# efmanu/SubspaceInference.jl

Measured on AMD Instinct MI355X. Metric: posterior samples/sec (whole node) + subspace-construct wall-clock, 1M-param MLP M=20, higher is better.
Workload: dtype f64

## Files before the change

include/subspace_hip.h:

```cpp
#ifndef SUBSPACE_HIP_H
#define SUBSPACE_HIP_H

#include <stdint.h>

#ifdef __cplusplus
extern "C" {
#endif

typedef struct si_ctx si_ctx;

enum {
  SI_OK = 0,
  SI_ERR_INVALID = -1,
  SI_ERR_STATE = -2,
  SI_ERR_HIP = -3,
  SI_ERR_NOMEM = -4,
  SI_ERR_BOUNDS = -5,
  SI_ERR_NODEVICE = -6,
  SI_ERR_COMM = -7
};

enum { SI_F32 = 0, SI_F64 = 1 };
enum { SI_ACT_IDENTITY = 0, SI_ACT_RELU = 1, SI_ACT_TANH = 2, SI_ACT_SIGMOID = 3, SI_ACT_LEAKYRELU = 4, SI_ACT_ELU = 5,
       SI_ACT_SOFTPLUS = 6, SI_ACT_SELU = 7, SI_ACT_COUNT = 8 };
enum { SI_LAYER_DENSE = 0, SI_LAYER_CONV = 1, SI_LAYER_MAXPOOL = 2, SI_LAYER_FLATTEN = 3 };

typedef struct {
  int32_t kind;
  int32_t in;
  int32_t out;
  int32_t act;
  int64_t w_off;
  int64_t b_off;
  int32_t kw, kh;
  int32_t cin, cout;
  int32_t wi, hi;
  int32_t sw, sh;
  int32_t pw, ph;
  int32_t dw, dh;
} si_layer;

enum {
  SI_K_PUSH = 0,
  SI_K_GRAM = 1,
  SI_K_GRAM_RED = 2,
  SI_K_PROJECT = 3,
  SI_K_RECON = 4,
  SI_K_DENSE = 5,
  SI_K_SSE = 6,
  SI_K_RWMH = 7,
  SI_K_DENSE_MAIN = 8,
  SI_K_EIG_HOST = 9,
  SI_K_BACKWARD = 10,
  SI_K_CONV = 11,
  SI_K_CONV_AUX = 12,
  SI_K_COUNT = 13
};

typedef struct {
  double ms[SI_K_COUNT];
  int64_t launches[SI_K_COUNT];
  double flops[SI_K_COUNT];
  double bytes[SI_K_COUNT];
} si_stats;

int32_t si_version(void);

int32_t si_create(si_ctx** out, int32_t device_id);
int32_t si_destroy(si_ctx* ctx);
const char* si_last_error(si_ctx* ctx);
int32_t si_set_stream(si_ctx* ctx, void* hip_stream);
int32_t si_synchronize(si_ctx* ctx);
int32_t si_set_profiling(si_ctx* ctx, int32_t on);
int32_t si_set_profiling_classes(si_ctx* ctx, uint32_t class_mask);
int32_t si_get_stats(si_ctx* ctx, si_stats* out);
int32_t si_reset_stats(si_ctx* ctx);
int32_t si_device_name(si_ctx* ctx, char* buf, int32_t buflen);

int32_t si_construct_begin(si_ctx* ctx, int64_t N, int64_t K_capacity, int32_t max_cols);
int32_t si_construct_set_mean(si_ctx* ctx, const void* w_host, int32_t w_dtype);
int32_t si_construct_set_storage(si_ctx* ctx, int32_t a_dtype);
int32_t si_construct_push(si_ctx* ctx, const void* w_host, int32_t w_dtype, double n);
int32_t si_construct_push_dev(si_ctx* ctx, const void* w_dev, int32_t w_dtype, double n);
int32_t si_construct_push_batch_dev(si_ctx* ctx, const void* w_dev, int32_t w_dtype, int64_t ld, int32_t count,
                                    const double* n_host);
int32_t si_construct_gram(si_ctx* ctx);
int32_t si_construct_gram_get(si_ctx* ctx, double* G_host , int64_t* K_out);
int32_t si_construct_gram_set(si_ctx* ctx, const double* G_host );
int32_t si_construct_gram_ptr(si_ctx* ctx, double** G_dev_out, int64_t* K_out);
int32_t si_construct_needs_refine(si_ctx* ctx, int32_t M, int32_t* flag_out);
int32_t si_construct_refine(si_ctx* ctx);
int32_t si_construct_finish(si_ctx* ctx, int32_t M, double* W_swa_out ,
                            double* P_out , double* s_out ,
                            int64_t* K_out);
int32_t si_construct_result_ptr(si_ctx* ctx, double** W_swa_dev_out, double** P_dev_out, int64_t* ld_out, int32_t* M_out);
int32_t si_construct_get_result(si_ctx* ctx, double* W_swa_out , double* P_out , double* s_out ,
                                int64_t* N_out, int32_t* M_out);
int32_t si_construct_get_A(si_ctx* ctx, int64_t k0, int64_t nk, double* A_out);

int32_t si_infer_setup(si_ctx* ctx, const si_layer* layers, int32_t L, int64_t N, int32_t M,
                       const double* W_swa, const double* P, const double* X, const double* Y,
                       int32_t in_dim, int32_t out_dim, int64_t B, double sigma_m,
                       int32_t compute_dtype);
int32_t si_infer_setup_dev(si_ctx* ctx, const si_layer* layers, int32_t L, int64_t N, int32_t M,
                           const double* W_swa_dev, const double* P_dev, int64_t ldP, int32_t borrow,
                           const double* X_dev, const double* Y_dev, int32_t in_dim, int32_t out_dim, int64_t B,
                           double sigma_m, int32_t compute_dtype);
int32_t si_infer_set_prior(si_ctx* ctx, double sigma_p);
int32_t si_logdensity(si_ctx* ctx, const double* Z, int32_t C, double* lp_out );
int32_t si_logdensity_grad(si_ctx* ctx, const double* z , double* lp_out, double* grad_out );
int32_t si_logdensity_grad_batch(si_ctx* ctx, const double* Z , int32_t C, double* lp_out ,
                                 double* grad_out );
int32_t si_grad_kernel_info(si_ctx* ctx, int32_t* fused_out);
int32_t si_sample_mala(si_ctx* ctx, int64_t itr, double sigma_z, uint64_t seed, int32_t chain_id0, int32_t nchains,
                       double* Z_out , double* lp_out , double* accept_rate_out ,
                       double* G_out );
int32_t si_mala_kernel_info(si_ctx* ctx, int32_t* fused_out, int32_t* passes_out);
int32_t si_sample_hmc(si_ctx* ctx, int64_t itr, int64_t n_adapts, double sigma_z, double delta, uint64_t seed, int32_t chain_id0,
                      int32_t nchains, double* Z_out , double* lp_out ,
                      double* alpha_out , double* eps_out ,
                      double* G_out , double* Minv_out );
int32_t si_hmc_kernel_info(si_ctx* ctx, int32_t* fused_out, int32_t* passes_out, int32_t* search_rounds_out);
int32_t si_sample_nuts(si_ctx* ctx, int64_t itr, int64_t n_adapts, double sigma_z, double delta, int32_t max_depth, double max_dh,
                       uint64_t seed, int32_t chain_id0, int32_t nchains, double* Z_out ,
                       double* lp_out , double* alpha_out , double* eps_out ,
                       int32_t* depth_out , int32_t* nleaf_out , int32_t* sel_out ,
                       double* G_out , double* Minv_out ,
                       double* leaf_out , int64_t leaf_cap);
int32_t si_nuts_kernel_info(si_ctx* ctx, int32_t* fused_out, int32_t* passes_out, int32_t* search_rounds_out, int64_t* rounds_out,
                            int64_t* leaves_out);
int32_t si_fit_advi(si_ctx* ctx, int64_t max_iters , int32_t samples_per_step , double sigma_z, double eta, double tau,
                    int32_t window , uint64_t seed, int32_t chain_id0, int32_t nruns , int64_t ndraws ,
                    double* theta_out , double* Z_out ,
                    double* elbo_out , double* theta_trace_out ,
                    double* points_out );
int32_t si_advi_kernel_info(si_ctx* ctx, int32_t* fused_out, int32_t* passes_out);
int32_t si_forward(si_ctx* ctx, const double* z , double* Yhat_out );
int32_t si_predict(si_ctx* ctx, const double* Z , int32_t C, const double* Xnew ,
                   int64_t Bn, double* Yhat_out);
int32_t si_sample_rwmh(si_ctx* ctx, int64_t itr, double sigma_z, uint64_t seed, int32_t chain_id0,
                       int32_t nchains, double* Z_out, double* lp_out, double* accept_rate_out);
int32_t si_sample_rwmh_weights(si_ctx* ctx, int64_t itr, double sigma_z, uint64_t seed, int32_t chain_id0,
                               int32_t nchains, double* Z_out, double* lp_out, double* accept_rate_out, double* W_out);
int32_t si_rwmh_begin(si_ctx* ctx, int64_t itr, double sigma_z, uint64_t seed, int32_t chain_id0, int32_t nchains,
                      int64_t d_total);
int32_t si_rwmh_step_eval(si_ctx* ctx, double* sse_local_out );
int32_t si_rwmh_step_accept(si_ctx* ctx, const double* sse_total );
int32_t si_rwmh_sse_ptr(si_ctx* ctx, double** sse_dev_out, int32_t* nchains_out);
int32_t si_rwmh_end(si_ctx* ctx, double* Z_out, double* lp_out, double* accept_rate_out);
int32_t si_rwmh_abort(si_ctx* ctx);
int32_t si_set_chain_loop(si_ctx* ctx, int32_t on);
int32_t si_chain_kernel_info(si_ctx* ctx, int32_t* density_specialised, int32_t* loop_specialised);
const char* si_chain_spec_message(si_ctx* ctx);
int32_t si_reconstruct(si_ctx* ctx, const double* Z , int64_t C, double* W_out);

int32_t si_train_setup(si_ctx* ctx, const si_layer* layers, int32_t L, int64_t N, const float* w0 ,
                       const double* X, const double* Y, int32_t in_dim, int32_t out_dim, int64_t B_total,
                       int64_t batch_max, int32_t opt_kind, double eta, double p1, double p2);
enum { SI_DTYPE_OF_DATA = -1 };
int32_t si_train_setup_ex(si_ctx* ctx, const si_layer* layers, int32_t L, int64_t N, const float* w0 , const void* X,
                          const void* Y, int32_t data_dtype, int32_t in_dim, int32_t out_dim, int64_t B_total, int64_t batch_max,
                          int32_t opt_kind, double eta, double p1, double p2, int32_t compute_dtype);
int32_t si_train_compute_dtype(si_ctx* ctx, int32_t* out );
int32_t si_train_step(si_ctx* ctx, const int64_t* idx , int64_t nb,
                      double* loss_out );
int32_t si_train_push(si_ctx* ctx, double n);
int32_t si_train_get_weights(si_ctx* ctx, float* w_out );
int32_t si_train_get_opt_state(si_ctx* ctx, float* m_out , float* v_out , double* beta_pows_out );
int32_t si_train_grad(si_ctx* ctx, const int64_t* idx, int64_t nb, int64_t nb_total, double* sse_local_out );
int32_t si_train_grad_ptr(si_ctx* ctx, double** grad_dev_out, int64_t* n_out);
int32_t si_train_grad_get(si_ctx* ctx, double* g_out );
int32_t si_train_grad_set(si_ctx* ctx, const double* g_in );
int32_t si_train_apply(si_ctx* ctx);

#define SI_COMM_ID_BYTES 128
enum { SI_COMM_SUM = 0, SI_COMM_MAX = 1 };
int32_t si_comm_unique_id(uint8_t* id_out );
int32_t si_comm_init_rank(si_ctx* ctx, int32_t world, int32_t rank, const uint8_t* id );
int32_t si_comm_destroy(si_ctx* ctx);
int32_t si_comm_info(si_ctx* ctx, int32_t* world_out, int32_t* rank_out, int32_t* rccl_version_out);
int32_t si_comm_allreduce_host(si_ctx* ctx, double* inout, int64_t n, int32_t op);
int32_t si_comm_allgather_host(si_ctx* ctx, const double* send , int64_t n, double* recv );
int32_t si_comm_barrier(si_ctx* ctx);
int32_t si_row_shard(int64_t n_total, int32_t rank, int32_t world, int64_t* r0_out, int64_t* r1_out);
int32_t si_construct_allreduce_gram(si_ctx* ctx);
int32_t si_construct_allgather(si_ctx* ctx, int64_t n_total);
int32_t si_bcast_subspace(si_ctx* ctx, int32_t root, int64_t N, int32_t M);
int32_t si_rwmh_allreduce_sse(si_ctx* ctx);
int32_t si_sample_rwmh_sharded(si_ctx* ctx, int64_t itr, double sigma_z, uint64_t seed, int32_t chain_id0, int32_t nchains,
                               int64_t d_total, double* Z_out, double* lp_out, double* accept_rate_out);
int32_t si_train_allreduce_grad(si_ctx* ctx, double* sse_total_out);
int32_t si_train_step_dp(si_ctx* ctx, const int64_t* idx, int64_t nb, int64_t nb_total, double* loss_out);

int si_host_sym_eig(int n, double* a, double* w);
int si_host_sym_eig_top(int n, const double* g, int m, double* w_top, double* V);
int si_host_jacobi_eig_psd(int n, double* a, double* w, double* v);
int32_t si_host_hmc_windows(int64_t n_adapts, int64_t* window_start, int64_t* window_end, int64_t* splits, int32_t cap);
int si_host_cpu_budget(void);
double si_host_parse_cpu_max(const char* text);
int si_host_copy_plan(int budget, int nproc, const char* env );

#ifdef __cplusplus
}
#endif
#endif
```

subspaceinference.jl_amd/_capi.py:

```python
import ctypes
import os
from ctypes import (POINTER, Structure, byref, c_char_p, c_double, c_int, c_int32, c_int64, c_uint64,
                    c_void_p)

import numpy as np

HERE = os.path.dirname(os.path.abspath(__file__))
LIB_PATH = os.path.join(HERE, "libsubspace_hip.so")

SI_OK, SI_ERR_INVALID, SI_ERR_STATE, SI_ERR_HIP, SI_ERR_NOMEM, SI_ERR_BOUNDS, SI_ERR_NODEVICE = 0, -1, -2, -3, -4, -5, -6
SI_ERR_COMM = -7
SI_COMM_ID_BYTES, SI_COMM_SUM, SI_COMM_MAX = 128, 0, 1
SI_F32, SI_F64 = 0, 1
SI_DTYPE_OF_DATA = -1
ACT_IDENTITY, ACT_RELU, ACT_TANH, ACT_SIGMOID = 0, 1, 2, 3
ACT_LEAKYRELU, ACT_ELU, ACT_SOFTPLUS, ACT_SELU = 4, 5, 6, 7
K_NAMES = ["push", "gram", "gram_reduce", "project", "reconstruct", "dense", "sse", "rwmh", "dense_main", "eig_host", "backward",
           "conv", "conv_aux"]
LAYER_DENSE, LAYER_CONV, LAYER_MAXPOOL, LAYER_FLATTEN = 0, 1, 2, 3
K_COUNT = len(K_NAMES)


class SubspaceError(RuntimeError):

    def __init__(self, msg, code=SI_ERR_INVALID):
        super().__init__(msg)
        self.code = code


class BoundsError(SubspaceError, IndexError):
    """Julia's BoundsError at `U[:,1:M]` (src/subspace_construction.jl:65) when rank(A) < M."""


class SiLayer(Structure):
    _fields_ = [("kind", c_int32), ("in_", c_int32), ("out", c_int32), ("act", c_int32),
                ("w_off", c_int64), ("b_off", c_int64),
                ("kw", c_int32), ("kh", c_int32), ("cin", c_int32), ("cout", c_int32), ("wi", c_int32), ("hi", c_int32),
                ("sw", c_int32), ("sh", c_int32), ("pw", c_int32), ("ph", c_int32), ("dw", c_int32), ("dh", c_int32)]


class SiStats(Structure):
    _fields_ = [("ms", c_double * K_COUNT), ("launches", c_int64 * K_COUNT),
                ("flops", c_double * K_COUNT), ("bytes", c_double * K_COUNT)]


SIGNATURES = {
    "si_version": (c_int32, []),
    "si_create": (c_int32, [POINTER(c_void_p), c_int32]),
    "si_destroy": (c_int32, [c_void_p]),
    "si_last_error": (c_char_p, [c_void_p]),
    "si_set_stream": (c_int32, [c_void_p, c_void_p]),
    "si_synchronize": (c_int32, [c_void_p]),
    "si_set_profiling": (c_int32, [c_void_p, c_int32]),
    "si_set_profiling_classes": (c_int32, [c_void_p, ctypes.c_uint32]),
    "si_get_stats": (c_int32, [c_void_p, POINTER(SiStats)]),
    "si_reset_stats": (c_int32, [c_void_p]),
    "si_device_name": (c_int32, [c_void_p, c_char_p, c_int32]),
    "si_construct_begin": (c_int32, [c_void_p, c_int64, c_int64, c_int32]),
    "si_construct_set_mean": (c_int32, [c_void_p, c_void_p, c_int32]),
    "si_construct_push": (c_int32, [c_void_p, c_void_p, c_int32, c_double]),
    "si_construct_push_dev": (c_int32, [c_void_p, c_void_p, c_int32, c_double]),
    "si_construct_push_batch_dev": (c_int32, [c_void_p, c_void_p, c_int32, c_int64, c_int32, c_void_p]),
    "si_construct_gram": (c_int32, [c_void_p]),
    "si_construct_gram_get": (c_int32, [c_void_p, c_void_p, POINTER(c_int64)]),
    "si_construct_gram_set": (c_int32, [c_void_p, c_void_p]),
    "si_construct_gram_ptr": (c_int32, [c_void_p, POINTER(c_void_p), POINTER(c_int64)]),
    "si_construct_result_ptr": (c_int32, [c_void_p, POINTER(c_void_p), POINTER(c_void_p), POINTER(c_int64),
                                          POINTER(c_int32)]),
    "si_construct_needs_refine": (c_int32, [c_void_p, c_int32, POINTER(c_int32)]),
    "si_construct_refine": (c_int32, [c_void_p]),
    "si_construct_finish": (c_int32, [c_void_p, c_int32, c_void_p, c_void_p, c_void_p, POINTER(c_int64)]),
    "si_construct_get_A": (c_int32, [c_void_p, c_int64, c_int64, c_void_p]),
    "si_construct_get_result": (c_int32, [c_void_p, c_void_p, c_void_p, c_void_p, POINTER(c_int64), POINTER(c_int32)]),
    "si_infer_setup": (c_int32, [c_void_p, POINTER(SiLayer), c_int32, c_int64, c_int32, c_void_p, c_void_p,
                                 c_void_p, c_void_p, c_int32, c_int32, c_int64, c_double, c_int32]),
    "si_infer_setup_dev": (c_int32, [c_void_p, POINTER(SiLayer), c_int32, c_int64, c_int32, c_void_p, c_void_p, c_int64,
                                     c_int32, c_void_p, c_void_p, c_int32, c_int32, c_int64, c_double, c_int32]),
    "si_infer_set_prior": (c_int32, [c_void_p, c_double]),
    "si_logdensity": (c_int32, [c_void_p, c_void_p, c_int32, c_void_p]),
    "si_logdensity_grad": (c_int32, [c_void_p, c_void_p, c_void_p, c_void_p]),
    "si_logdensity_grad_batch": (c_int32, [c_void_p, c_void_p, c_int32, c_void_p, c_void_p]),
    "si_grad_kernel_info": (c_int32, [c_void_p, POINTER(c_int32)]),
    "si_forward": (c_int32, [c_void_p, c_void_p, c_void_p]),
    "si_predict": (c_int32, [c_void_p, c_void_p, c_int32, c_void_p, c_int64, c_void_p]),
    "si_sample_rwmh": (c_int32, [c_void_p, c_int64, c_double, c_uint64, c_int32, c_int32, c_void_p, c_void_p,
                                 c_void_p]),
    "si_sample_rwmh_weights": (c_int32, [c_void_p, c_int64, c_double, c_uint64, c_int32, c_int32, c_void_p, c_void_p,
                                         c_void_p, c_void_p]),
    "si_sample_mala": (c_int32, [c_void_p, c_int64, c_double, c_uint64, c_int32, c_int32, c_void_p, c_void_p, c_void_p,
                                 c_void_p]),
    "si_mala_kernel_info": (c_int32, [c_void_p, POINTER(c_int32), POINTER(c_int32)]),
    "si_sample_hmc": (c_int32, [c_void_p, c_int64, c_int64, c_double, c_double, c_uint64, c_int32, c_int32, c_void_p, c_void_p,
                                c_void_p, c_void_p, c_void_p, c_void_p]),
    "si_hmc_kernel_info": (c_int32, [c_void_p, POINTER(c_int32), POINTER(c_int32), POINTER(c_int32)]),
    "si_sample_nuts": (c_int32, [c_void_p, c_int64, c_int64, c_double, c_double, c_int32, c_double, c_uint64, c_int32, c_int32,
                                 c_void_p, c_void_p, c_void_p, c_void_p, c_void_p, c_void_p, c_void_p, c_void_p, c_void_p, c_void_p,
                                 c_int64]),
    "si_nuts_kernel_info": (c_int32, [c_void_p, POINTER(c_int32), POINTER(c_int32), POINTER(c_int32), POINTER(c_int64),
                                      POINTER(c_int64)]),
    "si_fit_advi": (c_int32, [c_void_p, c_int64, c_int32, c_double, c_double, c_double, c_int32, c_uint64, c_int32, c_int32, c_int64,
                              c_void_p, c_void_p, c_void_p, c_void_p, c_void_p]),
    "si_advi_kernel_info": (c_int32, [c_void_p, POINTER(c_int32), POINTER(c_int32)]),
    "si_rwmh_begin": (c_int32, [c_void_p, c_int64, c_double, c_uint64, c_int32, c_int32, c_int64]),
    "si_rwmh_step_eval": (c_int32, [c_void_p, c_void_p]),
    "si_rwmh_step_accept": (c_int32, [c_void_p, c_void_p]),
    "si_rwmh_sse_ptr": (c_int32, [c_void_p, POINTER(c_void_p), POINTER(c_int32)]),
    "si_rwmh_end": (c_int32, [c_void_p, c_void_p, c_void_p, c_void_p]),
    "si_rwmh_abort": (c_int32, [c_void_p]),
    "si_reconstruct": (c_int32, [c_void_p, c_void_p, c_int64, c_void_p]),
    "si_train_setup": (c_int32, [c_void_p, POINTER(SiLayer), c_int32, c_int64, c_void_p, c_void_p, c_void_p, c_int32,
                                 c_int32, c_int64, c_int64, c_int32, c_double, c_double, c_double]),
    "si_train_setup_ex": (c_int32, [c_void_p, POINTER(SiLayer), c_int32, c_int64, c_void_p, c_void_p, c_void_p, c_int32, c_int32,
                                    c_int32, c_int64, c_int64, c_int32, c_double, c_double, c_double, c_int32]),
    "si_train_compute_dtype": (c_int32, [c_void_p, c_void_p]),
    "si_train_step": (c_int32, [c_void_p, c_void_p, c_int64, c_void_p]),
    "si_train_push": (c_int32, [c_void_p, c_double]),
    "si_train_get_weights": (c_int32, [c_void_p, c_void_p]),
    "si_train_get_opt_state": (c_int32, [c_void_p, c_void_p, c_void_p, c_void_p]),
    "si_train_grad": (c_int32, [c_void_p, c_void_p, c_int64, c_int64, c_void_p]),
    "si_train_grad_ptr": (c_int32, [c_void_p, c_void_p, c_void_p]),
    "si_train_grad_get": (c_int32, [c_void_p, c_void_p]),
    "si_train_grad_set": (c_int32, [c_void_p, c_void_p]),
    "si_train_apply": (c_int32, [c_void_p]),
    "si_comm_unique_id": (c_int32, [c_void_p]),
    "si_comm_init_rank": (c_int32, [c_void_p, c_int32, c_int32, c_void_p]),
    "si_comm_destroy": (c_int32, [c_void_p]),
    "si_comm_info": (c_int32, [c_void_p, POINTER(c_int32), POINTER(c_int32), POINTER(c_int32)]),
    "si_comm_allreduce_host": (c_int32, [c_void_p, c_void_p, c_int64, c_int32]),
    "si_comm_allgather_host": (c_int32, [c_void_p, c_void_p, c_int64, c_void_p]),
    "si_comm_barrier": (c_int32, [c_void_p]),
    "si_row_shard": (c_int32, [c_int64, c_int32, c_int32, POINTER(c_int64), POINTER(c_int64)]),
    "si_construct_allreduce_gram": (c_int32, [c_void_p]),
    "si_construct_allgather": (c_int32, [c_void_p, c_int64]),
    "si_bcast_subspace": (c_int32, [c_void_p, c_int32, c_int64, c_int32]),
    "si_rwmh_allreduce_sse": (c_int32, [c_void_p]),
    "si_sample_rwmh_sharded": (c_int32, [c_void_p, c_int64, c_double, c_uint64, c_int32, c_int32, c_int64, c_void_p, c_void_p,
                                         c_void_p]),
    "si_train_allreduce_grad": (c_int32, [c_void_p, c_void_p]),
    "si_train_step_dp": (c_int32, [c_void_p, c_void_p, c_int64, c_int64, c_void_p]),
    "si_host_sym_eig": (c_int, [c_int, c_void_p, c_void_p]),
    "si_host_sym_eig_top": (c_int, [c_int, c_void_p, c_int, c_void_p, c_void_p]),
    "si_host_jacobi_eig_psd": (c_int, [c_int, c_void_p, c_void_p, c_void_p]),
    "si_set_chain_loop": (c_int32, [c_void_p, c_int32]),
    "si_chain_kernel_info": (c_int32, [c_void_p, POINTER(c_int32), POINTER(c_int32)]),
    "si_chain_spec_message": (c_char_p, [c_void_p]),
    "si_construct_set_storage": (c_int32, [c_void_p, c_int32]),
    "si_host_hmc_windows": (c_int32, [c_int64, POINTER(c_int64), POINTER(c_int64), c_void_p, c_int32]),
    "si_host_cpu_budget": (c_int, []),
    "si_host_parse_cpu_max": (c_double, [c_char_p]),
    "si_host_copy_plan": (c_int, [c_int, c_int, c_char_p]),
}

_lib = None

ADVI_REFUSALS = (
    ("max_iters < 1", lambda a: not a["T"] >= 1),
    ("samples_per_step < 1", lambda a: not a["S"] >= 1),
    ("samples_per_step * ceil(M / 2) >= 2^24", lambda a: a["S"] * ((a["M"] + 1) // 2) >= 2 ** 24),
    ("window outside 1 .. 1024", lambda a: not 1 <= a["W"] <= 1024),
    ("nruns < 1", lambda a: not a["R"] >= 1),
    ("chain_id0 < 0", lambda a: not a["chain_id0"] >= 0),
    ("sigma_z <= 0", lambda a: not a["sigma_z"] > 0.0),
    ("tau <= 0", lambda a: not a["tau"] > 0.0),
    ("eta <= 0", lambda a: not a["eta"] > 0.0),
    ("ndraws < 0", lambda a: not a["D"] >= 0),
)


def advi_refusal(m, max_iters, samples_per_step, sigma_z, eta, tau, window, chain_id0, nruns, ndraws):
    a = dict(M=m, T=max_iters, S=samples_per_step, sigma_z=sigma_z, eta=eta, tau=tau, W=window, chain_id0=chain_id0, R=nruns, D=ndraws)
    return next((what for what, bad in ADVI_REFUSALS if bad(a)), None)


def load():
    global _lib
    if _lib is not None:
        return _lib
    if not os.path.exists(LIB_PATH):
        raise SubspaceError(
            "libsubspace_hip.so is missing (%s): build it with `python __graft_entry__.py` -- "
            "this package has no CPU or PyTorch fallback" % LIB_PATH, SI_ERR_NODEVICE)
    if os.environ.get("SI_PRELOAD_TORCH", "1") != "0":
        try:
            import torch
        except Exception:
            pass
    lib = ctypes.CDLL(LIB_PATH, mode=ctypes.RTLD_GLOBAL)
    for name, (res, args) in SIGNATURES.items():
        fn = getattr(lib, name)
        fn.restype = res
        fn.argtypes = args
    _lib = lib
    return lib


def _ptr(a):
    return None if a is None else c_void_p(a.__array_interface__["data"][0])


def conv_out_size(wi, k, s, p, d):
    return (wi + 2 * p - d * (k - 1) - 1) // s + 1


def _layer_array(table):
    arr = (SiLayer * len(table))()
    for i, row in enumerate(table):
        if row[0] == "conv":
            _, (kw, kh, cin, cout), (wi, hi), (sw, sh), (pw, ph), (dw, dh), act, w_off, b_off = row
            wo, ho = conv_out_size(wi, kw, sw, pw, dw), conv_out_size(hi, kh, sh, ph, dh)
            arr[i] = SiLayer(LAYER_CONV, wi * hi * cin, wo * ho * cout, int(act), int(w_off), int(b_off), kw, kh, cin, cout,
                             wi, hi, sw, sh, pw, ph, dw, dh)
        elif row[0] == "maxpool":
            _, (kw, kh), c, (wi, hi), (sw, sh) = row
            wo, ho = (wi - kw) // sw + 1, (hi - kh) // sh + 1
            arr[i] = SiLayer(LAYER_MAXPOOL, wi * hi * c, wo * ho * c, 0, 0, 0, kw, kh, c, c, wi, hi, sw, sh, 0, 0, 1, 1)
        elif row[0] == "flatten":
            _, c, (wi, hi) = row
            arr[i] = SiLayer(LAYER_FLATTEN, wi * hi * c, wi * hi * c, 0, 0, 0, 0, 0, c, c, wi, hi, 1, 1, 0, 0, 1, 1)
        else:
            fin, fout, act, w_off, b_off = row[:5]
            arr[i] = SiLayer(LAYER_DENSE, int(fin), int(fout), int(act), int(w_off), int(b_off))
    return arr


def _f64(a, order="F"):
    return np.require(a, dtype=np.float64, requirements=[order, "A"])


class Context:

    def __init__(self, device=0):
        self.lib = load()
        h = c_void_p()
        rc = self.lib.si_create(byref(h), int(device))
        if rc != SI_OK:
            msg = self.lib.si_last_error(None).decode()
            raise SubspaceError(msg, rc)
        self.h = h
        self.device = int(device)

    def _check(self, rc):
        if rc == SI_OK:
            return
        msg = self.lib.si_last_error(self.h).decode()
        if rc == SI_ERR_BOUNDS:
            raise BoundsError(msg, rc)
        raise SubspaceError(msg, rc)

    def close(self):
        if getattr(self, "h", None) is not None and self.h:
            self.lib.si_destroy(self.h)
            self.h = None

    def __del__(self):
        try:
            self.close()
        except Exception:
            pass

    def __enter__(self):
        return self

    def __exit__(self, *exc):
        self.close()

    def device_name(self):
        buf = ctypes.create_string_buffer(256)
        self._check(self.lib.si_device_name(self.h, buf, 256))
        return buf.value.decode()

    def set_stream(self, stream_handle):
        self._check(self.lib.si_set_stream(self.h, c_void_p(stream_handle) if stream_handle else None))

    def synchronize(self):
        self._check(self.lib.si_synchronize(self.h))

    def set_profiling(self, on, classes=None):
        self._check(self.lib.si_set_profiling(self.h, 1 if on else 0))
        mask = 0xFFFFFFFF if classes is None else sum(1 << K_NAMES.index(k) for k in classes)
        self._check(self.lib.si_set_profiling_classes(self.h, mask))

    def reset_stats(self):
        self._check(self.lib.si_reset_stats(self.h))

    def stats(self):
        st = SiStats()
        self._check(self.lib.si_get_stats(self.h, byref(st)))
        return {K_NAMES[i]: {"ms": st.ms[i], "launches": st.launches[i], "flops": st.flops[i], "bytes": st.bytes[i]}
                for i in range(K_COUNT)}

    def comm_init_rank(self, world, rank, uid):
        if len(uid) != SI_COMM_ID_BYTES:
            raise SubspaceError("comm_init_rank: the id must be %d bytes" % SI_COMM_ID_BYTES)
        buf = ctypes.create_string_buffer(bytes(uid), SI_COMM_ID_BYTES)
        self._check(self.lib.si_comm_init_rank(self.h, int(world), int(rank), buf))

    def comm_destroy(self):
        self._check(self.lib.si_comm_destroy(self.h))
# ... 246 lines not shown
            raise SubspaceError("DimensionMismatch: z has %d rows, M = %d" % (z.shape[0], self._m))
        lp = np.empty(z.shape[1], dtype=np.float64)
        self._check(self.lib.si_logdensity(self.h, _ptr(z), z.shape[1], _ptr(lp)))
        return lp

    def logdensity_grad(self, z):
        z = _f64(z).reshape(-1)
        if z.size != self._m:
            raise SubspaceError("DimensionMismatch: z has %d elements, M = %d" % (z.size, self._m))
        lp = np.empty(1, dtype=np.float64)
        g = np.empty(self._m, dtype=np.float64)
        self._check(self.lib.si_logdensity_grad(self.h, _ptr(z), _ptr(lp), _ptr(g)))
        return float(lp[0]), g

    def logdensity_grad_batch(self, z):
        z = _f64(z)
        if z.ndim == 1:
            z = z.reshape(-1, 1, order="F")
        if z.ndim != 2 or z.shape[0] != self._m:
            raise SubspaceError("DimensionMismatch: z has %d rows, M = %d" % (z.shape[0], self._m))
        lp = np.empty(z.shape[1], dtype=np.float64)
        g = np.empty((self._m, z.shape[1]), dtype=np.float64, order="F")
        self._check(self.lib.si_logdensity_grad_batch(self.h, _ptr(z), z.shape[1], _ptr(lp), _ptr(g)))
        return lp, g

    def grad_kernel_info(self):
        f = c_int32(0)
        self._check(self.lib.si_grad_kernel_info(self.h, byref(f)))
        return int(f.value)

    def forward(self, z):
        z = _f64(z).reshape(-1)
        yhat = np.empty((self._out, self._b), dtype=np.float64, order="F")
        self._check(self.lib.si_forward(self.h, _ptr(z), _ptr(yhat)))
        return yhat

    def predict(self, z, xnew):
        z = _f64(z)
        if z.ndim == 1:
            z = z.reshape(-1, 1, order="F")
        xnew = _f64(xnew)
        if z.shape[0] != self._m or xnew.ndim != 2 or xnew.shape[0] != self._in:
            raise SubspaceError("DimensionMismatch: Z %s, Xnew %s" % (z.shape, xnew.shape))
        out = np.empty((self._out, xnew.shape[1], z.shape[1]), dtype=np.float64, order="F")
        self._check(self.lib.si_predict(self.h, _ptr(z), z.shape[1], _ptr(xnew), xnew.shape[1], _ptr(out)))
        return out

    def sample_rwmh(self, itr, sigma_z, seed, chain_id0=0, nchains=1, want_z=True):
        z = np.empty((self._m, int(itr), int(nchains)), dtype=np.float64, order="F") if want_z else None
        lp = np.empty((int(itr), int(nchains)), dtype=np.float64, order="F")
        acc = np.empty(int(nchains), dtype=np.float64)
        self._check(self.lib.si_sample_rwmh(self.h, int(itr), float(sigma_z), int(seed), int(chain_id0), int(nchains),
                                            _ptr(z), _ptr(lp), _ptr(acc)))
        return z, lp, acc

    def sample_rwmh_weights(self, itr, sigma_z, seed, chain_id0=0, nchains=1, out=None):
        z = np.empty((self._m, int(itr), int(nchains)), dtype=np.float64, order="F")
        lp = np.empty((int(itr), int(nchains)), dtype=np.float64, order="F")
        acc = np.empty(int(nchains), dtype=np.float64)
        if out is None:
            w = np.empty((self._ni, int(itr), int(nchains)), dtype=np.float64, order="F")
        else:
            w = out
            if w.dtype != np.float64 or w.shape != (self._ni, int(itr), int(nchains)) or not w.flags.f_contiguous:
                raise ValueError("sample_rwmh_weights: `out` must be a Fortran-ordered float64 array of shape (N, itr, nchains)")
        self._check(self.lib.si_sample_rwmh_weights(self.h, int(itr), float(sigma_z), int(seed), int(chain_id0), int(nchains),
                                                    _ptr(z), _ptr(lp), _ptr(acc), _ptr(w)))
        return z, lp, acc, w

    def sample_mala(self, itr, sigma_z, seed, chain_id0=0, nchains=1, grad=False):
        z = np.empty((self._m, int(itr), int(nchains)), dtype=np.float64, order="F")
        lp = np.empty((int(itr), int(nchains)), dtype=np.float64, order="F")
        acc = np.empty(int(nchains), dtype=np.float64)
        g = np.empty((self._m, int(itr), int(nchains)), dtype=np.float64, order="F") if grad else None
        self._check(self.lib.si_sample_mala(self.h, int(itr), float(sigma_z), int(seed), int(chain_id0), int(nchains),
                                            _ptr(z), _ptr(lp), _ptr(acc), _ptr(g)))
        return (z, lp, acc, g) if grad else (z, lp, acc)

    def mala_kernel_info(self):
        f, p = c_int32(0), c_int32(0)
        self._check(self.lib.si_mala_kernel_info(self.h, byref(f), byref(p)))
        return int(f.value), int(p.value)

    def sample_hmc(self, itr, sigma_z, seed, chain_id0=0, nchains=1, n_adapts=None, delta=0.8, grad=False, metric=False):
        itr, c = int(itr), int(nchains)
        na = int(round(itr / 2)) if n_adapts is None else int(n_adapts)
        cols = max(itr, 0) + 1
        z = np.empty((self._m, cols, max(c, 0)), dtype=np.float64, order="F")
        lp, alpha, eps = (np.empty((cols, max(c, 0)), dtype=np.float64, order="F") for _ in range(3))
        g = np.empty_like(z, order="F") if grad else None
        mi = np.empty_like(z, order="F") if metric else None
        self._check(self.lib.si_sample_hmc(self.h, itr, na, float(sigma_z), float(delta), int(seed), int(chain_id0), c, _ptr(z),
                                           _ptr(lp), _ptr(alpha), _ptr(eps), _ptr(g), _ptr(mi)))
        return (z, lp, alpha, eps) + ((g,) if grad else ()) + ((mi,) if metric else ())

    def hmc_kernel_info(self):
        f, p, r = c_int32(0), c_int32(0), c_int32(0)
        self._check(self.lib.si_hmc_kernel_info(self.h, byref(f), byref(p), byref(r)))
        return int(f.value), int(p.value), int(r.value)

    def sample_nuts(self, itr, sigma_z, seed, chain_id0=0, nchains=1, n_adapts=None, delta=0.8, max_depth=10, max_dh=1000.0,
                    tree=True, grad=False, metric=False, leaf_cap=0):
        itr, c = int(itr), int(nchains)
        na = int(round(itr / 2)) if n_adapts is None else int(n_adapts)
        cols = max(itr, 0) + 1
        z = np.empty((self._m, cols, max(c, 0)), dtype=np.float64, order="F")
        lp, alpha, eps = (np.empty((cols, max(c, 0)), dtype=np.float64, order="F") for _ in range(3))
        depth, nleaf, sel = (np.zeros((cols, max(c, 0)), dtype=np.int32, order="F") if tree else None for _ in range(3))
        g = np.empty_like(z, order="F") if grad else None
        mi = np.empty_like(z, order="F") if metric else None
        leaf = np.full((3 * self._m + 1, int(leaf_cap), max(c, 0)), np.nan, dtype=np.float64, order="F") if leaf_cap else None
        self._check(self.lib.si_sample_nuts(self.h, itr, na, float(sigma_z), float(delta), int(max_depth), float(max_dh), int(seed),
                                            int(chain_id0), c, _ptr(z), _ptr(lp), _ptr(alpha), _ptr(eps), _ptr(depth), _ptr(nleaf),
                                            _ptr(sel), _ptr(g), _ptr(mi), _ptr(leaf), int(leaf_cap)))
        return ((z, lp, alpha, eps) + ((depth, nleaf, sel) if tree else ()) + ((g,) if grad else ()) + ((mi,) if metric else ())
                + ((leaf,) if leaf_cap else ()))

    def nuts_kernel_info(self):
        f, p, r = c_int32(0), c_int32(0), c_int32(0)
        n, lv = c_int64(0), c_int64(0)
        self._check(self.lib.si_nuts_kernel_info(self.h, byref(f), byref(p), byref(r), byref(n), byref(lv)))
        return int(f.value), int(p.value), int(r.value), int(n.value), int(lv.value)

    def fit_advi(self, max_iters, sigma_z, seed, samples_per_step=10, eta=0.1, tau=1.0, window=100, chain_id0=0, nruns=1,
                 ndraws=None, trace=False):
        t, s, w, r = int(max_iters), int(samples_per_step), int(window), int(nruns)
        d = t if ndraws is None else int(ndraws)
        why = advi_refusal(self._m, t, s, float(sigma_z), float(eta), float(tau), w, int(chain_id0), r, d)
        if why is not None:
            raise SubspaceError("si_fit_advi: bad argument (%s)" % why, SI_ERR_INVALID)
        m = self._m
        theta = np.empty((2 * m, r), dtype=np.float64, order="F")
        z = np.empty((m, d, r), dtype=np.float64, order="F")
        elbo = np.empty((t, r), dtype=np.float64, order="F")
        tr = np.empty((2 * m, t + 1, r), dtype=np.float64, order="F") if trace else None
        pts = np.empty((m, s, t, r), dtype=np.float64, order="F") if trace else None
        self._check(self.lib.si_fit_advi(self.h, t, s, float(sigma_z), float(eta), float(tau), w, int(seed), int(chain_id0), r, d,
                                         _ptr(theta), _ptr(z) if d > 0 else None, _ptr(elbo), _ptr(tr), _ptr(pts)))
        return (theta, z, elbo, tr, pts) if trace else (theta, z, elbo)

    def advi_kernel_info(self):
        f, p = c_int32(0), c_int32(0)
        self._check(self.lib.si_advi_kernel_info(self.h, byref(f), byref(p)))
        return int(f.value), int(p.value)

    def set_chain_loop(self, on):
        self._check(self.lib.si_set_chain_loop(self.h, int(on)))

    def chain_kernel_info(self):
        d, l = c_int32(0), c_int32(0)
        self._check(self.lib.si_chain_kernel_info(self.h, byref(d), byref(l)))
        return bool(d.value), bool(l.value), (self.lib.si_chain_spec_message(self.h) or b"").decode()

    def rwmh_begin(self, itr, sigma_z, seed, chain_id0=0, nchains=1, d_total=0):
        self._check(self.lib.si_rwmh_begin(self.h, int(itr), float(sigma_z), int(seed), int(chain_id0), int(nchains),
                                           int(d_total)))
        self._sw = (int(itr), int(nchains))

    def rwmh_step_eval(self, on_device=False):
        if on_device:
            self._check(self.lib.si_rwmh_step_eval(self.h, None))
            return None
        sse = np.empty(self._sw[1], dtype=np.float64)
        self._check(self.lib.si_rwmh_step_eval(self.h, _ptr(sse)))
        return sse

    def rwmh_step_accept(self, sse_total=None):
        if sse_total is None:
            self._check(self.lib.si_rwmh_step_accept(self.h, None))
            return
        sse_total = np.ascontiguousarray(sse_total, dtype=np.float64)
        self._check(self.lib.si_rwmh_step_accept(self.h, _ptr(sse_total)))

    def rwmh_sse_ptr(self):
        ptr, c = c_void_p(), c_int32()
        self._check(self.lib.si_rwmh_sse_ptr(self.h, byref(ptr), byref(c)))
        return int(ptr.value), int(c.value)

    def rwmh_abort(self):
        self._check(self.lib.si_rwmh_abort(self.h))

    def rwmh_end(self):
        itr, c = self._sw
        z = np.empty((self._m, itr, c), dtype=np.float64, order="F")
        lp = np.empty((itr, c), dtype=np.float64, order="F")
        acc = np.empty(c, dtype=np.float64)
        self._check(self.lib.si_rwmh_end(self.h, _ptr(z), _ptr(lp), _ptr(acc)))
        return z, lp, acc

    def reconstruct(self, z, out=None):
        z = _f64(z)
        if z.ndim == 1:
            z = z.reshape(-1, 1, order="F")
        if out is None:
            w = np.empty((self._ni, z.shape[1]), dtype=np.float64, order="F")
        else:
            w = out
            if w.dtype != np.float64 or w.shape != (self._ni, z.shape[1]) or not w.flags.f_contiguous:
                raise ValueError("reconstruct: `out` must be a Fortran-ordered float64 array of shape (N, C)")
        self._check(self.lib.si_reconstruct(self.h, _ptr(z), z.shape[1], _ptr(w)))
        return w


def comm_unique_id():
    lib = load()
    buf = ctypes.create_string_buffer(SI_COMM_ID_BYTES)
    rc = lib.si_comm_unique_id(buf)
    if rc != SI_OK:
        raise SubspaceError(lib.si_last_error(None).decode(), rc)
    return buf.raw


def row_shard(n_total, rank, world):
    r0, r1 = c_int64(), c_int64()
    if load().si_row_shard(int(n_total), int(rank), int(world), byref(r0), byref(r1)) != SI_OK:
        raise SubspaceError("si_row_shard: bad argument")
    return int(r0.value), int(r1.value)


def host_hmc_windows(n_adapts):
    lib = load()
    ws, we = c_int64(), c_int64()
    n = lib.si_host_hmc_windows(int(n_adapts), byref(ws), byref(we), None, 0)
    splits = np.zeros(max(1, n), dtype=np.int64)
    lib.si_host_hmc_windows(int(n_adapts), byref(ws), byref(we), _ptr(splits), n)
    return int(ws.value), int(we.value), [int(v) for v in splits[:n]]


def host_sym_eig(g):
    lib = load()
    a = np.array(g, dtype=np.float64, order="F")
    n = a.shape[0]
    w = np.empty(n, dtype=np.float64)
    rc = lib.si_host_sym_eig(n, _ptr(a), _ptr(w))
    if rc != 0:
        raise SubspaceError("eigensolver did not converge")
    return w, a


def host_sym_eig_top(g, m):
    lib = load()
    a = np.array(g, dtype=np.float64, order="F")
    n = a.shape[0]
    w = np.empty(int(m), dtype=np.float64)
    v = np.empty((n, int(m)), dtype=np.float64, order="F")
    rc = lib.si_host_sym_eig_top(n, _ptr(a), int(m), _ptr(w), _ptr(v))
    return (w, v) if rc == 0 else None


def host_jacobi_eig_psd(g):
    lib = load()
    a = np.array(g, dtype=np.float64, order="F")
    n = a.shape[0]
    w = np.empty(n, dtype=np.float64)
    v = np.empty((n, n), dtype=np.float64, order="F")
    lib.si_host_jacobi_eig_psd(n, _ptr(a), _ptr(w), _ptr(v))
    return w, v
```

subspaceinference.jl_amd/build.py:

```python
import os
import shutil
import subprocess

HERE = os.path.dirname(os.path.abspath(__file__))
CSRC = os.path.join(HERE, "csrc")
LIB = os.path.join(HERE, "libsubspace_hip.so")
ARCH = "gfx950"

SOURCES = [
    ("capi.hip", []),
    ("capi_infer.hip", []),
    ("capi_sample.hip", []),
    ("capi_mala.hip", []),
    ("capi_advi.hip", []),
    ("capi_hmc.hip", []),
    ("capi_nuts.hip", []),
    ("capi_train.hip", []),
    ("comm.hip", []),
    ("host_copy.cpp", []),
    ("kernels_stream.hip", ["-ffp-contract=off"]),
    ("kernels_chain.hip", ["-ffp-contract=off"]),
    ("kernels_mala.hip", ["-ffp-contract=off"]),
    ("kernels_hmc.hip", ["-ffp-contract=off"]),
    ("kernels_nuts.hip", ["-ffp-contract=off"]),
    ("kernels_advi.hip", ["-ffp-contract=off"]),
    ("kernels_chain_grid.hip", ["-ffp-contract=off", "-mllvm", "-amdgpu-mfma-vgpr-form=1"]),
    ("kernels_chain_grad.hip", ["-ffp-contract=off", "-mllvm", "-amdgpu-mfma-vgpr-form=1"]),
    ("kernels_gemm.hip", []),
    ("kernels_gemm_small.hip", []),
    ("kernels_gemm_panel.hip", []),
    ("kernels_gemm_f32.hip", []),
    ("kernels_gram.hip", []),
    ("kernels_gram_wave.hip", ["-DSI_GW_PART=0"], "kernels_gram_wave0"),
    ("kernels_gram_wave.hip", ["-DSI_GW_PART=1"], "kernels_gram_wave1"),
    ("kernels_gram_wave.hip", ["-DSI_GW_PART=2"], "kernels_gram_wave2"),
    ("kernels_project.hip", []),
    ("kernels_bwd.hip", []),
    ("kernels_bwd_f32.hip", []),
    ("kernels_conv.hip", []),
    ("kernels_conv.hip", ["-DSI_CONV_F32"], "kernels_conv_f32"),
    ("capi_net.hip", []),
    ("eig.cpp", ["-DSI_EIG_NS=base"]),
    ("eig.cpp", ["-DSI_EIG_NS=avx2", "-mavx2", "-mfma"], "eig_avx2"),
    ("eig.cpp", ["-DSI_EIG_NS=avx512", "-mavx512f", "-mavx512vl", "-mavx512dq", "-mfma"], "eig_avx512"),
    ("eig_dispatch.cpp", []),
    ("chain_spec_rtc.cpp", []),
]
HEADERS = ["si_internal.h", "dev_buf.h", "philox.h", "kernels_gemm.h", "gemm_pipeline.h", "chain_common.h", "hmc_device.h", "capi_common.h", "chain_spec.inc", "chain_spec_args.h",
           "chain_spec_rtc.h", os.path.join("..", "..", "include", "subspace_hip.h")]
SPEC_SOURCES = [("SI_SPEC_SRC_COMMON", "chain_common.h"), ("SI_SPEC_SRC_PHILOX", "philox.h"), ("SI_SPEC_SRC_ARGS", "chain_spec_args.h"),
                ("SI_SPEC_SRC_KERNELS", "chain_spec.inc")]


def _embed_spec_source(objdir):
    out = os.path.join(objdir, "chain_spec_src.h")
    parts = ["// generated by build.py from " + ", ".join(f for _, f in SPEC_SOURCES) + " -- do not edit\n"]
    for name, f in SPEC_SOURCES:
        text = open(os.path.join(CSRC, f)).read().replace("#pragma once", "")
        assert ')SISPEC"' not in text
        chunks, cur = [], ""
        for line in text.splitlines(keepends=True):
            if len(cur) + len(line) > 12000:
                chunks.append(cur)
                cur = ""
            cur += line
        chunks.append(cur)
        parts.append("static const char %s[] =\n%s;\n" % (name, "\n".join('R"SISPEC(' + c + ')SISPEC"' for c in chunks)))
    new = "".join(parts)
    if not os.path.exists(out) or open(out).read() != new:
        with open(out, "w") as fh:
            fh.write(new)
    return out


def _hipcc():
    exe = shutil.which("hipcc") or "/opt/rocm/bin/hipcc"
    if not os.path.exists(exe):
        raise RuntimeError("hipcc not found: cannot build libsubspace_hip.so")
    return exe


def _stale(target, deps):
    if not os.path.exists(target):
        return True
    t = os.path.getmtime(target)
    return any(os.path.getmtime(d) > t for d in deps)


DEV_LIB = os.path.join(os.path.dirname(HERE), "tools", "bin", "libsubspace_hip_dev.so")


def build(force=False, verbose=False, dev=False):
    hipcc = _hipcc()
    objdir = os.path.join(CSRC, "build_dev" if dev else "build")
    os.makedirs(objdir, exist_ok=True)
    lib = DEV_LIB if dev else LIB
    os.makedirs(os.path.dirname(lib), exist_ok=True)
    hdrs = [os.path.join(CSRC, h) for h in HEADERS] + [os.path.abspath(__file__)]
    _embed_spec_source(objdir)
    objs, jobs = [], []
    for entry in SOURCES + ([("guard_alloc.hip", [])] if dev else []):
        src, extra = entry[0], entry[1]
        s = os.path.join(CSRC, src)
        o = os.path.join(objdir, (entry[2] if len(entry) > 2 else os.path.splitext(src)[0]) + ".o")
        objs.append(o)
        if force or _stale(o, [s] + hdrs):
            jobs.append([hipcc, "--offload-arch=" + ARCH, "-O3", "-std=c++17", "-fPIC", "-Wall", "-Wno-unused-function",
                         "-I", objdir, "-c", s, "-o", o] + extra + (["-DSI_DEV_KNOBS"] if dev else []))

    def run(cmd):
        if verbose:
            print(" ".join(cmd))
        subprocess.run(cmd, check=True)
    if jobs:
        from concurrent.futures import ThreadPoolExecutor
        with ThreadPoolExecutor(max_workers=min(len(jobs), max(1, (os.cpu_count() or 2) - 1), 8)) as ex:
            list(ex.map(run, jobs))
    if force or _stale(lib, objs):
        cmd = [hipcc, "--offload-arch=" + ARCH, "-shared", "-fPIC", "-o", lib] + objs + ["-lhiprtc"]
        if verbose:
            print(" ".join(cmd))
        subprocess.run(cmd, check=True)
    return lib


if __name__ == "__main__":
    import sys
    print(build(verbose=True, dev="--dev" in sys.argv))
```

subspaceinference.jl_amd/csrc/capi.hip:

```cpp
#include <algorithm>
#include <cmath>
#include <chrono>
#include <cstdlib>
#include <cstring>
#include <new>
#include <type_traits>
#include <vector>

#include "capi_common.h"



namespace si {

#ifdef SI_DEV_KNOBS
hipError_t guard_malloc(void** out, size_t bytes);
hipError_t guard_free(void* p);
hipError_t raw_dev_malloc(void** out, size_t bytes) { return guard_malloc(out, bytes); }
hipError_t raw_dev_free(void* p) { return guard_free(p); }
#else
hipError_t raw_dev_malloc(void** out, size_t bytes) { return hipMalloc(out, bytes); }
hipError_t raw_dev_free(void* p) { return hipFree(p); }
#endif

static thread_local std::string g_create_err;

int32_t fail(Ctx* c, int32_t code, const std::string& msg) {
  if (c)
    c->err = msg;
  else
    g_create_err = msg;
  return code;
}

static hipEvent_t get_event(Ctx* c) {
  if (!c->event_pool.empty()) {
    hipEvent_t e = c->event_pool.back();
    c->event_pool.pop_back();
    return e;
  }
  hipEvent_t e = nullptr;
  if (hipEventCreate(&e) != hipSuccess) return nullptr;
  return e;
}

ProfScope::ProfScope(Ctx* c_, int cls_, double flops, double bytes) : c(c_), cls(cls_) {
  if (!c) return;
  c->stats.launches[cls] += 1;
  c->stats.flops[cls] += flops;
  c->stats.bytes[cls] += bytes;
  if (!c->profiling || !((c->prof_mask >> cls) & 1u) || c->pending.size() >= (1u << 20)) return;
  a = get_event(c);
  b = get_event(c);
  if (a && b) (void)hipEventRecord(a, c->stream);
}
ProfScope::~ProfScope() {
  if (!c || !a || !b) return;
  (void)hipEventRecord(b, c->stream);
  c->pending.push_back({a, b, cls});
}

static void resolve_events(Ctx* c) {
  for (auto& p : c->pending) {
    float ms = 0.f;
    if (hipEventElapsedTime(&ms, p.a, p.b) == hipSuccess) c->stats.ms[p.cls] += (double)ms;
    c->event_pool.push_back(p.a);
    c->event_pool.push_back(p.b);
  }
  c->pending.clear();
}


static void free_construct(Ctx* c) {
  if (c->i_ready && c->i_swa == c->d_swa && c->d_swa != nullptr) free_infer(c);
  static_cast<ConstructState&>(*c) = ConstructState();
}

void free_infer(Ctx* c) { static_cast<InferState&>(*c) = InferState(); }

int32_t construct_adopt(Ctx* c, int64_t N, int32_t M) {
  const int64_t ld = pad_ld(N);
  DevBuf<double> w, p;
  if (!w.alloc((size_t)ld) || !p.alloc((size_t)ld * (size_t)M))
    return fail(c, SI_ERR_NOMEM, "allocation of W_swa / P for a received subspace failed");
  SI_HIP(c, hipMemsetAsync(w, 0, (size_t)ld * sizeof(double), c->stream));
  SI_HIP(c, hipMemsetAsync(p, 0, (size_t)ld * (size_t)M * sizeof(double), c->stream));
  construct_install(c, N, M, w.release(), p.release());
  return SI_OK;
}

void construct_install(Ctx* c, int64_t N, int32_t M, double* w_swa, double* P) {
  (void)hipStreamSynchronize(c->stream);
  free_construct(c);
  c->N = N;
  c->ldA = pad_ld(N);
  c->d_swa.adopt(w_swa, (size_t)c->ldA);
  c->d_P.adopt(P, (size_t)c->ldA * (size_t)M);
  c->M_built = M;
  c->svals.assign((size_t)M, 0.0);
  c->c_active = false;
  c->c_finished = true;
}

struct DenseCost {
  double flops, bytes;
};
template <typename T>
static DenseCost dense_cost(const si_layer& ly, const si_layer* head, int slots, bool kept, int64_t B, int n) {
  const double es = (double)sizeof(T), w = (double)ly.in * ly.out, dB = (double)B, dn = (double)n;
  if (!head) return {2.0 * w * dB * dn, (w + ly.out + (double)(ly.in + ly.out) * dB) * es * dn};
  const double wh = (double)head->in * head->out;
  return {2.0 * (w + wh) * dB * dn, kept ? (w + ly.out + (double)(ly.in + ly.out) * dB) * es * dn
                                         : ((w + ly.out + (double)ly.in * dB + wh) * es + (double)slots * head->out * dB * 8.0) * dn};
}

template <typename T>
const T* dense_forward(Ctx* ctx, hipStream_t st, const DenseForward<T>& a) {
  constexpr bool f64 = std::is_same<T, double>::value;
  const size_t nl = a.nl, nplain = a.fuse_tail ? nl - 2 : nl;
  const int64_t B = a.B;
  ChainBatch cb = a.cb;
  cb.hin = 0;
  const T* h = a.X;
  for (size_t l = 0; l < nplain; ++l) {
    const si_layer& ly = a.layers[l];
    T* o = a.kept ? a.kept[l].get() : a.pingpong[l & 1];
    const DenseCost c = dense_cost<T>(ly, nullptr, 0, false, B, cb.n);
    {
      ProfScope ps(ctx, SI_K_DENSE, c.flops, a.traffic ? c.bytes : 0.0);
      ProfScope pm((int)l == a.main_layer ? ctx : nullptr, SI_K_DENSE_MAIN, c.flops, c.bytes);
      if constexpr (f64)
        launch_dense_f64(st, a.w + ly.w_off, a.w + ly.b_off, h, o, ly.out, ly.in, B, ly.act, cb);
      else
        launch_dense_f32(st, a.w + ly.w_off, a.w + ly.b_off, h, o, ly.out, ly.in, B, ly.act, cb);
    }
    h = o;
    cb.hin = cb.hout;
  }
  const si_layer& ll = a.layers[nl - 1];
  const int64_t di = (int64_t)ll.out * B;
  const double d = (double)di, dn = (double)cb.n;
  Ctx* sse_prof = a.traffic ? ctx : nullptr;
  if (a.fuse_tail) {
    const si_layer& ly = a.layers[nl - 2];
    const DenseCost c = dense_cost<T>(ly, &ll, a.slots, a.kept != nullptr, B, cb.n);
    {
      ProfScope ps(ctx, SI_K_DENSE, c.flops, a.traffic ? c.bytes : 0.0);
      ProfScope pm(((int)nl - 2 == a.main_layer || (int)nl - 1 == a.main_layer) ? ctx : nullptr, SI_K_DENSE_MAIN, c.flops, c.bytes);
      T* keep = a.kept ? a.kept[nl - 2].get() : nullptr;
      if constexpr (f64)
        launch_dense_f64_fused(st, a.w + ly.w_off, a.w + ly.b_off, h, ly.out, ly.in, B, ly.act, a.w + ll.w_off, ll.out, a.part, cb, keep);
      else
        launch_dense_f32_fused(st, a.w + ly.w_off, a.w + ly.b_off, h, ly.out, ly.in, B, ly.act, a.w + ll.w_off, ll.out, a.part, cb, keep);
    }
    ProfScope ps(sse_prof, SI_K_SSE, (3.0 + a.slots) * d * dn, (16.0 + 8.0 * a.slots) * d * dn);
    launch_tail_sse(st, a.part, a.slots, ll.out, B, a.w64 + ll.b_off, ll.act, a.Y, a.yhat, a.ssepart, a.sse_blocks, cb);
    if (!a.defer_sse_final) launch_sse_final(st, a.ssepart, a.sse_blocks, a.sse, cb.n);
  } else {
    ProfScope ps(sse_prof, SI_K_SSE, 3.0 * d * dn, (8.0 + (double)sizeof(T)) * d * dn);
    if constexpr (f64)
      launch_sse(st, h, a.Y, di, a.ssepart, a.sse_blocks, a.sse, cb.n, cb.hout, !a.defer_sse_final);
    else
      launch_sse_f32(st, h, a.Y, di, a.ssepart, a.sse_blocks, a.sse, cb.n, cb.hout, a.yhat, a.yhat ? di : 0, !a.defer_sse_final);
  }
  return h;
}
template const double* dense_forward<double>(Ctx*, hipStream_t, const DenseForward<double>&);
template const float* dense_forward<float>(Ctx*, hipStream_t, const DenseForward<float>&);

int32_t dense_reverse_sweep(Ctx* ctx, hipStream_t st, const DenseSweep& s) {
  int cur = 0;
  size_t top = s.nl;
  bool have_db = false;
  if (s.fuse_tail) {
    const si_layer& ll = s.layers[s.nl - 1];
    const si_layer& lp = s.layers[s.nl - 2];
    launch_rowsum(st, s.delta[cur], ll.out, s.B, s.rspart, s.gw + ll.b_off);
    launch_tail_bwd(st, s.w + ll.w_off, s.delta[cur], s.hs[s.nl - 2], ll.out, ll.in, s.B, lp.act, s.delta[cur ^ 1], s.bwpart,
                    s.gw + ll.w_off, s.gw + lp.b_off);
    cur ^= 1;
    top = s.nl - 1;
    have_db = true;
  }
  for (size_t li = top; li-- > 0;) {
    const si_layer& ly = s.layers[li];
    const double* hprev = li > 0 ? s.hs[li - 1] : s.X;
    launch_backward_weight(st, s.delta[cur], hprev, s.bwpart, ly.out, ly.in, s.B, ctx->num_cu, s.gw + ly.w_off,
                           (have_db && li + 1 == top) ? nullptr : s.gw + ly.b_off);
    if (li > 0) {
      launch_backward_data(st, s.w + ly.w_off, s.delta[cur], hprev, s.delta[cur ^ 1], ly.out, ly.in, s.B, s.layers[li - 1].act);
      cur ^= 1;
    }
  }
  return SI_OK;
}

int32_t dense_value_and_grad_f64(Ctx* ctx, hipStream_t st, const DenseValueGrad& s) {
  const DenseSweep& sw = s.sw;
  const size_t nl = sw.nl;
  const DenseForward<double> fw{sw.layers, nl, sw.fuse_tail, sw.w, sw.w, sw.X, s.Y, sw.B, sw.hs, {nullptr, nullptr}, ChainBatch(), s.slots,
                                s.part, sw.hs[nl - 1], s.ssepart, s.sse_blocks, s.sse, false, -1, s.traffic};
  dense_forward(ctx, st, fw);
  double bflops = 0.0;
  for (size_t l = 0; l < nl; ++l) bflops += 4.0 * (double)sw.layers[l].in * sw.layers[l].out * (double)sw.B;
  ProfScope ps(ctx, SI_K_BACKWARD, bflops, 0.0);
  SI_HIP(ctx, hipMemsetAsync(sw.gw, 0, (size_t)pad_ld(s.N) * sizeof(double), st));
  launch_delta_out(st, s.Y, sw.hs[nl - 1], (int64_t)sw.layers[nl - 1].out * sw.B, s.scale, sw.layers[nl - 1].act, sw.delta[0]);
  return dense_reverse_sweep(ctx, st, sw);
}

}

using namespace si;


extern "C" {

int32_t si_version(void) { return 500; }

const char* si_last_error(si_ctx* ctx) { return ctx ? ctx->err.c_str() : g_create_err.c_str(); }

int32_t si_create(si_ctx** out, int32_t device_id) {
  if (!out) return fail(nullptr, SI_ERR_INVALID, "si_create: out is NULL");
  *out = nullptr;
  int ndev = 0;
  hipError_t e = hipGetDeviceCount(&ndev);
  if (e != hipSuccess || ndev <= 0)
    return fail(nullptr, SI_ERR_NODEVICE,
                std::string("si_create: no HIP device available (") +
                    (e != hipSuccess ? hipGetErrorString(e) : "device count 0") +
                    "); this library has no CPU backend");
  if (device_id < 0 || device_id >= ndev)
    return fail(nullptr, SI_ERR_INVALID, "si_create: device_id out of range");
  si_ctx* c = new (std::nothrow) si_ctx();
  if (!c) return fail(nullptr, SI_ERR_NOMEM, "si_create: host allocation failed");
  c->device = device_id;
  hipDeviceProp_t prop;
  if ((e = hipSetDevice(device_id)) != hipSuccess || (e = hipGetDeviceProperties(&prop, device_id)) != hipSuccess ||
      (e = hipStreamCreateWithFlags(&c->own_stream, hipStreamNonBlocking)) != hipSuccess) {
    std::string m = std::string("si_create: ") + hipGetErrorString(e);
    delete c;
    return fail(nullptr, SI_ERR_HIP, m);
  }
  c->stream = c->own_stream;
  c->num_cu = prop.multiProcessorCount > 0 ? prop.multiProcessorCount : 256;
  snprintf(c->devname, sizeof(c->devname), "%s (%s)", prop.name, prop.gcnArchName);
  if (std::strncmp(prop.gcnArchName, "gfx950", 6) != 0) {
    std::string m = std::string("si_create: device is ") + prop.gcnArchName +
                    ", but libsubspace_hip.so carries gfx950 code objects only";
    (void)hipStreamDestroy(c->own_stream);
    delete c;
    return fail(nullptr, SI_ERR_NODEVICE, m);
  }
  *out = c;
  return SI_OK;
}

int32_t si_destroy(si_ctx* ctx) {
  CHECK_CTX(ctx);
  (void)hipSetDevice(ctx->device);
  (void)hipStreamSynchronize(ctx->stream);
  resolve_events(ctx);
  for (auto e : ctx->event_pool) (void)hipEventDestroy(e);
  comm_release(ctx);
  if (ctx->stream2) (void)hipStreamSynchronize(ctx->stream2);
  const hipStream_t stream2 = ctx->stream2, own_stream = ctx->own_stream;
  delete ctx;
  if (stream2) (void)hipStreamDestroy(stream2);
  if (own_stream) (void)hipStreamDestroy(own_stream);
  return SI_OK;
}

int32_t si_set_stream(si_ctx* ctx, void* hip_stream) {
  CHECK_CTX(ctx);
  BIND(ctx);
  SI_HIP(ctx, hipStreamSynchronize(ctx->stream));
  ctx->stream = hip_stream ? static_cast<hipStream_t>(hip_stream) : ctx->own_stream;
  return SI_OK;
}

int32_t si_synchronize(si_ctx* ctx) {
  CHECK_CTX(ctx);
  BIND(ctx);
  SI_HIP(ctx, hipStreamSynchronize(ctx->stream));
  return SI_OK;
}

int32_t si_set_profiling_classes(si_ctx* ctx, uint32_t class_mask) {
  CHECK_CTX(ctx);
  ctx->prof_mask = class_mask;
  return SI_OK;
}

int32_t si_set_profiling(si_ctx* ctx, int32_t on) {
  CHECK_CTX(ctx);
  ctx->profiling = on != 0;
  return SI_OK;
}

int32_t si_get_stats(si_ctx* ctx, si_stats* out) {
  CHECK_CTX(ctx);
  if (!out) return fail(ctx, SI_ERR_INVALID, "si_get_stats: out is NULL");
  BIND(ctx);
  SI_HIP(ctx, hipStreamSynchronize(ctx->stream));
  resolve_events(ctx);
  *out = ctx->stats;
  return SI_OK;
}

int32_t si_reset_stats(si_ctx* ctx) {
  CHECK_CTX(ctx);
  BIND(ctx);
  SI_HIP(ctx, hipStreamSynchronize(ctx->stream));
  resolve_events(ctx);
  std::memset(&ctx->stats, 0, sizeof(ctx->stats));
  return SI_OK;
}

int32_t si_device_name(si_ctx* ctx, char* buf, int32_t buflen) {
  CHECK_CTX(ctx);
  if (!buf || buflen <= 0) return fail(ctx, SI_ERR_INVALID, "si_device_name: bad buffer");
  std::strncpy(buf, ctx->devname, (size_t)buflen - 1);
  buf[buflen - 1] = 0;
  return SI_OK;
}

static int32_t ensure_A(si_ctx* ctx) {
  ctx->a_pending = false;
  const size_t esz = ctx->a_dtype == SI_F32 ? 4 : 8;
  const size_t need = (size_t)ctx->ldA * (size_t)ctx->Kcap * esz;
  if (ctx->d_A.size() < need) {
    SI_HIP(ctx, hipStreamSynchronize(ctx->stream));
    if (!ctx->d_A.alloc(need))
      return fail(ctx, SI_ERR_NOMEM, "si_construct_begin: device allocation of the deviation matrix failed");
    ctx->a_zero_dtype = -1;
    ctx->a_zero_cols = 0;
  }
  if (ctx->a_zero_dtype != ctx->a_dtype || ctx->a_zero_cols < ctx->Kcap) {
    if (ctx->ldA > ctx->N)
      SI_HIP(ctx, hipMemset2DAsync(ctx->d_A + (size_t)ctx->N * esz, (size_t)ctx->ldA * esz, 0,
                                   (size_t)(ctx->ldA - ctx->N) * esz, (size_t)ctx->Kcap, ctx->stream));
    ctx->a_zero_dtype = ctx->a_dtype;
    ctx->a_zero_cols = ctx->Kcap;
  }
  return SI_OK;
}

int32_t si_construct_begin(si_ctx* ctx, int64_t N, int64_t K_capacity, int32_t max_cols) {
  CHECK_CTX(ctx);
  if (N <= 0 || K_capacity <= 0 || max_cols < 0)
    return fail(ctx, SI_ERR_INVALID, "si_construct_begin: N and K_capacity must be positive, max_cols >= 0");
  BIND(ctx);
  SI_HIP(ctx, hipStreamSynchronize(ctx->stream));
  const int64_t kcap = max_cols > 0 ? std::min<int64_t>(max_cols, K_capacity) : K_capacity;
// ... 554 lines not shown
```

subspaceinference.jl_amd/csrc/capi_infer.hip:

```cpp
#include "capi_common.h"
#include "chain_spec_rtc.h"

using namespace si;

extern "C" {

static constexpr int SI_FUSED_MAX_WIDTH = 256;
static bool fused_chain_class(const si_ctx* ctx) {
  if (ctx->f32 || ctx->plan.has_conv) return false;
  const int L = (int)ctx->layers.size();
  if (L < 1 || L > SI_CHAIN_MAX_LAYERS) return false;
  for (int l = 0; l + 1 < L; ++l)
    if (ctx->layers[(size_t)l].out > SI_FUSED_MAX_WIDTH) return false;
  if (!ctx->fuse_tail && ctx->layers[(size_t)L - 1].out > SI_FUSED_MAX_WIDTH) return false;
  if ((int64_t)ctx->out_dim * ctx->B > (int64_t)256 * ctx->sse_blocks) return false;
  ChainFusedPlan fp;
  return chain_fused_plan(fp, ctx->layers.data(), L, ctx->B, 1, ctx->fuse_tail,
                          ctx->fuse_tail ? dense_fused_slot_feats(ctx->layers[(size_t)L - 2].out) : 0, ctx->fuse_slots) != 0;
}
void fused_fill_program(const si_ctx* ctx, ChainFusedPlan& fp) {
  fp.prog = ctx->d_cgprog;
  for (int i = 0; i < 5; ++i) {
    fp.prog_start[i] = ctx->cg_start[i];
    fp.prog_count[i] = ctx->cg_count[i];
    fp.prog_chunks[i] = ctx->cg_chunks[i];
  }
}
static size_t fused_plan_for(const si_ctx* ctx, int nchains, ChainFusedPlan& fp, int* nb_out, bool* wave_tiles) {
  fused_fill_program(ctx, fp);
  const int L = (int)ctx->layers.size();
  const int sf = ctx->fuse_tail ? dense_fused_slot_feats(ctx->layers[(size_t)L - 2].out) : 0;
  *wave_tiles = false;
  for (int nb : {2, 1}) {
    const size_t lds = chain_fused_plan(fp, ctx->layers.data(), L, ctx->B, nb, ctx->fuse_tail, sf, ctx->fuse_slots);
    const int64_t wgs = (ctx->B + 16 * nb - 1) / (16 * nb) * nchains;
    if (lds != 0 && (nb == 1 || (lds <= (size_t)80 * 1024 && wgs >= (int64_t)2 * ctx->num_cu))) {
      *nb_out = nb;
      return lds;
    }
  }
  return 0;
}

static bool alloc_forward(si_ctx* ctx, int slots) {
  for (DevBuf<double>* b : {&ctx->d_w, &ctx->d_act[0], &ctx->d_act[1], &ctx->d_ssepart, &ctx->d_part, &ctx->d_yhat}) b->reset();
  for (DevBuf<float>* b : {&ctx->d_w32, &ctx->d_act32[0], &ctx->d_act32[1]}) b->reset();
  ctx->fw_slots = 0;
  const size_t S = (size_t)slots, dB = (size_t)ctx->out_dim * (size_t)ctx->B;
  const size_t pslots = (size_t)std::max(ctx->fuse_slots, ctx->fuse_slots32);
  if (!ctx->d_w.alloc(S * (size_t)pad_ld(ctx->iN)) ||
      (!ctx->f32 && (!ctx->d_act[0].alloc(S * (size_t)ctx->act_elems) || !ctx->d_act[1].alloc(S * (size_t)ctx->act_elems))) ||
      (ctx->f32 && (!ctx->d_w32.alloc(S * (size_t)pad_ld(ctx->iN)) || !ctx->d_act32[0].alloc(S * (size_t)ctx->act_elems) ||
                    !ctx->d_act32[1].alloc(S * (size_t)ctx->act_elems))) ||
      !ctx->d_ssepart.alloc(S * (size_t)ctx->sse_blocks) ||
      (ctx->fuse_tail && !ctx->d_part.alloc(S * pslots * dB)) ||
      ((ctx->fuse_tail || ctx->f32 || ctx->fused_ok) && !ctx->d_yhat.alloc(S * dB)))
    return false;
  ctx->wsq_blocks = sse_num_blocks(ctx->iN, ctx->num_cu);
  if (!ctx->d_wsqpart.alloc(S * (size_t)ctx->wsq_blocks)) return false;
  ctx->fw_slots = slots;
  return true;
}

enum SetupSrc { SRC_HOST = 0, SRC_DEV_COPY = 1, SRC_DEV_BORROW = 2 };

static int32_t infer_setup_common(si_ctx* ctx, const si_layer* layers, int32_t L, int64_t N, int32_t M, const double* W_swa,
                                  const double* P, int64_t ldP_in, const double* X, const double* Y, int32_t in_dim,
                                  int32_t out_dim, int64_t B, double sigma_m, int32_t compute_dtype, SetupSrc src) {
  CHECK_CTX(ctx);
  if (!layers || L <= 0 || N <= 0 || M <= 0 || !X || !Y || in_dim <= 0 || out_dim <= 0 || B <= 0)
    return fail(ctx, SI_ERR_INVALID, "si_infer_setup: bad argument");
  if (!(sigma_m > 0.0)) return fail(ctx, SI_ERR_INVALID, "si_infer_setup: sigma_m must be positive");
  if (compute_dtype != SI_F64 && compute_dtype != SI_F32)
    return fail(ctx, SI_ERR_INVALID, "si_infer_setup: compute_dtype must be SI_F64 (the reference's arithmetic) or SI_F32");
  if ((W_swa == nullptr) != (P == nullptr))
    return fail(ctx, SI_ERR_INVALID, "si_infer_setup: W_swa and P must both be given or both be NULL");
  NetPlan plan;
  {
    const int32_t prc = net_plan(ctx, "si_infer_setup", layers, L, N, in_dim, out_dim, plan);
    if (prc != SI_OK) return prc;
  }
  int main_layer = 0;
  double main_flops = -1.0;
  for (int l = 0; l < L; ++l) {
    const LayerPlan& q = plan.L[(size_t)l];
    const double fl = q.kind == SI_LAYER_DENSE ? 2.0 * q.in_feat * (double)q.out_feat
                      : q.kind == SI_LAYER_CONV ? 2.0 * q.KW * q.KH * q.C * (double)q.Co * q.Wo * q.Ho : 0.0;
    if (fl > main_flops) {
      main_flops = fl;
      main_layer = l;
    }
  }
  BIND(ctx);
  SI_HIP(ctx, hipStreamSynchronize(ctx->stream));
  free_infer(ctx);
  if (!W_swa) {
    if (!ctx->c_finished) return fail(ctx, SI_ERR_STATE, "si_infer_setup: no finished construction to take W_swa / P from");
    if (ctx->N != N || ctx->M_built != M)
      return fail(ctx, SI_ERR_INVALID, "si_infer_setup: N / M differ from the finished construction");
    ctx->i_swa = ctx->d_swa;
    ctx->i_P = ctx->d_P;
    ctx->ldP = ctx->ldA;
  } else {
    if (src == SRC_DEV_BORROW) {
      ctx->ldP = ldP_in;
      ctx->i_swa = W_swa;
      ctx->i_P = P;
    } else {
      const hipMemcpyKind kind = src == SRC_HOST ? hipMemcpyHostToDevice : hipMemcpyDeviceToDevice;
      ctx->ldP = pad_ld(N);
      if (!ctx->d_iswa.alloc((size_t)ctx->ldP) || !ctx->d_iP.alloc((size_t)ctx->ldP * M)) {
        free_infer(ctx);
        return fail(ctx, SI_ERR_NOMEM, "si_infer_setup: allocation of W_swa / P failed");
      }
      SI_HIP(ctx, hipMemsetAsync(ctx->d_iswa, 0, (size_t)ctx->ldP * sizeof(double), ctx->stream));
      SI_HIP(ctx, hipMemsetAsync(ctx->d_iP, 0, (size_t)ctx->ldP * M * sizeof(double), ctx->stream));
      SI_HIP(ctx, hipMemcpyAsync(ctx->d_iswa, W_swa, (size_t)N * sizeof(double), kind, ctx->stream));
      SI_HIP(ctx, hipMemcpy2DAsync(ctx->d_iP, (size_t)ctx->ldP * sizeof(double), P, (size_t)ldP_in * sizeof(double),
                                   (size_t)N * sizeof(double), (size_t)M, kind, ctx->stream));
      ctx->i_swa = ctx->d_iswa;
      ctx->i_P = ctx->d_iP;
    }
  }
  ctx->layers.assign(layers, layers + L);
  ctx->iN = N;
  ctx->iM = M;
  ctx->in_dim = in_dim;
  ctx->out_dim = out_dim;
  ctx->B = B;
  ctx->sigma_m = sigma_m;
  ctx->main_layer = main_layer;
  ctx->plan = plan;
  ctx->fuse_tail = !plan.has_conv && (L >= 2) && layers[L - 1].out <= SI_FUSE_MAX_OUT &&
                   layers[L - 1].act < SI_ACT_LEAKYRELU && layers[L - 2].act < SI_ACT_LEAKYRELU;
  ctx->fuse_slots = ctx->fuse_tail ? dense_fused_slots(layers[L - 2].out) : 0;
  ctx->f32 = compute_dtype == SI_F32;
  ctx->fuse_slots32 = (ctx->f32 && ctx->fuse_tail) ? dense_f32_fused_slots(layers[L - 2].out, layers[L - 2].in, layers[L - 2].w_off % 4 == 0) : 0;
  int64_t maxstored = 1;
  for (int l = 0; l < (ctx->fuse_tail ? L - 2 : L); ++l) maxstored = std::max<int64_t>(maxstored, plan.L[(size_t)l].out_elems);
  ctx->max_stored = maxstored;
  ctx->act_elems = pad_ld(maxstored * B);
  ctx->sse_blocks = sse_num_blocks((int64_t)out_dim * B, ctx->num_cu);
  ctx->fused_ok = fused_chain_class(ctx);
  if (ctx->fused_ok) {
    std::vector<CgTileD> prog;
    chain_fused_program(ctx->layers.data(), L, ctx->fuse_tail, prog, ctx->cg_start, ctx->cg_count, ctx->cg_chunks);
    if (!ctx->d_cgprog.alloc(prog.size())) {
      free_infer(ctx);
      return fail(ctx, SI_ERR_NOMEM, "si_infer_setup: device allocation failed");
    }
    SI_HIP(ctx, hipMemcpy(ctx->d_cgprog, prog.data(), prog.size() * sizeof(CgTileD), hipMemcpyHostToDevice));
  }
  if (!ctx->d_X.alloc((size_t)in_dim * B) || !ctx->d_Y.alloc((size_t)out_dim * B) ||
      (ctx->f32 && !ctx->d_X32.alloc((size_t)pad_ld(std::max<int64_t>((int64_t)in_dim * B, plan.input_spatial ? plan.in_elems * B : 0)))) ||
      (ctx->f32 && plan.has_conv && !ctx->d_wpack32.alloc(plan.wpack_elems)) ||
      !alloc_forward(ctx, 1) ||
      (plan.has_conv && !ctx->d_wpack.alloc(plan.wpack_elems)) ||
      (plan.input_spatial && !ctx->d_Xc.alloc((size_t)plan.in_elems * B))) {
    free_infer(ctx);
    return fail(ctx, SI_ERR_NOMEM, "si_infer_setup: device allocation failed");
  }
  {
    const hipMemcpyKind kind = src == SRC_HOST ? hipMemcpyHostToDevice : hipMemcpyDeviceToDevice;
    SI_HIP(ctx, hipMemcpyAsync(ctx->d_X, X, (size_t)in_dim * B * sizeof(double), kind, ctx->stream));
    SI_HIP(ctx, hipMemcpyAsync(ctx->d_Y, Y, (size_t)out_dim * B * sizeof(double), kind, ctx->stream));
  }
  if (plan.input_spatial) net_input(ctx, plan, ctx->d_X, ctx->d_Xc, B);
  if (ctx->f32 && plan.input_spatial)
    launch_narrow_f32(ctx->stream, ctx->d_Xc, ctx->d_X32, plan.in_elems * B);
  else if (ctx->f32)
    launch_narrow_f32(ctx->stream, ctx->d_X, ctx->d_X32, (int64_t)in_dim * B);
  SI_HIP(ctx, hipGetLastError());
  SI_HIP(ctx, hipStreamSynchronize(ctx->stream));
  ctx->i_ready = true;
  return SI_OK;
}

int32_t si_infer_setup(si_ctx* ctx, const si_layer* layers, int32_t L, int64_t N, int32_t M, const double* W_swa,
                       const double* P, const double* X, const double* Y, int32_t in_dim, int32_t out_dim,
                       int64_t B, double sigma_m, int32_t compute_dtype) {
  return infer_setup_common(ctx, layers, L, N, M, W_swa, P, N, X, Y, in_dim, out_dim, B, sigma_m, compute_dtype, SRC_HOST);
}

int32_t si_infer_setup_dev(si_ctx* ctx, const si_layer* layers, int32_t L, int64_t N, int32_t M, const double* W_swa_dev,
                           const double* P_dev, int64_t ldP, int32_t borrow, const double* X_dev, const double* Y_dev,
                           int32_t in_dim, int32_t out_dim, int64_t B, double sigma_m, int32_t compute_dtype) {
  CHECK_CTX(ctx);
  if (W_swa_dev && P_dev) {
    if (ldP < N) return fail(ctx, SI_ERR_INVALID, "si_infer_setup_dev: ldP < N");
    if (borrow) {
      if ((ldP & 1) || ldP < N + (N & 1) || (reinterpret_cast<uintptr_t>(P_dev) & 15u) ||
          (reinterpret_cast<uintptr_t>(W_swa_dev) & 15u))
        return fail(ctx, SI_ERR_INVALID,
                    "si_infer_setup_dev: borrowed W_swa / P need 16-byte aligned bases, an even ldP >= N + (N mod 2) and "
                    "N + (N mod 2) readable elements of W_swa");
    }
  }
  return infer_setup_common(ctx, layers, L, N, M, W_swa_dev, P_dev, ldP, X_dev, Y_dev, in_dim, out_dim, B, sigma_m,
                            compute_dtype, borrow ? SRC_DEV_BORROW : SRC_DEV_COPY);
}

int32_t si_construct_result_ptr(si_ctx* ctx, double** W_swa_dev_out, double** P_dev_out, int64_t* ld_out, int32_t* M_out) {
  CHECK_CTX(ctx);
  if (!ctx->c_finished) return fail(ctx, SI_ERR_STATE, "si_construct_result_ptr: no finished construction");
  if (W_swa_dev_out) *W_swa_dev_out = ctx->d_swa;
  if (P_dev_out) *P_dev_out = ctx->d_P;
  if (ld_out) *ld_out = ctx->ldA;
  if (M_out) *M_out = ctx->M_built;
  return SI_OK;
}

static constexpr double SI_BATCH_BYTES = 2.0 * 1024.0 * 1024.0 * 1024.0;
static int batch_width(const si_ctx* ctx, int C) {
  if (ctx->plan.has_conv) return 1;
  const double pslots = (double)std::max(ctx->fuse_slots, ctx->fuse_slots32);
  const double per = (ctx->f32 ? 4.0 : 8.0) * 2.0 * (double)ctx->act_elems +
                     8.0 * ((pslots + 1.0) * (double)ctx->out_dim * (double)ctx->B + (ctx->f32 ? 1.5 : 1.0) * (double)pad_ld(ctx->iN) +
                            (double)ctx->sse_blocks);
  const double fit = std::floor(SI_BATCH_BYTES / per);
  return (int)std::max(1.0, std::min({(double)C, fit, 1024.0}));
}

int32_t ensure_chains(si_ctx* ctx, int32_t C) {
  const int want = batch_width(ctx, C);
  if (ctx->fw_slots < want) {
    SI_HIP(ctx, hipStreamSynchronize(ctx->stream));
    if (!alloc_forward(ctx, want)) {
      if (!alloc_forward(ctx, 1)) {
        ctx->i_ready = false;
        return fail(ctx, SI_ERR_NOMEM, "forward workspace allocation failed");
      }
    }
  }
  if (ctx->chains_cap >= C) return SI_OK;
  SI_HIP(ctx, hipStreamSynchronize(ctx->stream));
  for (DevBuf<double>* b : {&ctx->d_zcur, &ctx->d_zprop, &ctx->d_lpcur, &ctx->d_sse, &ctx->d_wsq}) b->reset();
  ctx->d_nacc.reset();
  ctx->d_steps.reset();
  ctx->chains_cap = 0;
  if (!ctx->d_wsq.alloc((size_t)C) || !ctx->d_zcur.alloc((size_t)ctx->iM * C) || !ctx->d_zprop.alloc((size_t)ctx->iM * C) ||
      !ctx->d_lpcur.alloc((size_t)C) || !ctx->d_sse.alloc((size_t)C) || !ctx->d_nacc.alloc((size_t)C) || !ctx->d_steps.alloc((size_t)C))
    return fail(ctx, SI_ERR_NOMEM, "sampler state allocation failed");
  ctx->chains_cap = C;
  return SI_OK;
}

int32_t eval_density(si_ctx* ctx, int c0, int nc, const double** yhat_out) {
  ctx->last_density_spec = 0;
  const int64_t N = ctx->iN, B = ctx->B, ldw = pad_ld(N);
  const int32_t M = ctx->iM;
  const double dn = (double)nc;
  {
    ProfScope ps(ctx, SI_K_RECON, 2.0 * (double)N * M * dn, (double)N * (M + 1 + dn) * 8.0);
    launch_reconstruct(ctx->stream, ctx->i_swa, ctx->i_P, ctx->ldP, N, M, ctx->d_zprop + (size_t)c0 * M, nc, ctx->d_w, ldw,
                       ctx->num_cu, ctx->f32 ? ctx->d_w32 : nullptr, ldw);
  }
  if (ctx->sigma_p > 0.0)
    launch_sse(ctx->stream, ctx->d_w, nullptr, N, ctx->d_wsqpart, ctx->wsq_blocks, ctx->d_wsq + c0, nc, ldw);
  if (ctx->plan.has_conv && ctx->f32) {
    float* last32 = nullptr;
    const int32_t rc = net_forward<float>(ctx, ctx->plan, ctx->d_w32, ctx->d_X32, B, ctx->d_act32, ctx->d_wpack32, true, &last32);
    if (rc != SI_OK) return rc;
    const int64_t d = (int64_t)ctx->out_dim * B;
    {
      ProfScope ps(ctx, SI_K_SSE, 3.0 * (double)d, 12.0 * (double)d);
      launch_sse_f32(ctx->stream, last32, ctx->d_Y, d, ctx->d_ssepart, ctx->sse_blocks, ctx->d_sse + c0, 1, ctx->act_elems,
                     yhat_out ? ctx->d_yhat : nullptr, d, !ctx->defer_sse_final);
    }
    SI_HIP(ctx, hipGetLastError());
    if (yhat_out) *yhat_out = ctx->d_yhat;
    return SI_OK;
  }
  if (ctx->plan.has_conv) {
    double* last = nullptr;
    const int32_t rc = net_forward<double>(ctx, ctx->plan, ctx->d_w, ctx->plan.input_spatial ? ctx->d_Xc : ctx->d_X, B, ctx->d_act,
                                           ctx->d_wpack, true, &last);
    if (rc != SI_OK) return rc;
    const int64_t d = (int64_t)ctx->out_dim * B;
    {
      ProfScope ps(ctx, SI_K_SSE, 3.0 * (double)d, 16.0 * (double)d);
      launch_sse(ctx->stream, last, ctx->d_Y, d, ctx->d_ssepart, ctx->sse_blocks, ctx->d_sse + c0, 1, ctx->act_elems, !ctx->defer_sse_final);
    }
    SI_HIP(ctx, hipGetLastError());
    if (yhat_out) *yhat_out = last;
    return SI_OK;
  }
  if (ctx->fused_ok && ctx->chain_mode != 0 && !yhat_out) {
    ChainFusedPlan fp;
    int nb = 1;
    bool wave_tiles = false;
    const size_t lds = fused_plan_for(ctx, nc, fp, &nb, &wave_tiles);
    if (lds != 0) {
      const int64_t d = (int64_t)ctx->out_dim * B;
      {
        const double fl = 2.0 * (double)N * (double)B * dn;
        const double by = ((double)N * dn + (double)ctx->in_dim * (double)B + (double)d * dn) * 8.0;
        ProfScope ps(ctx, SI_K_DENSE, fl, by);
        ProfScope pm(ctx, SI_K_DENSE_MAIN, fl, by);
        const SpecKernels* sk = nullptr;
        if (ctx->chain_spec && ctx->fuse_tail)
          sk = spec_kernels(ctx->layers.data(), (int)ctx->layers.size(), nb, dense_fused_slot_feats(ctx->layers[ctx->layers.size() - 2].out), 0, false,
                            &ctx->spec_message);
        ctx->last_density_spec = sk != nullptr;
        if (sk) {
          const double* wp = ctx->d_w;
          const double* xp = ctx->d_X;
          double* yp = ctx->d_yhat;
          long long ws = ldw, ys = d;
          int Bi = (int)B;
          void* args[] = {&wp, &ws, &xp, &yp, &ys, &Bi};
          if (sk->stack && nc >= 16) {
            const int splits = nc >= ctx->num_cu ? 1 : std::min(8, (ctx->num_cu + nc - 1) / nc);
            SI_HIP(ctx, hipModuleLaunchKernel(sk->stack, (unsigned)splits, (unsigned)nc, 1, 512, 1, 1,
                                              (unsigned)((size_t)sk->wvec_doubles * sizeof(double)), ctx->stream, args, nullptr));
          } else {
            SI_HIP(ctx, hipModuleLaunchKernel(sk->fused, (unsigned)((B + 16 * nb - 1) / (16 * nb)), (unsigned)nc, 1, 256, 1, 1,
                                              (unsigned)((size_t)sk->lds_doubles * sizeof(double)), ctx->stream, args, nullptr));
          }
        } else {
          launch_chain_fused(ctx->stream, fp, nb, wave_tiles, lds, ctx->d_w, ldw, ctx->d_X, ctx->d_yhat, d, nc);
        }
      }
      {
        ProfScope ps(ctx, SI_K_SSE, 3.0 * (double)d * dn, 16.0 * (double)d * dn);
        launch_sse(ctx->stream, ctx->d_yhat, ctx->d_Y, d, ctx->d_ssepart, ctx->sse_blocks, ctx->d_sse + c0, nc, d, !ctx->defer_sse_final);
      }
      SI_HIP(ctx, hipGetLastError());
      return SI_OK;
    }
  }
  const int slots = ctx->f32 ? ctx->fuse_slots32 : ctx->fuse_slots;
  ChainBatch cb;
  cb.n = nc;
  cb.w = ldw;
  cb.hout = ctx->act_elems;
  cb.part = (int64_t)slots * ctx->out_dim * B;
  const double* yh = ctx->d_yhat;
  double* yhat = yhat_out ? ctx->d_yhat.get() : nullptr;
  if (ctx->f32) {
    const DenseForward<float> fw{ctx->layers.data(), ctx->layers.size(), ctx->fuse_tail, ctx->d_w32, ctx->d_w, ctx->d_X32, ctx->d_Y, B, nullptr,
                                 {ctx->d_act32[0], ctx->d_act32[1]}, cb, slots, ctx->d_part, yhat, ctx->d_ssepart, ctx->sse_blocks,
                                 ctx->d_sse + c0, ctx->defer_sse_final, ctx->main_layer, true};
    dense_forward(ctx, ctx->stream, fw);
  } else {
    const DenseForward<double> fw{ctx->layers.data(), ctx->layers.size(), ctx->fuse_tail, ctx->d_w, ctx->d_w, ctx->d_X, ctx->d_Y, B, nullptr,
                                  {ctx->d_act[0], ctx->d_act[1]}, cb, slots, ctx->d_part, yhat, ctx->d_ssepart, ctx->sse_blocks,
                                  ctx->d_sse + c0, ctx->defer_sse_final, ctx->main_layer, true};
    const double* h = dense_forward(ctx, ctx->stream, fw);
    if (!ctx->fuse_tail) yh = h;
  }
  SI_HIP(ctx, hipGetLastError());
  if (yhat_out) *yhat_out = yh;
  return SI_OK;
}

int32_t eval_density_all(si_ctx* ctx, int C) {
  const int w = std::max(1, ctx->fw_slots);
  for (int c0 = 0; c0 < C; c0 += w) {
    const int32_t rc = eval_density(ctx, c0, std::min(w, C - c0), nullptr);
    if (rc != SI_OK) return rc;
  }
  return SI_OK;
}

double mvnormal_c0(double d, double sigma) {
  return -(d * std::log(2.0 * 3.14159265358979323846) + d * std::log(sigma * sigma)) / 2.0;
}

double prior_c0(const si_ctx* ctx) { return ctx->sigma_p > 0.0 ? mvnormal_c0((double)ctx->iN, ctx->sigma_p) : 0.0; }

int32_t si_infer_set_prior(si_ctx* ctx, double sigma_p) {
  CHECK_CTX(ctx);
  if (!ctx->i_ready) return fail(ctx, SI_ERR_STATE, "si_infer_set_prior: call si_infer_setup first");
  if (ctx->sw_Z) return fail(ctx, SI_ERR_STATE, "si_infer_set_prior: a step-wise RWMH session is open");
  if (!(sigma_p >= 0.0)) return fail(ctx, SI_ERR_INVALID, "si_infer_set_prior: sigma_p must be >= 0 (0 = off, the reference's behaviour)");
  ctx->sigma_p = sigma_p;
  return SI_OK;
}

int32_t si_logdensity(si_ctx* ctx, const double* Z, int32_t C, double* lp_out) {
  CHECK_CTX(ctx);
  if (!ctx->i_ready) return fail(ctx, SI_ERR_STATE, "si_logdensity: call si_infer_setup first");
  if (!Z || C <= 0 || !lp_out) return fail(ctx, SI_ERR_INVALID, "si_logdensity: bad argument");
  if (ctx->sw_Z) return fail(ctx, SI_ERR_STATE, "si_logdensity: a step-wise RWMH session is open; its proposal / SSE buffers are shared (si_rwmh_end or si_rwmh_abort first)");
  BIND(ctx);
  int32_t rc = ensure_chains(ctx, C);
  if (rc != SI_OK) return rc;
  SI_HIP(ctx, hipMemcpyAsync(ctx->d_zprop, Z, (size_t)ctx->iM * C * sizeof(double), hipMemcpyHostToDevice, ctx->stream));
  if ((rc = eval_density_all(ctx, C)) != SI_OK) return rc;
  std::vector<double> sse((size_t)C), wsq((size_t)C, 0.0);
  SI_HIP(ctx, hipMemcpyAsync(sse.data(), ctx->d_sse, (size_t)C * sizeof(double), hipMemcpyDeviceToHost, ctx->stream));
  if (ctx->sigma_p > 0.0)
    SI_HIP(ctx, hipMemcpyAsync(wsq.data(), ctx->d_wsq, (size_t)C * sizeof(double), hipMemcpyDeviceToHost, ctx->stream));
  SI_HIP(ctx, hipStreamSynchronize(ctx->stream));
  const double d = (double)ctx->out_dim * (double)ctx->B;
  const double c0 = mvnormal_c0(d, ctx->sigma_m), s2 = ctx->sigma_m * ctx->sigma_m;
  for (int c = 0; c < C; ++c) {
    lp_out[c] = c0 - (sse[(size_t)c] / s2) / 2.0;
    if (ctx->sigma_p > 0.0) lp_out[c] += prior_c0(ctx) - (wsq[(size_t)c] / (ctx->sigma_p * ctx->sigma_p)) / 2.0;
  }
  return SI_OK;
}

static int32_t drop_grad(si_ctx* ctx) {
  ctx->d_hs.clear();
  ctx->d_pidx.clear();
  ctx->g_scratch = NetScratch();
  ctx->g_ws32 = SweepF32Ws();
  for (DevBuf<double>* b : {&ctx->d_delta[0], &ctx->d_delta[1], &ctx->d_gw, &ctx->d_bwpart, &ctx->d_rspart, &ctx->d_ptgpart, &ctx->d_gz}) b->reset();
  return fail(ctx, SI_ERR_NOMEM, "si_logdensity_grad: workspace allocation failed");
}

static int32_t ensure_grad(si_ctx* ctx) {
  if (ctx->g_ready) return SI_OK;
  const int64_t B = ctx->B;
  if (ctx->plan.has_conv && ctx->f32)
    return fail(ctx, SI_ERR_INVALID, "si_logdensity_grad: compute_dtype = SI_F32 has a reverse sweep for Dense chains only; set a Conv chain up with SI_F64 for gradients");
  if (ctx->plan.has_conv) {
    const NetPlan& p = ctx->plan;
    size_t nb, nr, nw, nd;
    net_scratch_sizes(p, B, ctx->num_cu, &nb, &nr, &nw, &nd);
    ctx->d_hs = std::vector<DevBuf<double>>(p.L.size());
    ctx->d_pidx = std::vector<DevBuf<uint8_t>>(p.L.size());
    bool ok = true;
    for (size_t l = 0; l < p.L.size() && ok; ++l) {
      if (net_grad_fused(p, l))
        ok = ctx->d_pidx[l].alloc(net_pidx_bytes(p, l, B));
      else
        ok = ctx->d_hs[l].alloc((size_t)p.L[l].out_elems * B);
    }
    ctx->g_scratch.pidx = ctx->d_pidx.data();
    ok = ok && ctx->d_delta[0].alloc((size_t)p.max_elems * B) && ctx->d_delta[1].alloc((size_t)p.max_elems * B) &&
         ctx->d_gw.alloc((size_t)pad_ld(ctx->iN)) && ctx->g_scratch.bwpart.alloc(nb) && ctx->g_scratch.rspart.alloc(nr) &&
         ctx->g_scratch.wt.alloc(nw) && ctx->g_scratch.dbtmp.alloc(nd) && ctx->d_ptgpart.alloc((size_t)ptg_blocks() * ctx->iM) &&
         ctx->d_gz.alloc((size_t)ctx->iM);
    if (!ok) return drop_grad(ctx);
    ctx->g_ready = true;
    return SI_OK;
  }
  if (ctx->f32) {
    const bool ok32 = sweep_f32_alloc(ctx, ctx->g_ws32, ctx->layers.data(), (int)ctx->layers.size(), ctx->fuse_tail, ctx->iN, ctx->in_dim,
                                      ctx->out_dim, B) &&
                      ctx->d_gw.alloc((size_t)pad_ld(ctx->iN)) && ctx->d_ptgpart.alloc((size_t)ptg_blocks() * ctx->iM) &&
                      ctx->d_gz.alloc((size_t)ctx->iM);
    if (!ok32) return drop_grad(ctx);
    ctx->g_ready = true;
    return SI_OK;
  }
  int64_t maxw = 1;
  size_t maxpart = 1;
  ctx->d_hs = std::vector<DevBuf<double>>(ctx->layers.size());
  bool ok = true;
  for (size_t l = 0; l < ctx->layers.size() && ok; ++l) {
    const si_layer& ly = ctx->layers[l];
    maxw = std::max<int64_t>(maxw, ly.out);
    maxpart = std::max(maxpart, backward_weight_part_elems(ly.out, ly.in, B, ctx->num_cu));
    ok = ctx->d_hs[l].alloc((size_t)ly.out * B);
  }
  if (ctx->fuse_tail) maxpart = std::max(maxpart, tail_bwd_part_elems(ctx->layers.back().out, ctx->layers.back().in));
  ok = ok && ctx->d_delta[0].alloc((size_t)maxw * B) && ctx->d_delta[1].alloc((size_t)maxw * B) &&
       ctx->d_gw.alloc((size_t)pad_ld(ctx->iN)) && ctx->d_bwpart.alloc(maxpart) && ctx->d_rspart.alloc((size_t)rowsum_chunks() * maxw) &&
       ctx->d_ptgpart.alloc((size_t)ptg_blocks() * ctx->iM) && ctx->d_gz.alloc((size_t)ctx->iM);
  if (!ok) return drop_grad(ctx);
  ctx->g_ready = true;
  return SI_OK;
}

static int32_t logdensity_grad_point(si_ctx* ctx, const double* z, double* lp_out, double* grad_out) {
  int32_t rc = ensure_chains(ctx, 1);
  if (rc != SI_OK) return rc;
  if ((rc = ensure_grad(ctx)) != SI_OK) return rc;
  const int64_t N = ctx->iN, B = ctx->B;
  const int32_t M = ctx->iM;
  const size_t nl = ctx->layers.size();
  const double s2 = ctx->sigma_m * ctx->sigma_m;
  SI_HIP(ctx, hipMemcpyAsync(ctx->d_zprop, z, (size_t)M * sizeof(double), hipMemcpyHostToDevice, ctx->stream));
  {
    ProfScope ps(ctx, SI_K_RECON, 2.0 * (double)N * M, (double)N * (M + 2) * 8.0);
    launch_reconstruct(ctx->stream, ctx->i_swa, ctx->i_P, ctx->ldP, N, M, ctx->d_zprop, 1, ctx->d_w, pad_ld(N), ctx->num_cu,
                       ctx->f32 ? ctx->d_w32 : nullptr, pad_ld(N));
  }
  const bool prior = ctx->sigma_p > 0.0;
  if (prior) launch_sse(ctx->stream, ctx->d_w, nullptr, N, ctx->d_wsqpart, ctx->wsq_blocks, ctx->d_wsq, 1, pad_ld(N));
  if (ctx->f32) {
    DenseSweepF32 sw{ctx->layers.data(), nl, ctx->fuse_tail, ctx->d_w32, ctx->d_w, ctx->d_X32, ctx->d_Y, &ctx->g_ws32, ctx->d_part,
                     ctx->d_ssepart, ctx->d_sse, ctx->sse_blocks, B, N, 1.0 / s2};
    if ((rc = dense_value_and_grad_f32(ctx, ctx->stream, sw)) != SI_OK) return rc;
    launch_widen_f32_to_f64(ctx->stream, ctx->g_ws32.gw32, N, ctx->d_gw, ctx->num_cu);
  } else if (ctx->plan.has_conv) {
    const NetPlan& p = ctx->plan;
    double bflops = 0.0;
    for (const auto& q : p.L)
      bflops += q.kind == SI_LAYER_DENSE ? 4.0 * (double)q.in_feat * q.out_feat * (double)B
                : q.kind == SI_LAYER_CONV ? 4.0 * (double)q.KW * q.KH * q.C * q.Co * (double)q.Wo * q.Ho * (double)B : 0.0;
    const NetValueGrad vg{&p, ctx->d_w, p.input_spatial ? ctx->d_Xc : ctx->d_X, ctx->d_Y, B, ctx->d_hs.data(), ctx->d_wpack, ctx->d_ssepart,
                          ctx->sse_blocks, ctx->d_sse, {ctx->d_delta[0], ctx->d_delta[1]}, ctx->d_gw, &ctx->g_scratch, N, 1.0 / s2, bflops};
    if ((rc = net_value_and_grad(ctx, vg)) != SI_OK) return rc;
  } else {
    const DenseValueGrad vg{{ctx->layers.data(), nl, ctx->fuse_tail, ctx->d_w, ctx->d_X, ctx->d_hs.data(), {ctx->d_delta[0], ctx->d_delta[1]},
                             ctx->d_gw, ctx->d_rspart, ctx->d_bwpart, B},
                            ctx->d_Y, ctx->fuse_slots, ctx->d_part, ctx->d_ssepart, ctx->d_sse, ctx->sse_blocks, N, 1.0 / s2, true};
    if ((rc = dense_value_and_grad_f64(ctx, ctx->stream, vg)) != SI_OK) return rc;
  }
  if (prior) launch_prior_grad(ctx->stream, ctx->d_gw, ctx->d_w, N, 1.0 / (ctx->sigma_p * ctx->sigma_p), ctx->num_cu);
  launch_ptg(ctx->stream, ctx->i_P, ctx->ldP, N, M, ctx->d_gw, ctx->d_ptgpart, ctx->d_gz);
  SI_HIP(ctx, hipGetLastError());
  double sse = 0.0, wsq = 0.0;
  SI_HIP(ctx, hipMemcpyAsync(&sse, ctx->d_sse, sizeof(double), hipMemcpyDeviceToHost, ctx->stream));
  SI_HIP(ctx, hipMemcpyAsync(grad_out, ctx->d_gz, (size_t)M * sizeof(double), hipMemcpyDeviceToHost, ctx->stream));
  if (prior) SI_HIP(ctx, hipMemcpyAsync(&wsq, ctx->d_wsq, sizeof(double), hipMemcpyDeviceToHost, ctx->stream));
  SI_HIP(ctx, hipStreamSynchronize(ctx->stream));
  const int64_t d = (int64_t)ctx->out_dim * B;
  *lp_out = mvnormal_c0((double)d, ctx->sigma_m) - (sse / s2) / 2.0;
  if (prior) *lp_out += prior_c0(ctx) - (wsq / (ctx->sigma_p * ctx->sigma_p)) / 2.0;
  return SI_OK;
}

int32_t grad_entry_check(si_ctx* ctx, const char* who, bool args_ok) {
  if (!ctx->i_ready) return fail(ctx, SI_ERR_STATE, std::string(who) + ": call si_infer_setup first");
  if (!args_ok) return fail(ctx, SI_ERR_INVALID, std::string(who) + ": bad argument");
  if (ctx->sw_Z) return fail(ctx, SI_ERR_STATE, std::string(who) + ": a step-wise RWMH session is open; its proposal / SSE buffers are shared (si_rwmh_end or si_rwmh_abort first)");
  return SI_OK;
}

int32_t si_logdensity_grad(si_ctx* ctx, const double* z, double* lp_out, double* grad_out) {
  CHECK_CTX(ctx);
  const int32_t rc = grad_entry_check(ctx, "si_logdensity_grad", z && lp_out && grad_out);
  if (rc != SI_OK) return rc;
  BIND(ctx);
  return logdensity_grad_point(ctx, z, lp_out, grad_out);
}

static int vgrad_class(si_ctx* ctx) {
  if (ctx->vg_class >= 0) return ctx->vg_class;
  ctx->vg_class = 0;
  if (ctx->f32 || ctx->plan.has_conv) return 0;
  const int L = (int)ctx->layers.size();
  ChainVgradPlan vp;
  if (chain_vgrad_plan(vp, ctx->layers.data(), L, ctx->B, 1) == 0) return 0;
  if (ctx->layers[0].in != ctx->in_dim || ctx->layers[(size_t)L - 1].out != ctx->out_dim) return 0;
  std::vector<char> seen((size_t)ctx->iN, 0);
  auto mark = [&](int64_t off, int64_t n) {
    if (off < 0 || off + n > ctx->iN) return false;
    for (int64_t i = off; i < off + n; ++i) {
      if (seen[(size_t)i]) return false;
      seen[(size_t)i] = 1;
    }
    return true;
  };
  int64_t total = 0;
  for (const si_layer& ly : ctx->layers) {
    if (!mark(ly.w_off, (int64_t)ly.in * ly.out) || !mark(ly.b_off, ly.out)) return 0;
    total += (int64_t)ly.in * ly.out + ly.out;
  }
  if (total != ctx->iN) return 0;
  const size_t lds2 = chain_vgrad_plan(vp, ctx->layers.data(), L, ctx->B, 2);
  ctx->vg_class = (lds2 != 0 && lds2 <= (size_t)64 * 1024) ? 2 : 1;
  return ctx->vg_class;
}

static int vgrad_route(si_ctx* ctx, int64_t* G_out, int64_t* fit_out) {
  const int64_t B = ctx->B, ldw = pad_ld(ctx->iN);
  const int nb = vgrad_class(ctx);
  const int64_t G = nb > 0 ? (B + 16 * nb - 1) / (16 * nb) : 0;
  const double per = 8.0 * ((double)ldw * ((double)G + 2.0) + (double)G + 2.0 * ctx->iM + 1.0);
  *G_out = G;
  *fit_out = nb > 0 ? (int64_t)std::min(65535.0, std::floor(SI_BATCH_BYTES / per)) : 0;
  return nb;
}

static int32_t vgrad_ensure(si_ctx* ctx, const char* who, int cap, int64_t G) {
  if (ctx->vg_cap >= cap) return SI_OK;
  const int64_t ldw = pad_ld(ctx->iN);
  const int32_t M = ctx->iM;
  SI_HIP(ctx, hipStreamSynchronize(ctx->stream));
  const size_t S = (size_t)cap;
  ctx->vg_cap = 0;
  if (!ctx->d_vg_z.alloc(S * M) || !ctx->d_vg_w.alloc(S * (size_t)ldw) || !ctx->d_vg_part.alloc(S * (size_t)G * (size_t)ldw) ||
      !ctx->d_vg_ssepart.alloc(S * (size_t)G) || !ctx->d_vg_gw.alloc(S * (size_t)ldw) || !ctx->d_vg_lp.alloc(S) ||
      !ctx->d_vg_gz.alloc(S * M)) {
    for (DevBuf<double>* b : {&ctx->d_vg_z, &ctx->d_vg_w, &ctx->d_vg_part, &ctx->d_vg_ssepart, &ctx->d_vg_gw, &ctx->d_vg_lp, &ctx->d_vg_gz})
      b->reset();
    return fail(ctx, SI_ERR_NOMEM, std::string(who) + ": workspace allocation failed");
  }
  ctx->vg_cap = cap;
  return SI_OK;
}

static void vgrad_pass(si_ctx* ctx, int nb, int64_t G, const double* z_dev, int n, double* lp_dev, double* gz_dev) {
  const int64_t N = ctx->iN, B = ctx->B, ldw = pad_ld(N);
  const int32_t M = ctx->iM;
  ChainVgradPlan vp;
  const size_t lds = chain_vgrad_plan(vp, ctx->layers.data(), (int)ctx->layers.size(), B, nb);
  const double s2 = ctx->sigma_m * ctx->sigma_m;
  const double c0 = mvnormal_c0((double)ctx->out_dim * (double)B, ctx->sigma_m);
  {
    ProfScope ps(ctx, SI_K_RECON, 2.0 * (double)N * M * n, (double)N * (M + 1 + n) * 8.0);
    launch_reconstruct(ctx->stream, ctx->i_swa, ctx->i_P, ctx->ldP, N, M, z_dev, n, ctx->d_vg_w, ldw, ctx->num_cu);
  }
  {
    ProfScope ps(ctx, SI_K_BACKWARD, 6.0 * (double)N * (double)B * n, 0.0);
    launch_chain_vgrad(ctx->stream, vp, nb, lds, ctx->d_vg_w, ldw, ctx->d_X, ctx->d_Y, 1.0 / s2, ctx->d_vg_part, ldw, ctx->d_vg_ssepart, n);
    launch_chain_vgrad_reduce(ctx->stream, ctx->d_vg_part, (int)G, N, ldw, ctx->d_vg_ssepart, ctx->d_vg_w, ldw, ctx->i_P, ctx->ldP, M,
                              ctx->sigma_p, prior_c0(ctx), c0, s2, ctx->d_vg_gw, lp_dev, gz_dev, n);
  }
}

}

namespace si {

int32_t StackedVgrad::open(si_ctx* c, const char* who, int32_t npoints) {
  ctx = c, C = npoints;
  int64_t fit = 0;
  nb = vgrad_route(ctx, &G, &fit);
  fused = fit >= 1;
  if (fused) {
    const int32_t rc = vgrad_ensure(ctx, who, (int)std::min<int64_t>(fit, C), G);
    if (rc != SI_OK) return rc;
  } else {
    hz.resize((size_t)ctx->iM * C);
    hlp.resize((size_t)C);
    hg.resize((size_t)ctx->iM * C);
  }
  passes = fused ? (C + ctx->vg_cap - 1) / ctx->vg_cap : C;
  return SI_OK;
}

void StackedVgrad::eval(const double* z_dev, double* lp_dev, double* g_dev, hipError_t& e, int32_t& rc) {
  const size_t M = (size_t)ctx->iM;
  if (fused) {
    for (int32_t p0 = 0; p0 < C; p0 += ctx->vg_cap)
      vgrad_pass(ctx, nb, G, z_dev + M * p0, std::min<int32_t>(ctx->vg_cap, C - p0), lp_dev + p0, g_dev + M * p0);
    e = hipGetLastError();
    return;
  }
  e = hipMemcpyAsync(hz.data(), z_dev, hz.size() * sizeof(double), hipMemcpyDeviceToHost, ctx->stream);
  if (e == hipSuccess) e = hipStreamSynchronize(ctx->stream);
  for (int32_t c = 0; c < C && e == hipSuccess && rc == SI_OK; ++c)
    rc = logdensity_grad_point(ctx, hz.data() + M * c, hlp.data() + c, hg.data() + M * c);
  if (rc != SI_OK) return;
  if (e == hipSuccess) e = hipMemcpyAsync(lp_dev, hlp.data(), hlp.size() * sizeof(double), hipMemcpyHostToDevice, ctx->stream);
  if (e == hipSuccess) e = hipMemcpyAsync(g_dev, hg.data(), hg.size() * sizeof(double), hipMemcpyHostToDevice, ctx->stream);
}

int32_t finish_downloads(si_ctx* ctx, const char* who, hipError_t e, int32_t rc, std::initializer_list<Download> downs) {
  for (const Download& d : downs)
    if (e == hipSuccess && rc == SI_OK && d.dst) e = hipMemcpyAsync(d.dst, d.src, d.bytes, hipMemcpyDeviceToHost, ctx->stream);
  const hipError_t e2 = hipStreamSynchronize(ctx->stream);
  if (rc != SI_OK) return rc;
  if (e != hipSuccess) return fail(ctx, SI_ERR_HIP, std::string(who) + ": " + hipGetErrorString(e));
  if (e2 != hipSuccess) return fail(ctx, SI_ERR_HIP, std::string(who) + ": " + hipGetErrorString(e2));
  return SI_OK;
}
// ... 117 lines not shown
```

subspaceinference.jl_amd/csrc/kernels_gemm.hip:

```cpp
#include <type_traits>

#include "kernels_gemm.h"

namespace si {

#ifdef SI_GEMM_DEBUG_KNOB
__device__ int si_gemm_dbg = 0;
static size_t si_gemm_lds_floor = 0;
__device__ long long si_gemm_stamps[4 * 16384];
#define SI_STAMP(i) do { if (threadIdx.x == 0 && blockIdx.x < 16384) si_gemm_stamps[4 * blockIdx.x + (i)] = __builtin_amdgcn_s_memtime(); } while (0)
#else
#define SI_STAMP(i) do {} while (0)
#endif

__device__ __forceinline__ double apply_act(double v, int act) {
  switch (act) {
    case SI_ACT_RELU: return v > 0.0 ? v : 0.0;
    case SI_ACT_TANH: return tanh(v);
    case SI_ACT_SIGMOID: return 1.0 / (1.0 + exp(-v));
    default: return v;
  }
}

template <int BM, int BN, int WM, int WN, int MINW, bool VEC, bool KEDGE, bool FUSE>
// ... 229 lines not shown
    return apply_act(v, act);
  };
  if constexpr (FUSE) {
    int gi[TM];
    double bv[TM];
#pragma unroll
    for (int a = 0; a < TM; ++a) {
      gi[a] = iw0 + a * 16 + c;
      bv[a] = gi[a] < out ? bias[gi[a]] : 0.0;
    }
#pragma unroll
    for (int a = 0; a < TM; ++a)
#pragma unroll
      for (int b = 0; b < TN; ++b)
#pragma unroll
        for (int r = 0; r < 4; ++r) acc[a][b][r] = finish(acc[a][b][r] + bv[a]);
    if (Hout != nullptr) {
#pragma unroll
      for (int a = 0; a < TM; ++a)
#pragma unroll
        for (int b = 0; b < TN; ++b)
#pragma unroll
          for (int r = 0; r < 4; ++r) {
            const int64_t gb = bw0 + b * 16 + q + 4 * r;
            if (gi[a] < out && gb < B) Hout[gi[a] + (int64_t)out * gb] = acc[a][b][r];
          }
    }
    const int64_t slot = (int64_t)mt * WM + wm;
    for (int o = 0; o < out_last; ++o) {
      double wl[TM];
#pragma unroll
      for (int a = 0; a < TM; ++a) wl[a] = gi[a] < out ? Wlast[o + (int64_t)out_last * gi[a]] : 0.0;
#pragma unroll
      for (int b = 0; b < TN; ++b) {
#pragma unroll
        for (int r = 0; r < 4; ++r) {
          double p = 0.0;
#pragma unroll
          for (int a = 0; a < TM; ++a) p = fma(acc[a][b][r], wl[a], p);
          p += __shfl_xor(p, 8, 16);
          p += __shfl_xor(p, 4, 16);
          p += __shfl_xor(p, 2, 16);
          p += __shfl_xor(p, 1, 16);
          const int64_t gb = bw0 + b * 16 + q + 4 * r;
          if (c == 0 && gb < B) part[(slot * out_last + o) * (cb.part_ld ? cb.part_ld : B) + gb] = p;
        }
      }
    }
  } else if constexpr (WIDE) {
    constexpr int CH_ROW = WI / 2;
    constexpr int NCH = 16 * CH_ROW / 64;
    double* reg = smem + wave * (16 * WI);
    constexpr bool FIXCOL = 64 % CH_ROW == 0;
    const int col2_fixed = lane % CH_ROW;
    double2 bfix = make_double2(0.0, 0.0);
    if (FIXCOL) {
      const int gi = iw0 + 2 * col2_fixed;
      if (gi + 1 < out) bfix = *reinterpret_cast<const double2*>(bias + gi);
    }
#pragma unroll
    for (int bt = 0; bt < TN; ++bt) {
#pragma unroll
      for (int a = 0; a < TM; ++a)
#pragma unroll
        for (int r = 0; r < 4; ++r) reg[(q + 4 * r) * WI + a * 16 + c] = acc[a][bt][r];
#pragma unroll
      for (int p = 0; p < NCH; ++p) {
        const int chunk = p * 64 + lane;
        const int row = chunk / CH_ROW, col2 = chunk % CH_ROW;
        const double2 v = *reinterpret_cast<const double2*>(reg + 2 * chunk);
        const int gi = iw0 + 2 * col2;
        const int64_t gb = bw0 + bt * 16 + row;
        double2 bv = bfix;
        if (!FIXCOL) bv = (gi + 1 < out) ? *reinterpret_cast<const double2*>(bias + gi) : make_double2(0.0, 0.0);
        if (gi + 1 < out && gb < B && !(dbg & 16))
          *reinterpret_cast<double2*>(Hout + gi + (int64_t)out * gb) = make_double2(finish(v.x + bv.x), finish(v.y + bv.y));
      }
    }
  } else {
#pragma unroll
    for (int a = 0; a < TM; ++a) {
      const int gi = iw0 + a * 16 + c;
      const double bv = (gi < out) ? bias[gi] : 0.0;
#pragma unroll
      for (int b = 0; b < TN; ++b) {
#pragma unroll
        for (int r = 0; r < 4; ++r) {
          const int64_t gb = bw0 + b * 16 + q + 4 * r;
          if (gi < out && gb < B) Hout[gi + (int64_t)out * gb] = finish(acc[a][b][r] + bv);
        }
      }
    }
  }
  SI_STAMP(3);
}

struct FuseArgs {
  const double* Wlast = nullptr;
  int out_last = 0;
  double* part = nullptr;
  ChainBatch cb;
};

template <int BM, int BN, int WM, int WN, int MINW, bool VEC, bool KEDGE, bool FUSE>
static void launch_dense_inst(hipStream_t st, const double* W, const double* bias, const double* Hin, double* Hout,
                              int32_t out, int32_t in, int64_t B, int32_t act, const FuseArgs& fa) {
  size_t lds = 2 * (16 * (BM + 16) + BN * 18) * sizeof(double);
#ifdef SI_GEMM_DEBUG_KNOB
  if (si_gemm_lds_floor > lds) lds = si_gemm_lds_floor;
#endif
  constexpr int NT = 64 * WM * WN;
  const int nMt = (out + BM - 1) / BM;
  const int64_t nNt = (B + BN - 1) / BN;
  const int64_t groups = (nNt + 7) / 8;
  const int64_t grid = groups * nMt * 8;
  auto kern = dense_f64_kernel<BM, BN, WM, WN, MINW, VEC, KEDGE, FUSE>;
  static LdsOptIn optin;
  optin.ensure(reinterpret_cast<const void*>(kern), lds);
  hipLaunchKernelGGL(kern, dim3((unsigned)grid, (unsigned)fa.cb.n), dim3(NT), lds, st, W, bias, Hin, Hout, (int)out,
                     (int)in, B, (int)act, nMt, nNt, fa.Wlast, fa.out_last, fa.part, fa.cb);
}

template <int BM, int BN, int WM, int WN, int MINW, bool FUSE = false>
void launch_dense_cfg(hipStream_t st, const double* W, const double* bias, const double* Hin, double* Hout,
                      int32_t out, int32_t in, int64_t B, int32_t act, const FuseArgs& fa = FuseArgs()) {
  const bool vec = (out % 2 == 0) && (in % 2 == 0) && ((reinterpret_cast<uintptr_t>(W) & 15u) == 0) &&
                   ((reinterpret_cast<uintptr_t>(Hin) & 15u) == 0) &&
                   (FUSE || (((reinterpret_cast<uintptr_t>(Hout) & 15u) == 0) && ((reinterpret_cast<uintptr_t>(bias) & 15u) == 0))) &&
                   (((fa.cb.w | fa.cb.hin | fa.cb.hout) & 1) == 0);
  const bool kedge = (in % 16) != 0;
  if (vec && !kedge)
    launch_dense_inst<BM, BN, WM, WN, MINW, true, false, FUSE>(st, W, bias, Hin, Hout, out, in, B, act, fa);
  else if (vec)
    launch_dense_inst<BM, BN, WM, WN, MINW, true, true, FUSE>(st, W, bias, Hin, Hout, out, in, B, act, fa);
  else if (!kedge)
    launch_dense_inst<BM, BN, WM, WN, MINW, false, false, FUSE>(st, W, bias, Hin, Hout, out, in, B, act, fa);
  else
    launch_dense_inst<BM, BN, WM, WN, MINW, false, true, FUSE>(st, W, bias, Hin, Hout, out, in, B, act, fa);
}

#ifndef SI_GEMM_NO_DISPATCH
static int pick_bm(int32_t out) {
  if (out <= 32) return 32;
  auto padded = [&](int bm) { return (out + bm - 1) / bm * bm; };
  const int p96 = padded(96), p128 = padded(128), p64 = padded(64);
  if (p96 <= p128 && p96 <= p64) return 96;
  return p128 <= p64 ? 128 : 64;
}

int dense_fused_slot_feats(int32_t out);
int dense_fused_slots(int32_t out);

void launch_dense_f64(hipStream_t st, const double* W, const double* bias, const double* Hin,
                      double* Hout, int32_t out, int32_t in, int64_t B, int32_t act, const ChainBatch& cb) {
  if (act_is_extra(act)) {
    launch_dense_f64(st, W, bias, Hin, Hout, out, in, B, SI_ACT_IDENTITY, cb);
    for (int s = 0; s < cb.n; ++s) launch_act_inplace(st, Hout + (int64_t)s * cb.hout, (int64_t)out * B, act);
    return;
  }
  if (dense_small_applies(out, in, B, cb.n, pick_bm(out))) {
    launch_dense_small_f64(st, W, bias, Hin, Hout, out, in, B, act, dense_fused_slot_feats(out), cb);
    return;
  }
  if (cb.n <= 1 && dense_panel_applies(W, out, in, B, act) && launch_dense_f64_panel(st, W, bias, Hin, Hout, out, in, B, act))
    return;
  FuseArgs fa;
  fa.cb = cb;
  switch (pick_bm(out)) {
    case 32: launch_dense_cfg<32, 128, 1, 4, 2>(st, W, bias, Hin, Hout, out, in, B, act, fa); break;
    case 96: launch_dense_cfg<96, 128, 2, 4, 4>(st, W, bias, Hin, Hout, out, in, B, act, fa); break;
    case 128: launch_dense_cfg<128, 128, 2, 4, 4>(st, W, bias, Hin, Hout, out, in, B, act, fa); break;
    default: launch_dense_cfg<64, 128, 2, 4, 4>(st, W, bias, Hin, Hout, out, in, B, act, fa); break;
  }
}

int dense_fused_slots(int32_t out) {
  const int bm = pick_bm(out);
  const int wm = bm == 32 ? 1 : 2;
  return (out + bm - 1) / bm * wm;
}

int dense_fused_slot_feats(int32_t out) {
  const int bm = pick_bm(out);
  return bm == 32 ? 32 : bm / 2;
}

void launch_dense_f64_fused(hipStream_t st, const double* W, const double* bias, const double* Hin, int32_t out,
                            int32_t in, int64_t B, int32_t act, const double* Wlast, int32_t out_last, double* part,
                            const ChainBatch& cb, double* Hkeep) {
  if (dense_small_applies(out, in, B, cb.n, pick_bm(out))) {
    launch_dense_small_f64_fused(st, W, bias, Hin, out, in, B, act, dense_fused_slot_feats(out), dense_fused_slots(out), Wlast, out_last,
                                 part, cb, Hkeep);
    return;
  }
  FuseArgs fa;
  fa.Wlast = Wlast;
  fa.out_last = out_last;
  fa.part = part;
  fa.cb = cb;
  switch (pick_bm(out)) {
    case 32: launch_dense_cfg<32, 128, 1, 4, 2, true>(st, W, bias, Hin, Hkeep, out, in, B, act, fa); break;
    case 96: launch_dense_cfg<96, 128, 2, 4, 4, true>(st, W, bias, Hin, Hkeep, out, in, B, act, fa); break;
    case 128: launch_dense_cfg<128, 128, 2, 4, 4, true>(st, W, bias, Hin, Hkeep, out, in, B, act, fa); break;
    default: launch_dense_cfg<64, 128, 2, 4, 4, true>(st, W, bias, Hin, Hkeep, out, in, B, act, fa); break;
  }
}

__global__ __launch_bounds__(256) void tail_sse_kernel(const double* __restrict__ part, int slots, int out_last,
                                                       int64_t B, const double* __restrict__ bias_last, int act_last,
                                                       const double* __restrict__ Y, double* __restrict__ yhat,
                                                       double* __restrict__ blockpart, ChainBatch cb) {
  __shared__ double red[4];
  double accv = 0.0;
  const int64_t d = (int64_t)out_last * B;
  {
    const int64_t ch = blockIdx.y;
    part += ch * cb.part;
    bias_last += ch * cb.w;
    if (yhat) yhat += ch * d;
    blockpart += ch * gridDim.x;
  }
  const int64_t stride = (int64_t)gridDim.x * blockDim.x;
  for (int64_t idx = (int64_t)blockIdx.x * blockDim.x + threadIdx.x; idx < d; idx += stride) {
    const int o = (int)(idx % out_last);
    const int64_t b = idx / out_last;
    double s = 0.0;
#pragma unroll 4
    for (int sl = 0; sl < slots; ++sl) s += part[((int64_t)sl * out_last + o) * B + b];
    double v = s + bias_last[o];
    if (act_last == SI_ACT_RELU)
      v = v > 0.0 ? v : 0.0;
    else if (act_last != SI_ACT_IDENTITY)
      v = act_full(v, act_last);
    if (yhat) yhat[idx] = v;
    const double r = Y[idx] - v;
    accv += r * r;
  }
#pragma unroll
  for (int off = 32; off > 0; off >>= 1) accv += __shfl_down(accv, off, 64);
  if ((threadIdx.x & 63) == 0) red[threadIdx.x >> 6] = accv;
  __syncthreads();
  if (threadIdx.x == 0) blockpart[blockIdx.x] = (red[0] + red[1]) + (red[2] + red[3]);
}

void launch_tail_sse(hipStream_t st, const double* part, int slots, int out_last, int64_t B, const double* bias_last,
                     int act_last, const double* Y, double* yhat, double* blockpart, int nblocks, const ChainBatch& cb) {
  hipLaunchKernelGGL(tail_sse_kernel, dim3(nblocks, cb.n), dim3(256), 0, st, part, slots, out_last, B, bias_last,
                     act_last, Y, yhat, blockpart, cb);
}
#endif

}
```

subspaceinference.jl_amd/csrc/kernels_gemm_panel.hip:

```cpp
#include <atomic>
#include <cstdlib>
#include <type_traits>

#include "kernels_gemm.h"

namespace si {

typedef __attribute__((address_space(3))) void* lds_void_ptr_p;

__device__ __attribute__((aligned(16))) double si_panel_zero[1024 + 16];

#if defined(SI_PANEL_KNOB) && (SI_PANEL_KNOB & 8)
__device__ long long si_panel_stamps[4 * 2048];
#endif

__device__ __forceinline__ double panel_act(double v, int act) {
  switch (act) {
    case SI_ACT_RELU: return v > 0.0 ? v : 0.0;
    case SI_ACT_TANH: return tanh(v);
    case SI_ACT_SIGMOID: return 1.0 / (1.0 + exp(-v));
    default: return v;
  }
}

template <int N, typename F>
__device__ __forceinline__ void panel_static_for(F&& f) {
  if constexpr (N > 0) {
    panel_static_for<N - 1>(f);
    f(std::integral_constant<int, N - 1>{});
  }
}

typedef __attribute__((address_space(3))) const double* panel_lds_cptr;
template <int OFF>
__device__ __forceinline__ double panel_lds_read(unsigned addr) {
  double v;
  asm volatile("ds_read_b64 %0, %1 offset:%2" : "=v"(v) : "v"(addr), "n"(OFF));
  return v;
}
template <int N>
__device__ __forceinline__ void panel_lds_wait(double (&a)[4]) {
  asm volatile("s_waitcnt lgkmcnt(%0)" ::"n"(N) : "memory");
#pragma unroll
  for (int i = 0; i < 4; ++i) asm volatile("" : "+v"(a[i]));
}
template <int CH>
__device__ __forceinline__ void panel_read_chunk(unsigned fa, double (&a)[4]) {
  a[0] = panel_lds_read<512 * (4 * CH + 0)>(fa);
  a[1] = panel_lds_read<512 * (4 * CH + 1)>(fa);
  a[2] = panel_lds_read<512 * (4 * CH + 2)>(fa);
  a[3] = panel_lds_read<512 * (4 * CH + 3)>(fa);
}
template <int KT, int CH>
__device__ __forceinline__ void panel_chunks(unsigned fa, const double (&xf)[4 * KT], double (&cur)[4], double (&nxt)[4], d4& acc) {
  if constexpr (CH < KT) {
    if constexpr (CH + 1 < KT) {
      panel_read_chunk<CH + 1>(fa, nxt);
      panel_lds_wait<4>(cur);
    } else {
      panel_lds_wait<0>(cur);
    }
#pragma unroll
    for (int i = 0; i < 4; ++i) acc = __builtin_amdgcn_mfma_f64_16x16x4f64(xf[4 * CH + i], cur[i], acc, 0, 0, 0);
    panel_chunks<KT, CH + 1>(fa, xf, nxt, cur, acc);
  }
}

template <int KT, int RD, bool RAG>
__global__ __launch_bounds__(512, 4) void dense_f64_panel_kernel(const double* __restrict__ W, const double* __restrict__ bias,
                                                                  const double* __restrict__ Hin, double* __restrict__ Hout, int out,
                                                                  int in, int64_t B, int act, int ntile, int64_t units) {
  constexpr int IN = 16 * KT, KS = 4 * KT;
  constexpr int SLOT = IN * 16;
  constexpr int NINST = 2 * KT;
  constexpr int NDMA = (NINST + 7) / 8;
  constexpr int NST = 4;
  constexpr int NWAIT = (RD - 1) * NST + (RD - 2) * NDMA;
  static_assert(RD >= 2 && NWAIT <= 63, "vmcnt is a 6-bit counter");
  extern __shared__ double ring[];

#if defined(SI_PANEL_KNOB) && (SI_PANEL_KNOB & 8)
  const long long sr_entry = __builtin_amdgcn_s_memrealtime();
#endif
  const int64_t u0 = units * blockIdx.x / gridDim.x, u1 = units * (blockIdx.x + 1) / gridDim.x;
  if (u0 >= u1) return;
  const int tid = threadIdx.x, lane = tid & 63, wave = tid >> 6, q = lane >> 4, c = lane & 15;
  int64_t pan = u0 / ntile;
  int t = (int)(u0 - pan * ntile);
  const int tail = 16 * ntile - out;

  double* sbias = ring + RD * SLOT;
  for (int i = tid; i < 16 * ntile; i += 512) sbias[i] = bias[i >= 16 * (ntile - 1) ? i - tail : i];
  __syncthreads();

  const double* src[NDMA];
  int dsto[NDMA];
#pragma unroll
  for (int s = 0; s < NDMA; ++s) {
    int id = wave + 8 * s;
    if (id > NINST - 1) id = NINST - 1;
    const int k = 8 * id + (lane >> 3);
    src[s] = RAG && k >= in ? si_panel_zero + 2 * (lane & 7) : W + (int64_t)out * k + 2 * (lane & 7);
    dsto[s] = id * 128;
  }
  auto issue = [&](int tt, int slot) {
    const int shift = tt == ntile - 1 ? 16 * tt - tail : 16 * tt;
    panel_static_for<NDMA>([&](auto SC) {
      constexpr int s = decltype(SC)::value;
      __builtin_amdgcn_global_load_lds(reinterpret_cast<const void*>(src[s] + shift), (lds_void_ptr_p)(ring + slot * SLOT + dsto[s]), 16, 0, 0);
    });
  };

  double xf[KS];
  int so[4];
  double* Hp = Hout;
  auto load_panel = [&]() {
    int64_t gb = pan * 128 + 16 * wave + c;
    if (gb > B - 1) gb = B - 1;
    if constexpr (RAG) {
      const double* xp = Hin + (int64_t)in * gb + q;
#pragma unroll
      for (int s = 0; s < KS; ++s) {
        double xv = 0.0;
        if (4 * s + q < in) xv = xp[4 * s];
        xf[s] = xv;
      }
    } else {
      const double* xp = Hin + (int64_t)IN * gb + q;
#pragma unroll
      for (int s = 0; s < KS; ++s) xf[s] = xp[4 * s];
    }
    const int64_t left = B - 1 - pan * 128;
#pragma unroll
    for (int r = 0; r < 4; ++r) {
      int b = 16 * wave + q + 4 * r;
      if (b > left) b = (int)left;
      so[r] = b * out;
    }
    Hp = Hout + pan * 128 * out;
#pragma unroll
    for (int s = 0; s < KS; ++s) asm volatile("" : "+v"(xf[s]));
  };
  load_panel();
  int tpre = t;
#pragma unroll
  for (int d = 0; d < RD - 1; ++d) {
    issue(tpre, d);
    tpre = tpre + 1 == ntile ? 0 : tpre + 1;
  }

#if defined(SI_PANEL_KNOB) && (SI_PANEL_KNOB & 8)
  const long long st0 = __builtin_amdgcn_s_memtime(), sr0 = __builtin_amdgcn_s_memrealtime();
#endif
  const unsigned frag0 = (unsigned)(uintptr_t)(panel_lds_cptr)(ring + q * 16 + c);
  int slot = 0;
  for (int64_t u = u0; u < u1; ++u) {
    const int64_t n = u - u0;
    const double bv = sbias[16 * t + c];
    if (n >= RD - 1) {
      asm volatile("s_waitcnt vmcnt(%0) lgkmcnt(0)" ::"n"(NWAIT) : "memory");
    } else {
      panel_static_for<RD - 1>([&](auto NC) {
        constexpr int nc = decltype(NC)::value;
        if (n == nc) asm volatile("s_waitcnt vmcnt(%0) lgkmcnt(0)" ::"n"((RD - 2) * NDMA + NST * nc) : "memory");
      });
    }
#if !(defined(SI_PANEL_KNOB) && (SI_PANEL_KNOB & 4))
    __builtin_amdgcn_s_barrier();
#endif
    const int nxt = slot == 0 ? RD - 1 : slot - 1;
#if !(defined(SI_PANEL_KNOB) && (SI_PANEL_KNOB & 2))
    issue(tpre, nxt);
#endif
    tpre = tpre + 1 == ntile ? 0 : tpre + 1;
    d4 acc = (d4){0.0, 0.0, 0.0, 0.0};
    {
      const unsigned fa = frag0 + slot * (SLOT * 8);
      double wa[4], wb[4];
      panel_read_chunk<0>(fa, wa);
      panel_chunks<KT, 0>(fa, xf, wa, wb, acc);
    }
    const int fi = t == ntile - 1 ? 16 * t + c - tail : 16 * t + c;
    double v[4];
#pragma unroll
    for (int r = 0; r < 4; ++r) v[r] = acc[r] + bv;
    if (act == SI_ACT_RELU) {
#pragma unroll
      for (int r = 0; r < 4; ++r) v[r] = v[r] > 0.0 ? v[r] : 0.0;
    } else if (act != SI_ACT_IDENTITY) {
#pragma unroll
      for (int r = 0; r < 4; ++r) v[r] = panel_act(v[r], act);
    }
#pragma unroll
    for (int r = 0; r < 4; ++r) {
#if defined(SI_PANEL_KNOB) && (SI_PANEL_KNOB & 1)
      if (v[r] == 1.2345e300) Hp[so[r] + fi] = v[r];
#else
      Hp[so[r] + fi] = v[r];
#endif
    }
    slot = slot + 1 == RD ? 0 : slot + 1;
    if (++t == ntile) {
      t = 0;
      ++pan;
      if (u + 1 < u1) load_panel();
    }
  }
#if defined(SI_PANEL_KNOB) && (SI_PANEL_KNOB & 8)
  if (tid == 0 && blockIdx.x < 2048) {
    si_panel_stamps[4 * blockIdx.x] = __builtin_amdgcn_s_memtime() - st0;
    si_panel_stamps[4 * blockIdx.x + 1] = sr_entry;
    si_panel_stamps[4 * blockIdx.x + 2] = sr0;
    si_panel_stamps[4 * blockIdx.x + 3] = __builtin_amdgcn_s_memrealtime();
  }
#endif
  asm volatile("s_waitcnt vmcnt(0)" ::: "memory");
}

template <int KT>
static void launch_panel_inst(hipStream_t st, const double* W, const double* bias, const double* Hin, double* Hout, int32_t out,
                              int32_t in, int64_t B, int32_t act, int grid) {
#ifdef SI_PANEL_RD
  constexpr int RD = SI_PANEL_RD;
#else
  constexpr int RD = 4;
#endif
  const int ntile = (out + 15) / 16;
  const int64_t npan = (B + 127) / 128, units = npan * ntile;
  if (grid > units) grid = (int)units;
  const size_t lds = ((size_t)RD * KT * 256 + 16 * (size_t)ntile) * sizeof(double);
  if (in == 16 * KT)
    hipLaunchKernelGGL((dense_f64_panel_kernel<KT, RD, false>), dim3((unsigned)grid), dim3(512), lds, st, W, bias, Hin, Hout, (int)out, (int)in, B, (int)act,
                       ntile, units);
  else
    hipLaunchKernelGGL((dense_f64_panel_kernel<KT, RD, true>), dim3((unsigned)grid), dim3(512), lds, st, W, bias, Hin, Hout, (int)out, (int)in, B, (int)act,
                       ntile, units);
}

static int panel_grid() {
  static std::atomic<int> cached[64];
  int dev = 0;
  if (hipGetDevice(&dev) != hipSuccess || dev < 0 || dev >= 64) return 512;
  int g = cached[dev].load(std::memory_order_relaxed);
  if (g == 0) {
    int cus = 0;
    if (hipDeviceGetAttribute(&cus, hipDeviceAttributeMultiprocessorCount, dev) != hipSuccess || cus < 1) cus = 256;
    g = 2 * cus;
    cached[dev].store(g, std::memory_order_relaxed);
  }
  return g;
}

bool dense_panel_applies(const double* W, int32_t out, int32_t in, int64_t B, int32_t act) {
#ifdef SI_DEV_KNOBS
  static const bool off = [] { const char* e = getenv("SI_PANEL"); return e && e[0] == '0'; }();
  if (off) return false;
#endif
  if (in < 1 || in > 128 || out < 64 || out > 1024 || out % 2 != 0 || act_is_extra(act) || B < 1) return false;
  if ((reinterpret_cast<uintptr_t>(W) & 15) != 0) return false;
  return (int64_t)((out + 15) / 16) * ((B + 127) / 128) >= 16 * (int64_t)panel_grid();
}

bool launch_dense_f64_panel(hipStream_t st, const double* W, const double* bias, const double* Hin, double* Hout, int32_t out,
                            int32_t in, int64_t B, int32_t act, int grid) {
  if (in < 1 || in > 128 || out < 16 || out > 1024 || out % 2 != 0 || act_is_extra(act) || B < 1 || grid < 0) return false;
  if ((reinterpret_cast<uintptr_t>(W) & 15) != 0) return false;
  if (grid == 0) grid = panel_grid();
  switch ((in + 15) / 16) {
    case 1: launch_panel_inst<1>(st, W, bias, Hin, Hout, out, in, B, act, grid); break;
    case 2: launch_panel_inst<2>(st, W, bias, Hin, Hout, out, in, B, act, grid); break;
    case 3: launch_panel_inst<3>(st, W, bias, Hin, Hout, out, in, B, act, grid); break;
    case 4: launch_panel_inst<4>(st, W, bias, Hin, Hout, out, in, B, act, grid); break;
    case 5: launch_panel_inst<5>(st, W, bias, Hin, Hout, out, in, B, act, grid); break;
    case 6: launch_panel_inst<6>(st, W, bias, Hin, Hout, out, in, B, act, grid); break;
    case 7: launch_panel_inst<7>(st, W, bias, Hin, Hout, out, in, B, act, grid); break;
    default: launch_panel_inst<8>(st, W, bias, Hin, Hout, out, in, B, act, grid); break;
  }
  return true;
}

}
```

subspaceinference.jl_amd/csrc/si_internal.h:

```cpp
#pragma once
#include <hip/hip_runtime.h>
#include <stdint.h>

#include <string>
#include <vector>

#include "../../include/subspace_hip.h"
#include "dev_buf.h"

namespace si {

constexpr int64_t LD_ALIGN = 64;
inline int64_t pad_ld(int64_t n) { return (n + LD_ALIGN - 1) / LD_ALIGN * LD_ALIGN; }

enum { SI_CG_SYNC = 1, SI_CG_GLOBAL = 2, SI_CG_MARKER = 4 };
struct CgTileD {
  int64_t woff, boff;
  int32_t out, row0;
  int32_t in, pad2;
  int32_t flags;
  int32_t img_in, ldi;
  int32_t img_out, ldo;
  int32_t act, pad0, pad1;
};
// ... 39 lines not shown
  std::vector<DevBuf<float>> hs32;
  DevBuf<float> delta32[2];
  DevBuf<float> gw32, wt32, zero32, part32;
  DevBuf<double> rspart64, tailpart64, yhat64;
};

struct TrainState {
  std::vector<si_layer> layers;
  int64_t N = 0, Btot = 0, Bmax = 0;
  int32_t in_dim = 0, out_dim = 0;
  DevBuf<double> X, Y, Xb, Yb;
  DevBuf<int64_t> idx;
  PinBuf<int64_t> idx_pin[2];
  Event idx_ev[2];
  bool idx_busy[2] = {false, false};
  int idx_slot = 0;
  DevBuf<float> w32, m32, v32;
  DevBuf<double> w64, gw;
  std::vector<DevBuf<double>> hs;
  DevBuf<double> delta[2];
  DevBuf<double> bwpart, rspart, ssepart, sse;
  int sse_blocks = 0;
  int opt = 0;
  double eta = 0.0, p1 = 0.0, p2 = 0.0, bp1 = 0.0, bp2 = 0.0;
  bool grad_ready = false;
  bool fuse_tail = false;
  int fuse_slots = 0;
  DevBuf<double> part;
  bool f32 = false;
  DevBuf<float> X32, Xb32;
  SweepF32Ws ws32;
  NetPlan plan;
  DevBuf<double> Xc, wpack;
  NetScratch scratch;
  std::vector<DevBuf<uint8_t>> pidx;
};

struct CtxCore {
  int device = -1;
  TrainState* train = nullptr;
  hipStream_t own_stream = nullptr;
  hipStream_t stream = nullptr;
  std::string err;
  char devname[256] = {0};
  int num_cu = 256;
  void* comm = nullptr;
  int comm_world = 0, comm_rank = 0;
  double* d_commtmp = nullptr;
  double* d_gathertmp = nullptr;
  size_t gathertmp_cap = 0;

  hipStream_t stream2 = nullptr;
  PinBuf<double> h_pin;
  PinBuf<char> h_outpin;
  PinBuf<double> h_stage[2];
  DevBuf<double> d_stage[2], d_zstage[2];
  DevBuf<double> d_wring;
  DevBuf<int32_t> d_accflag;
  PinBuf<double> h_wring[4];
  Event ev_wcomp[4], ev_wcopy[4];
  int64_t wring_N = 0;
  int32_t wring_C = 0;
  bool profiling = false;
  uint32_t prof_mask = 0xffffffffu;
  std::vector<EventPair> pending;
  std::vector<hipEvent_t> event_pool;
  si_stats stats{};

  int32_t max_cols = 0;
  DevBuf<float> d_wstage;
  PinBuf<char> h_wpin[2];
  DevBuf<char> d_wpush[2];
  Event ev_wpin[2];
  Event ev_wk1[2];
  bool wpin_busy[2] = {false, false};
  uint64_t wpin_next = 0;
  DevBuf<double> d_nvals;
  std::vector<double> svals;
  std::vector<double> vfull;

  std::vector<si_layer> layers;
  int64_t iN = 0, ldP = 0;
  int32_t iM = 0;
  int32_t in_dim = 0, out_dim = 0;
  int64_t B = 0;
  double sigma_m = 1.0;
  int wsq_blocks = 0;
  int64_t act_elems = 0, max_stored = 0;
  int fuse_slots = 0;
  int sse_blocks = 0;
  int main_layer = 0;
  int64_t sw_itr = 0, sw_next = 0;
  double sw_sigma_z = 0.0, sw_d = 0.0;
  uint64_t sw_seed = 0;
  int32_t sw_chain0 = 0, sw_C = 0;
  bool sw_evaluated = false;
  bool defer_sse_final = false;
  bool chain_loop_enabled = true;
  int chain_mode = 1;
  int cg_start[5] = {0}, cg_count[5] = {0}, cg_chunks[5] = {0};
  bool chain_spec = true;
  std::string spec_message;

  CtxCore() = default;
  CtxCore(const CtxCore&) = delete;
  CtxCore& operator=(const CtxCore&) = delete;
  ~CtxCore() { delete train; }
};

struct ConstructState {
  bool c_active = false, c_finished = false, gram_valid = false;
  int64_t N = 0, ldA = 0, Kcap = 0, K = 0;
  int64_t npush = 0;
  DevBuf<double> d_swa;
  DevBuf<char> d_A;
  int32_t a_dtype = SI_F64;
  int32_t a_zero_dtype = -1;
  int64_t a_zero_cols = 0;
  bool a_pending = false;
  DevBuf<double> d_G;
  DevBuf<double> d_Gpart;
  DevBuf<double> d_V;
  DevBuf<double> d_P;
  int32_t M_built = 0;
  int refine_stage = 0;
  DevBuf<double> d_At;
  DevBuf<double> d_B;
};

struct HmcChain {
  double eps, mu, hbar, log_eps_bar, k0;
  int64_t da_t, wn;
  double s_eps, s_next, s_lo, s_hi, s_h0, s_trial;
  int32_t s_phase, s_dir, s_iter, s_done;
};

static constexpr int NUTS_MAX_DEPTH = 10;
struct NutsChain {
  double h0, logw, lpc, alpha_sum;
  double s_lp[NUTS_MAX_DEPTH], s_logw[NUTS_MAX_DEPTH], s_alpha[NUTS_MAX_DEPTH];
  int32_t s_n[NUTS_MAX_DEPTH], s_sel[NUTS_MAX_DEPTH];
  int64_t nlog;
  int32_t n_alpha, depth, ndoub, dir, k, sp, nleaf, selc, open;
};

struct InferState {
  bool i_ready = false;
  const double* i_swa = nullptr;
  const double* i_P = nullptr;
  DevBuf<double> d_iswa;
  DevBuf<double> d_iP;
  DevBuf<double> d_X;
  DevBuf<double> d_Y;
  double sigma_p = 0.0;
  DevBuf<double> d_wsq;
  DevBuf<double> d_wsqpart;
  int fw_slots = 0;
  DevBuf<double> d_w;
  DevBuf<double> d_act[2];
  DevBuf<double> d_ssepart;
  bool fuse_tail = false;
  DevBuf<double> d_part;
  DevBuf<double> d_yhat;
  bool f32 = false;
  int fuse_slots32 = 0;
  DevBuf<float> d_X32;
  DevBuf<float> d_w32;
  DevBuf<float> d_act32[2];
  bool g_ready = false;
  std::vector<DevBuf<double>> d_hs;
  DevBuf<double> d_delta[2];
  DevBuf<double> d_gw;
  DevBuf<double> d_bwpart;
  DevBuf<double> d_rspart;
  DevBuf<double> d_ptgpart;
  DevBuf<double> d_gz;
  SweepF32Ws g_ws32;
  NetPlan plan;
  DevBuf<double> d_Xc;
  DevBuf<double> d_wpack;
  DevBuf<float> d_wpack32;
  NetScratch g_scratch;
  std::vector<DevBuf<uint8_t>> d_pidx;
  DevBuf<double> d_zcur;
  DevBuf<double> d_zprop;
  DevBuf<double> d_lpcur;
  DevBuf<double> d_sse;
  DevBuf<int64_t> d_nacc;
  DevBuf<uint64_t> d_steps;
  int32_t chains_cap = 0;
  DevBuf<double> sw_Z, sw_lp;
  DevBuf<double> d_outZ, d_outlp;
  bool fused_ok = false;
  DevBuf<unsigned> d_gridsync;
  DevBuf<CgTileD> d_cgprog;
  DevBuf<double> d_specw;
  DevBuf<double> d_specy;
  DevBuf<int> d_specperm;
  const void* specperm_for = nullptr;
  int spec_chains = 0, spec_fo = 0;
  int last_density_spec = 0, last_loop_spec = 0;
  int vg_class = -1;
  int vg_cap = 0;
  DevBuf<double> d_vg_z, d_vg_w, d_vg_part, d_vg_ssepart, d_vg_gw, d_vg_lp, d_vg_gz;
  int last_grad_fused = 0;
  int mala_cap = 0;
  DevBuf<double> d_mala_z, d_mala_g, d_mala_zp, d_mala_gp;
  DevBuf<double> d_mala_lp, d_mala_lpp;
  DevBuf<int64_t> d_mala_nacc;
  DevBuf<double> d_outG;
  int last_mala_fused = 0, last_mala_passes = 0;
  int hmc_cap = 0;
  DevBuf<double> d_hmc_z, d_hmc_g, d_hmc_zp, d_hmc_gp, d_hmc_rh;
  DevBuf<double> d_hmc_minv, d_hmc_wmean, d_hmc_wm2;
  DevBuf<double> d_hmc_lp, d_hmc_lpp;
  DevBuf<HmcChain> d_hmc_chain;
  DevBuf<int32_t> d_hmc_open;
  DevBuf<double> d_outalpha, d_outeps, d_outMinv;
  int last_hmc_fused = 0, last_hmc_passes = 0, last_hmc_rounds = 0;
  int nuts_cap = 0;
  DevBuf<double> d_nuts_zm, d_nuts_rm, d_nuts_gm, d_nuts_zq, d_nuts_rq, d_nuts_gq, d_nuts_rho, d_nuts_zc, d_nuts_gc;
  DevBuf<double> d_nuts_stack;
  DevBuf<NutsChain> d_nuts_tree;
  DevBuf<int32_t> d_outdepth, d_outnleaf, d_outsel;
  DevBuf<double> d_outleaf;
  int last_nuts_fused = 0, last_nuts_passes = 0, last_nuts_search = 0;
  int64_t last_nuts_rounds = 0, last_nuts_leaves = 0;
  DevBuf<double> d_advi_theta;
  DevBuf<double> d_advi_ring;
  DevBuf<double> d_advi_eta, d_advi_z, d_advi_g;
  DevBuf<double> d_advi_lp;
  DevBuf<double> d_advi_trace, d_advi_pts;
  int last_advi_fused = 0, last_advi_passes = 0;
};

struct Ctx : CtxCore, ConstructState, InferState {};

void free_train(Ctx* c);
void comm_release(Ctx* c);
int32_t construct_adopt(Ctx* c, int64_t N, int32_t M);
void construct_install(Ctx* c, int64_t N, int32_t M, double* w_swa, double* P);

int32_t fail(Ctx* c, int32_t code, const std::string& msg);
#define SI_HIP(c, expr)                                                                    \
  do {                                                                                     \
    hipError_t e_ = (expr);                                                                \
    if (e_ != hipSuccess)                                                                  \
      return si::fail((c), SI_ERR_HIP, std::string(#expr) + ": " + hipGetErrorString(e_)); \
  } while (0)

struct LdsOptIn {
  size_t done[64] = {0};
  void ensure(const void* kern, size_t lds) {
    int dev = 0;
    if (hipGetDevice(&dev) != hipSuccess || dev < 0 || dev >= 64) dev = -1;
    if (dev >= 0 && done[dev] >= lds) return;
    (void)hipFuncSetAttribute(kern, hipFuncAttributeMaxDynamicSharedMemorySize, (int)lds);
    if (dev >= 0) done[dev] = lds;
  }
};

struct ProfScope {
  Ctx* c;
  int cls;
  hipEvent_t a = nullptr, b = nullptr;
  ProfScope(Ctx* c, int cls, double flops, double bytes);
  ~ProfScope();
};

void launch_swa_dev_push(hipStream_t st, const void* w, int32_t w_dtype, double* s, void* acol,
                         int64_t N, double n, int num_cu, int32_t a_dtype = SI_F64);
void launch_swa_dev_push_batch(hipStream_t st, const void* w, int32_t w_dtype, int64_t ld, double* s, void* A,
                               int64_t ldA, int64_t N, int count, const double* nvals_dev, int64_t slot0, int64_t kcap,
                               int num_cu, int32_t a_dtype = SI_F64);
size_t launch_gram(hipStream_t st, const void* A, int64_t ldA, int64_t N, int64_t K, double* Gpart,
                   double* G, int num_cu, Ctx* prof, int32_t a_dtype = SI_F64);
int project_mpad(int M);
void launch_project(hipStream_t st, const void* A, int64_t ldA, int64_t N, int64_t K, const double* V,
                    int32_t M, int32_t Mpad, double* P, int64_t ldP, int num_cu, int32_t a_dtype = SI_F64);
void launch_project_mfma(hipStream_t st, const double* A, int64_t ldA, int64_t N, int64_t K, const double* V, int32_t M,
                         int32_t Mpad, double* P, int64_t ldP);
bool launch_project_stream(hipStream_t st, const double* A, int64_t ldA, int64_t N, int64_t K, const double* V, int32_t M,
                           int32_t Mpad, double* P, int64_t ldP, int num_cu);
bool launch_project_stream_f32(hipStream_t st, const float* A, int64_t ldA, int64_t N, int64_t K, const double* V, int32_t M,
                               int32_t Mpad, double* P, int64_t ldP, int num_cu);
void launch_reconstruct(hipStream_t st, const double* swa, const double* P, int64_t ldP, int64_t N,
                        int32_t M, const double* Z, int32_t C, double* w, int64_t ldw, int num_cu,
                        float* w32 = nullptr , int64_t ldw32 = 0);
struct ChainBatch {
  int n = 1;
  int64_t w = 0, hin = 0, hout = 0, part = 0;
  int64_t part_ld = 0;
};
void launch_dense_f64(hipStream_t st, const double* W, const double* bias, const double* Hin,
                      double* Hout, int32_t out, int32_t in, int64_t B, int32_t act, const ChainBatch& cb = ChainBatch());
constexpr int SI_FUSE_MAX_OUT = 4;
int dense_fused_slots(int32_t out);
void launch_dense_f64_fused(hipStream_t st, const double* W, const double* bias, const double* Hin, int32_t out,
                            int32_t in, int64_t B, int32_t act, const double* Wlast, int32_t out_last, double* part,
                            const ChainBatch& cb = ChainBatch(), double* Hkeep = nullptr );
bool dense_panel_applies(const double* W, int32_t out, int32_t in, int64_t B, int32_t act);
bool launch_dense_f64_panel(hipStream_t st, const double* W, const double* bias, const double* Hin, double* Hout, int32_t out,
                            int32_t in, int64_t B, int32_t act, int grid = 0);
bool dense_small_applies(int32_t out, int32_t in, int64_t B, int nchains, int32_t bm);
void launch_dense_small_f64(hipStream_t st, const double* W, const double* bias, const double* Hin, double* Hout, int32_t out,
                            int32_t in, int64_t B, int32_t act, int32_t slot_feats, const ChainBatch& cb);
void launch_dense_small_f64_fused(hipStream_t st, const double* W, const double* bias, const double* Hin, int32_t out, int32_t in,
                                  int64_t B, int32_t act, int32_t slot_feats, int32_t nslots, const double* Wlast, int32_t out_last,
                                  double* part, const ChainBatch& cb, double* Hkeep);
void launch_dense_f32(hipStream_t st, const float* W, const float* bias, const float* Hin, float* Hout, int32_t out, int32_t in,
                      int64_t B, int32_t act, const ChainBatch& cb = ChainBatch());
int dense_f32_fused_slots(int32_t out, int32_t in, bool aligned);
bool launch_dense_f32_dx(hipStream_t st, const float* Wt, const float* zero_bias, const float* Delta, float* Dout, int32_t out,
                         int32_t in, int64_t B, const float* Hprev, int32_t act_prev);
void launch_dense_f32_fused(hipStream_t st, const float* W, const float* bias, const float* Hin, int32_t out, int32_t in, int64_t B,
                            int32_t act, const float* Wlast, int32_t out_last, double* part, const ChainBatch& cb = ChainBatch(),
                            float* Hkeep = nullptr);
void launch_narrow_f32(hipStream_t st, const double* src, float* dst, int64_t n);
void launch_sse_f32(hipStream_t st, const float* yhat, const double* y, int64_t d, double* part, int nblocks, double* sse_out,
                    int nch = 1, int64_t yhat_stride = 0, double* yhat64 = nullptr, int64_t yhat64_stride = 0, bool with_final = true);
void launch_tail_sse(hipStream_t st, const double* part, int slots, int out_last, int64_t B, const double* bias_last,
                     int act_last, const double* Y, double* yhat, double* blockpart, int nblocks,
                     const ChainBatch& cb = ChainBatch());
void launch_sse_final(hipStream_t st, const double* blockpart, int nblocks, double* sse_out, int nch = 1);
int sse_num_blocks(int64_t d, int num_cu);
void launch_sse(hipStream_t st, const double* yhat, const double* y, int64_t d, double* part,
                int nblocks, double* sse_out, int nch = 1, int64_t yhat_stride = 0, bool with_final = true);
void launch_backward_data(hipStream_t st, const double* W, const double* Delta, const double* Hprev, double* DeltaPrev,
                          int32_t out, int32_t in, int64_t B, int32_t act_prev);
template <typename T>
struct DenseForward {
  const si_layer* layers;
  size_t nl;
  bool fuse_tail;
  const T* w;
  const double* w64;
  const T* X;
  const double* Y;
  int64_t B;
  const DevBuf<T>* kept;
  T* pingpong[2];
  ChainBatch cb;
  int slots;
  double* part;
  double* yhat;
  double* ssepart;
  int sse_blocks;
  double* sse;
  bool defer_sse_final;
  int main_layer;
  bool traffic;
};
template <typename T>
const T* dense_forward(Ctx* ctx, hipStream_t st, const DenseForward<T>& a);
struct DenseSweep {
  const si_layer* layers;
  size_t nl;
  bool fuse_tail;
  const double* w;
  const double* X;
  const DevBuf<double>* hs;
  double* delta[2];
  double* gw;
  double* rspart;
  double* bwpart;
  int64_t B;
};
int32_t dense_reverse_sweep(Ctx* ctx, hipStream_t st, const DenseSweep& s);
struct DenseValueGrad {
  DenseSweep sw;
  const double* Y;
  int slots;
  double* part;
  double *ssepart, *sse;
  int sse_blocks;
  int64_t N;
  double scale;
  bool traffic;
};
int32_t dense_value_and_grad_f64(Ctx* ctx, hipStream_t st, const DenseValueGrad& s);
bool sweep_f32_alloc(Ctx* ctx, SweepF32Ws& ws, const si_layer* layers, int L, bool fuse_tail, int64_t N, int32_t in_dim, int32_t out_dim,
                     int64_t Bmax);
struct DenseSweepF32 {
  const si_layer* layers;
  size_t nl;
  bool fuse_tail;
  const float* w32;
  const double* w64;
  const float* X32;
  const double* Y;
  SweepF32Ws* ws;
  double* part;
  double *ssepart, *sse;
  int sse_blocks;
  int64_t B, N;
  double scale;
};
int32_t dense_value_and_grad_f32(Ctx* ctx, hipStream_t st, const DenseSweepF32& s);
void launch_widen_f32_to_f64(hipStream_t st, const float* src, int64_t n, double* dst, int num_cu);
size_t backward_weight_part_elems(int32_t out, int32_t in, int64_t B, int num_cu);
void launch_backward_weight(hipStream_t st, const double* Delta, const double* Hprev, double* part, int32_t out,
                            int32_t in, int64_t B, int num_cu, double* dW, double* db = nullptr);
void launch_split_reduce(hipStream_t st, const double* part, int nsplit, int64_t elems, double* dst);
void launch_delta_out(hipStream_t st, const double* Y, const double* Yhat, int64_t d, double scale, int act, double* delta);
void launch_rowsum(hipStream_t st, const double* D, int32_t out, int64_t B, double* part, double* db);
size_t tail_bwd_part_elems(int32_t out_last, int32_t F);
void launch_tail_bwd(hipStream_t st, const double* W, const double* Delta, const double* H, int32_t out_last, int32_t F,
                     int64_t B, int32_t act_prev, double* DeltaPrev, double* part, double* dW, double* dbprev);
int rowsum_chunks();
size_t backward_weight_f32_part_elems(int32_t out, int32_t in, int64_t B, int num_cu);
void launch_backward_weight_f32(hipStream_t st, const float* Delta, const float* Hprev, float* part, int32_t out, int32_t in, int64_t B,
                                int num_cu, float* dW);
void launch_transpose_f32(hipStream_t st, const float* W, int32_t out, int32_t in, float* Wt);
size_t rowsum_f32_part_elems(int max_rows);
void launch_mul_dact_rowsum_f32(hipStream_t st, const float* G, const float* H, int rows, int64_t B, int act, float* D, double* part,
                                float* db);
void launch_delta_out_f32(hipStream_t st, const double* Y, const double* Yhat64, const float* Yhat32, int64_t d, double scale, int act,
                          float* delta);
size_t tail_bwd_f32_part_elems(int32_t out_last, int32_t F);
void launch_tail_bwd_f32(hipStream_t st, const float* W, const float* Delta, const float* H, int32_t out_last, int32_t F, int64_t B,
                         int32_t act_prev, float* DeltaPrev, double* part, float* dW, float* dbprev);
void launch_ptg(hipStream_t st, const double* P, int64_t ldP, int64_t N, int M, const double* g, double* part, double* gz);
int ptg_blocks();
void launch_conv_pack(hipStream_t st, const double* w, const double* b, double* Wp, double* bp, int KW, int KH, int CIN, int COUT,
                      int CINp, int COUTp, int Kp);
void launch_conv_pack_t(hipStream_t st, const double* w, double* Wt, int KW, int KH, int CIN, int COUT, int CINp, int COUTp, int KpT);
void launch_conv_forward(hipStream_t st, const double* Wp, const double* bp, const double* In, double* Out, const ConvGeom& g,
                         int COUTp, int Kp, int64_t npos, int act);
void launch_conv_forward_pool2(hipStream_t st, const double* Wp, const double* bp, const double* In, double* Out, const ConvGeom& g,
                         int COUTp, int Kp, int64_t npos, int act);
void launch_conv_forward_pool2_idx(hipStream_t st, const double* Wp, const double* bp, const double* In, double* Out, uint8_t* Idx,
                                   const ConvGeom& g, int COUTp, int Kp, int64_t npos, int act);
void launch_pool2_bwd_idx(hipStream_t st, const double* G, const double* Hp, const uint8_t* Idx, double* D, int Cp, int W2, int H2,
                          int64_t B, int act, double* part, int nout, double* db);
void launch_conv_backward_data(hipStream_t st, const double* Wt, const double* Delta, double* dX, const ConvGeom& gT, int CINp,
                               int KpT, int64_t npos_in);
int conv_dw_max_splits(int COUTp, int Kp, int64_t npos, int num_cu);
int conv_dw_splits(int COUTp, int Kp, int64_t npos, int num_cu, int64_t* ksplit_out);
void launch_conv_backward_weight(hipStream_t st, const double* Delta, const double* In, double* part, const ConvGeom& g, int COUTp,
                                 int Kp, int64_t npos, int nsplit, int64_t ksplit);
void launch_conv_unpack_dw(hipStream_t st, const double* part, int nsplit, double* gw, int KW, int KH, int CIN, int COUT, int CINp,
                           int COUTp, int Kp);
void launch_whcn_to_cwhn(hipStream_t st, const double* X, double* Xc, int W, int H, int C, int Cp, int64_t B);
void launch_cwhn_to_whcn(hipStream_t st, const double* Xc, double* X, int W, int H, int C, int Cp, int64_t B);
void launch_maxpool(hipStream_t st, const double* In, double* Out, int Cp, int Wi, int Hi, int Wo, int Ho, int PW, int PH, int sw,
                    int sh, int64_t B);
void launch_maxpool_bwd(hipStream_t st, const double* In, const double* Out, const double* Gout, double* Gin, int Cp, int Wi, int Hi,
                        int Wo, int Ho, int PW, int PH, int sw, int sh, int64_t B);
void launch_mul_dact(hipStream_t st, const double* G, const double* H, int64_t n, int act, double* D);
size_t dact_rowsum_ws_elems(int max_rows);
void launch_act_inplace(hipStream_t st, double* H, int64_t n, int act);
void launch_conv_pack(hipStream_t st, const float* w, const float* b, float* Wp, float* bp, int KW, int KH, int CIN, int COUT, int CINp,
                      int COUTp, int Kp);
void launch_conv_forward(hipStream_t st, const float* Wp, const float* bp, const float* In, float* Out, const ConvGeom& g, int COUTp,
                         int Kp, int64_t npos, int act);
void launch_conv_forward_pool2(hipStream_t st, const float* Wp, const float* bp, const float* In, float* Out, const ConvGeom& g,
                               int COUTp, int Kp, int64_t npos, int act);
void launch_whcn_to_cwhn(hipStream_t st, const float* X, float* Xc, int W, int H, int C, int Cp, int64_t B);
void launch_cwhn_to_whcn(hipStream_t st, const float* Xc, float* X, int W, int H, int C, int Cp, int64_t B);
void launch_maxpool(hipStream_t st, const float* In, float* Out, int Cp, int Wi, int Hi, int Wo, int Ho, int PW, int PH, int sw, int sh,
                    int64_t B);
void launch_act_inplace(hipStream_t st, float* H, int64_t n, int act);
void launch_dense_narrow(hipStream_t st, const float* W, const float* bias, const float* Hin, float* Hout, int out, int in, int64_t B,
                         int act);
bool dense_narrow_applies(int out, int in, int64_t B, int num_cu);
void launch_dense_narrow(hipStream_t st, const double* W, const double* bias, const double* Hin, double* Hout, int out, int in, int64_t B,
                         int act);
void launch_maxpool_bwd_dact_rowsum(hipStream_t st, const double* In, const double* Out, const double* Gout, double* D, int Cp, int Wi,
                                    int Hi, int Wo, int Ho, int PW, int PH, int sw, int sh, int64_t B, int act, double* part, int nout,
                                    double* db);
void launch_mul_dact_rowsum(hipStream_t st, const double* G, const double* H, int rows, int64_t ncols, int act, double* D, double* part,
                            int nout, double* db);
int32_t net_plan(Ctx* c, const char* who, const si_layer* layers, int L, int64_t N, int in_dim, int out_dim, NetPlan& out);
void net_input(Ctx* c, const NetPlan& p, const double* X, double* Xc, int64_t B);
template <typename T>
int32_t net_forward(Ctx* c, const NetPlan& p, const T* w, const T* xin, int64_t B, const DevBuf<T>* outs, T* wpack, bool pingpong = false,
                    T** final_out = nullptr, const DevBuf<uint8_t>* pidx = nullptr);
bool net_grad_fused(const NetPlan& p, size_t l);
size_t net_pidx_bytes(const NetPlan& p, size_t l, int64_t B);
void net_scratch_sizes(const NetPlan& p, int64_t B, int num_cu, size_t* bwpart, size_t* rspart, size_t* wt, size_t* dbtmp);
int32_t net_backward(Ctx* c, const NetPlan& p, const double* w, const double* xin, int64_t B, const DevBuf<double>* hs, double* g0,
                     double* g1, double* gw, const NetScratch& s);
struct NetValueGrad {
  const NetPlan* plan;
  const double *w, *xin, *Y;
  int64_t B;
  const DevBuf<double>* hs;
  double* wpack;
  double* ssepart;
  int sse_blocks;
  double* sse;
  double* delta[2];
  double* gw;
  const NetScratch* scratch;
  int64_t N;
  double scale;
  double bwd_flops;
};
int32_t net_value_and_grad(Ctx* c, const NetValueGrad& s);
constexpr int SI_CHAIN_MAX_LAYERS = 8;
struct ChainLoopArgs {
  si_layer lay[SI_CHAIN_MAX_LAYERS];
  const double *swa, *P, *X, *Y;
  double *Z_out, *lp_out;
  int64_t* nacc_out;
  int64_t ldP, itr;
  uint64_t seed;
  double sigma_z, c0, sigma2;
  int N, M, B, L, chain_id0;
  int slot_feats, fuse_slots, nblocks;
  int p_in_lds;
  int o_X, o_Y, o_act0, o_act1, o_part, o_blk, o_z, o_red, o_P, o_swa, o_map;
  int wp[SI_CHAIN_MAX_LAYERS], bp[SI_CHAIN_MAX_LAYERS];
  long long* dbg_stamps;
};
size_t chain_loop_plan(ChainLoopArgs& a, size_t lds_limit);
void launch_chain_loop(hipStream_t st, const ChainLoopArgs& a, int nchains, size_t lds);
struct ChainFusedPlan {
  si_layer lay[SI_CHAIN_MAX_LAYERS];
  int L, B;
  int fuse_tail, slot_feats, fuse_slots;
  int ld[SI_CHAIN_MAX_LAYERS + 1];
  int o_x, o_buf[2], o_part;
  int lds_doubles;
  const CgTileD* prog;
  int prog_start[5], prog_count[5], prog_chunks[5];
};
void chain_fused_program(const si_layer* layers, int L, bool fuse_tail, std::vector<CgTileD>& prog, int start[5], int count[5],
                         int chunks[5]);
size_t chain_fused_plan(ChainFusedPlan& p, const si_layer* layers, int L, int64_t B, int NB, bool fuse_tail, int slot_feats,
                        int fuse_slots);
// ... 111 lines not shown
```

Baseline: 317.2.

## Pre-swizzle input X into MFMA fragment layout for first-layer panel GEMM

At inference setup, the input matrix X is rearranged once into the register-fragment order used by the f64 MFMA panel kernel. The first dense layer then loads X fragments with contiguous 16-byte vector loads instead of strided scalar loads. The panel kernel body moves into a shared header templated on this path. This costs extra device memory and a setup-time copy kernel, and only applies to f64 dense MLPs with in<=128 whose first layer qualifies for the panel kernel.

Measured after the change: 318.2, median of 6. Within noise of the previous version (+0.3%).

```diff
diff --git a/include/subspace_hip.h b/include/subspace_hip.h
--- a/include/subspace_hip.h
+++ b/include/subspace_hip.h
@@ -106,6 +106,7 @@
                            const double* W_swa_dev, const double* P_dev, int64_t ldP, int32_t borrow,
                            const double* X_dev, const double* Y_dev, int32_t in_dim, int32_t out_dim, int64_t B,
                            double sigma_m, int32_t compute_dtype);
+int32_t si_infer_xfrag_stats(si_ctx* ctx, int64_t* bytes_out);
 int32_t si_infer_set_prior(si_ctx* ctx, double sigma_p);
 int32_t si_logdensity(si_ctx* ctx, const double* Z, int32_t C, double* lp_out );
 int32_t si_logdensity_grad(si_ctx* ctx, const double* z , double* lp_out, double* grad_out );
diff --git a/subspaceinference.jl_amd/_capi.py b/subspaceinference.jl_amd/_capi.py
--- a/subspaceinference.jl_amd/_capi.py
+++ b/subspaceinference.jl_amd/_capi.py
@@ -144,6 +144,7 @@
     "si_set_chain_loop": (c_int32, [c_void_p, c_int32]),
     "si_chain_kernel_info": (c_int32, [c_void_p, POINTER(c_int32), POINTER(c_int32)]),
     "si_chain_spec_message": (c_char_p, [c_void_p]),
+    "si_infer_xfrag_stats": (c_int32, [c_void_p, POINTER(c_int64)]),
     "si_construct_set_storage": (c_int32, [c_void_p, c_int32]),
     "si_host_hmc_windows": (c_int32, [c_int64, POINTER(c_int64), POINTER(c_int64), c_void_p, c_int32]),
     "si_host_cpu_budget": (c_int, []),
@@ -696,6 +697,11 @@
         self._check(self.lib.si_chain_kernel_info(self.h, byref(d), byref(l)))
         return bool(d.value), bool(l.value), (self.lib.si_chain_spec_message(self.h) or b"").decode()
 
+    def infer_xfrag_bytes(self):
+        n = c_int64(0)
+        self._check(self.lib.si_infer_xfrag_stats(self.h, byref(n)))
+        return int(n.value)
+
     def rwmh_begin(self, itr, sigma_z, seed, chain_id0=0, nchains=1, d_total=0):
         self._check(self.lib.si_rwmh_begin(self.h, int(itr), float(sigma_z), int(seed), int(chain_id0), int(nchains),
                                            int(d_total)))
diff --git a/subspaceinference.jl_amd/build.py b/subspaceinference.jl_amd/build.py
--- a/subspaceinference.jl_amd/build.py
+++ b/subspaceinference.jl_amd/build.py
@@ -29,6 +29,7 @@
     ("kernels_gemm.hip", []),
     ("kernels_gemm_small.hip", []),
     ("kernels_gemm_panel.hip", []),
+    ("kernels_gemm_panel_xf.hip", []),
     ("kernels_gemm_f32.hip", []),
     ("kernels_gram.hip", []),
     ("kernels_gram_wave.hip", ["-DSI_GW_PART=0"], "kernels_gram_wave0"),
@@ -46,7 +47,7 @@
     ("eig_dispatch.cpp", []),
     ("chain_spec_rtc.cpp", []),
 ]
-HEADERS = ["si_internal.h", "dev_buf.h", "philox.h", "kernels_gemm.h", "gemm_pipeline.h", "chain_common.h", "hmc_device.h", "capi_common.h", "chain_spec.inc", "chain_spec_args.h",
+HEADERS = ["si_internal.h", "dev_buf.h", "philox.h", "kernels_gemm.h", "gemm_pipeline.h", "gemm_panel_body.h", "chain_common.h", "hmc_device.h", "capi_common.h", "chain_spec.inc", "chain_spec_args.h",
            "chain_spec_rtc.h", os.path.join("..", "..", "include", "subspace_hip.h")]
 SPEC_SOURCES = [("SI_SPEC_SRC_COMMON", "chain_common.h"), ("SI_SPEC_SRC_PHILOX", "philox.h"), ("SI_SPEC_SRC_ARGS", "chain_spec_args.h"),
                 ("SI_SPEC_SRC_KERNELS", "chain_spec.inc")]
diff --git a/subspaceinference.jl_amd/csrc/capi.hip b/subspaceinference.jl_amd/csrc/capi.hip
--- a/subspaceinference.jl_amd/csrc/capi.hip
+++ b/subspaceinference.jl_amd/csrc/capi.hip
@@ -130,7 +130,7 @@
       ProfScope ps(ctx, SI_K_DENSE, c.flops, a.traffic ? c.bytes : 0.0);
       ProfScope pm((int)l == a.main_layer ? ctx : nullptr, SI_K_DENSE_MAIN, c.flops, c.bytes);
       if constexpr (f64)
-        launch_dense_f64(st, a.w + ly.w_off, a.w + ly.b_off, h, o, ly.out, ly.in, B, ly.act, cb);
+        launch_dense_f64(st, a.w + ly.w_off, a.w + ly.b_off, h, o, ly.out, ly.in, B, ly.act, cb, l == 0 ? a.Xfrag : nullptr);
       else
         launch_dense_f32(st, a.w + ly.w_off, a.w + ly.b_off, h, o, ly.out, ly.in, B, ly.act, cb);
     }
@@ -199,7 +199,7 @@
   const DenseSweep& sw = s.sw;
   const size_t nl = sw.nl;
   const DenseForward<double> fw{sw.layers, nl, sw.fuse_tail, sw.w, sw.w, sw.X, s.Y, sw.B, sw.hs, {nullptr, nullptr}, ChainBatch(), s.slots,
-                                s.part, sw.hs[nl - 1], s.ssepart, s.sse_blocks, s.sse, false, -1, s.traffic};
+                                s.part, sw.hs[nl - 1], s.ssepart, s.sse_blocks, s.sse, false, -1, s.traffic, s.Xfrag};
   dense_forward(ctx, st, fw);
   double bflops = 0.0;
   for (size_t l = 0; l < nl; ++l) bflops += 4.0 * (double)sw.layers[l].in * sw.layers[l].out * (double)sw.B;
diff --git a/subspaceinference.jl_amd/csrc/capi_infer.hip b/subspaceinference.jl_amd/csrc/capi_infer.hip
--- a/subspaceinference.jl_amd/csrc/capi_infer.hip
+++ b/subspaceinference.jl_amd/csrc/capi_infer.hip
@@ -170,6 +170,16 @@
     launch_narrow_f32(ctx->stream, ctx->d_Xc, ctx->d_X32, plan.in_elems * B);
   else if (ctx->f32)
     launch_narrow_f32(ctx->stream, ctx->d_X, ctx->d_X32, (int64_t)in_dim * B);
+  if (!ctx->f32 && !plan.has_conv && !(ctx->fuse_tail && L == 2) && layers[0].in == in_dim &&
+      dense_panel_applies(ctx->d_w + layers[0].w_off, layers[0].out, layers[0].in, B,
+                          layers[0].act >= SI_ACT_LEAKYRELU ? SI_ACT_IDENTITY : layers[0].act )) {
+    if (ctx->d_Xfrag.alloc((size_t)dense_panel_xfrag_elems(in_dim, B))) {
+      launch_panel_xfrag(ctx->stream, ctx->d_X, in_dim, B, ctx->d_Xfrag);
+      ctx->xfrag_src = ctx->d_X;
+    } else {
+      (void)hipGetLastError();
+    }
+  }
   SI_HIP(ctx, hipGetLastError());
   SI_HIP(ctx, hipStreamSynchronize(ctx->stream));
   ctx->i_ready = true;
@@ -198,6 +208,14 @@
   }
   return infer_setup_common(ctx, layers, L, N, M, W_swa_dev, P_dev, ldP, X_dev, Y_dev, in_dim, out_dim, B, sigma_m,
                             compute_dtype, borrow ? SRC_DEV_BORROW : SRC_DEV_COPY);
+}
+
+int32_t si_infer_xfrag_stats(si_ctx* ctx, int64_t* bytes_out) {
+  CHECK_CTX(ctx);
+  if (!bytes_out) return fail(ctx, SI_ERR_INVALID, "si_infer_xfrag_stats: bad argument");
+  if (!ctx->i_ready) return fail(ctx, SI_ERR_STATE, "si_infer_xfrag_stats: call si_infer_setup first");
+  *bytes_out = ctx->xfrag_src ? (int64_t)(ctx->d_Xfrag.size() * sizeof(double)) : 0;
+  return SI_OK;
 }
 
 int32_t si_construct_result_ptr(si_ctx* ctx, double** W_swa_dev_out, double** P_dev_out, int64_t* ld_out, int32_t* M_out) {
@@ -345,7 +363,7 @@
   } else {
     const DenseForward<double> fw{ctx->layers.data(), ctx->layers.size(), ctx->fuse_tail, ctx->d_w, ctx->d_w, ctx->d_X, ctx->d_Y, B, nullptr,
                                   {ctx->d_act[0], ctx->d_act[1]}, cb, slots, ctx->d_part, yhat, ctx->d_ssepart, ctx->sse_blocks,
-                                  ctx->d_sse + c0, ctx->defer_sse_final, ctx->main_layer, true};
+                                  ctx->d_sse + c0, ctx->defer_sse_final, ctx->main_layer, true, ctx->xfrag_of(ctx->d_X)};
     const double* h = dense_forward(ctx, ctx->stream, fw);
     if (!ctx->fuse_tail) yh = h;
   }
@@ -499,7 +517,8 @@
   } else {
     const DenseValueGrad vg{{ctx->layers.data(), nl, ctx->fuse_tail, ctx->d_w, ctx->d_X, ctx->d_hs.data(), {ctx->d_delta[0], ctx->d_delta[1]},
                              ctx->d_gw, ctx->d_rspart, ctx->d_bwpart, B},
-                            ctx->d_Y, ctx->fuse_slots, ctx->d_part, ctx->d_ssepart, ctx->d_sse, ctx->sse_blocks, N, 1.0 / s2, true};
+                            ctx->d_Y, ctx->fuse_slots, ctx->d_part, ctx->d_ssepart, ctx->d_sse, ctx->sse_blocks, N, 1.0 / s2, true,
+                            ctx->xfrag_of(ctx->d_X)};
     if ((rc = dense_value_and_grad_f64(ctx, ctx->stream, vg)) != SI_OK) return rc;
   }
   if (prior) launch_prior_grad(ctx->stream, ctx->d_gw, ctx->d_w, N, 1.0 / (ctx->sigma_p * ctx->sigma_p), ctx->num_cu);
diff --git a/subspaceinference.jl_amd/csrc/gemm_panel_body.h b/subspaceinference.jl_amd/csrc/gemm_panel_body.h
--- /dev/null
+++ b/subspaceinference.jl_amd/csrc/gemm_panel_body.h
@@ -0,0 +1,235 @@
+#pragma once
+#include <type_traits>
+
+#include "kernels_gemm.h"
+
+namespace si {
+
+typedef __attribute__((address_space(3))) void* lds_void_ptr_p;
+typedef double panel_d2 __attribute__((ext_vector_type(2)));
+
+static __device__ __attribute__((aligned(16))) double si_panel_zero[1024 + 16];
+
+#if defined(SI_PANEL_KNOB) && (SI_PANEL_KNOB & 8)
+__device__ long long si_panel_stamps[4 * 2048];
+#endif
+
+__host__ __device__ inline int64_t panel_xfrag_groups(int64_t B) { return 8 * ((B + 127) / 128); }
+__host__ __device__ inline int64_t panel_xfrag_elems(int32_t in, int64_t B) { return panel_xfrag_groups(B) * (int64_t)((in + 15) / 16) * 256; }
+
+__device__ __forceinline__ double panel_act(double v, int act) {
+  switch (act) {
+    case SI_ACT_RELU: return v > 0.0 ? v : 0.0;
+    case SI_ACT_TANH: return tanh(v);
+    case SI_ACT_SIGMOID: return 1.0 / (1.0 + exp(-v));
+    default: return v;
+  }
+}
+
+template <int N, typename F>
+__device__ __forceinline__ void panel_static_for(F&& f) {
+  if constexpr (N > 0) {
+    panel_static_for<N - 1>(f);
+    f(std::integral_constant<int, N - 1>{});
+  }
+}
+
+typedef __attribute__((address_space(3))) const double* panel_lds_cptr;
+template <int OFF>
+__device__ __forceinline__ double panel_lds_read(unsigned addr) {
+  double v;
+  asm volatile("ds_read_b64 %0, %1 offset:%2" : "=v"(v) : "v"(addr), "n"(OFF));
+  return v;
+}
+template <int N>
+__device__ __forceinline__ void panel_lds_wait(double (&a)[4]) {
+  asm volatile("s_waitcnt lgkmcnt(%0)" ::"n"(N) : "memory");
+#pragma unroll
+  for (int i = 0; i < 4; ++i) asm volatile("" : "+v"(a[i]));
+}
+template <int CH>
+__device__ __forceinline__ void panel_read_chunk(unsigned fa, double (&a)[4]) {
+  a[0] = panel_lds_read<512 * (4 * CH + 0)>(fa);
+  a[1] = panel_lds_read<512 * (4 * CH + 1)>(fa);
+  a[2] = panel_lds_read<512 * (4 * CH + 2)>(fa);
+  a[3] = panel_lds_read<512 * (4 * CH + 3)>(fa);
+}
+template <int KT, int CH>
+__device__ __forceinline__ void panel_chunks(unsigned fa, const double (&xf)[4 * KT], double (&cur)[4], double (&nxt)[4], d4& acc) {
+  if constexpr (CH < KT) {
+    if constexpr (CH + 1 < KT) {
+      panel_read_chunk<CH + 1>(fa, nxt);
+      panel_lds_wait<4>(cur);
+    } else {
+      panel_lds_wait<0>(cur);
+    }
+#pragma unroll
+    for (int i = 0; i < 4; ++i) acc = __builtin_amdgcn_mfma_f64_16x16x4f64(xf[4 * CH + i], cur[i], acc, 0, 0, 0);
+    panel_chunks<KT, CH + 1>(fa, xf, nxt, cur, acc);
+  }
+}
+
+template <int KT, int RD, bool RAG, bool XF>
+__device__ __forceinline__ void panel_body(const double* __restrict__ W, const double* __restrict__ bias, const double* __restrict__ Hin,
+                                           double* __restrict__ Hout, int out, int in, int64_t B, int act, int ntile, int64_t units) {
+  static_assert(!(RAG && XF), "the copy pads the reduction itself");
+  constexpr int IN = 16 * KT, KS = 4 * KT;
+  constexpr int SLOT = IN * 16;
+  constexpr int NINST = 2 * KT;
+  constexpr int NDMA = (NINST + 7) / 8;
+  constexpr int NST = 4;
+  constexpr int NWAIT = (RD - 1) * NST + (RD - 2) * NDMA;
+  static_assert(RD >= 2 && NWAIT <= 63, "vmcnt is a 6-bit counter");
+  extern __shared__ double ring[];
+
+#if defined(SI_PANEL_KNOB) && (SI_PANEL_KNOB & 8)
+  const long long sr_entry = __builtin_amdgcn_s_memrealtime();
+#endif
+  const int64_t u0 = units * blockIdx.x / gridDim.x, u1 = units * (blockIdx.x + 1) / gridDim.x;
+  if (u0 >= u1) return;
+  const int tid = threadIdx.x, lane = tid & 63, wave = tid >> 6, q = lane >> 4, c = lane & 15;
+  int64_t pan = u0 / ntile;
+  int t = (int)(u0 - pan * ntile);
+  const int tail = 16 * ntile - out;
+
+  double* sbias = ring + RD * SLOT;
+  for (int i = tid; i < 16 * ntile; i += 512) sbias[i] = bias[i >= 16 * (ntile - 1) ? i - tail : i];
+  __syncthreads();
+
+  const double* src[NDMA];
+  int dsto[NDMA];
+#pragma unroll
+  for (int s = 0; s < NDMA; ++s) {
+    int id = wave + 8 * s;
+    if (id > NINST - 1) id = NINST - 1;
+    const int k = 8 * id + (lane >> 3);
+    src[s] = (RAG || XF) && k >= in ? si_panel_zero + 2 * (lane & 7) : W + (int64_t)out * k + 2 * (lane & 7);
+    dsto[s] = id * 128;
+  }
+  auto issue = [&](int tt, int slot) {
+    const int shift = tt == ntile - 1 ? 16 * tt - tail : 16 * tt;
+    panel_static_for<NDMA>([&](auto SC) {
+      constexpr int s = decltype(SC)::value;
+      __builtin_amdgcn_global_load_lds(reinterpret_cast<const void*>(src[s] + shift), (lds_void_ptr_p)(ring + slot * SLOT + dsto[s]), 16, 0, 0);
+    });
+  };
+
+  double xf[KS];
+  int so[4];
+  double* Hp = Hout;
+  auto load_panel = [&]() {
+    if constexpr (XF) {
+      const panel_d2* xp = reinterpret_cast<const panel_d2*>(Hin) + ((pan * 8 + wave) * (int64_t)(2 * KT) * 64 + lane);
+#pragma unroll
+      for (int j = 0; j < 2 * KT; ++j) {
+        const panel_d2 v = xp[64 * j];
+        xf[2 * j] = v.x;
+        xf[2 * j + 1] = v.y;
+      }
+    } else {
+      int64_t gb = pan * 128 + 16 * wave + c;
+      if (gb > B - 1) gb = B - 1;
+      if constexpr (RAG) {
+        const double* xp = Hin + (int64_t)in * gb + q;
+#pragma unroll
+        for (int s = 0; s < KS; ++s) {
+          double xv = 0.0;
+          if (4 * s + q < in) xv = xp[4 * s];
+          xf[s] = xv;
+        }
+      } else {
+        const double* xp = Hin + (int64_t)IN * gb + q;
+#pragma unroll
+        for (int s = 0; s < KS; ++s) xf[s] = xp[4 * s];
+      }
+    }
+    const int64_t left = B - 1 - pan * 128;
+#pragma unroll
+    for (int r = 0; r < 4; ++r) {
+      int b = 16 * wave + q + 4 * r;
+      if (b > left) b = (int)left;
+      so[r] = b * out;
+    }
+    Hp = Hout + pan * 128 * out;
+#pragma unroll
+    for (int s = 0; s < KS; ++s) asm volatile("" : "+v"(xf[s]));
+  };
+  load_panel();
+  int tpre = t;
+#pragma unroll
+  for (int d = 0; d < RD - 1; ++d) {
+    issue(tpre, d);
+    tpre = tpre + 1 == ntile ? 0 : tpre + 1;
+  }
+
+#if defined(SI_PANEL_KNOB) && (SI_PANEL_KNOB & 8)
+  const long long st0 = __builtin_amdgcn_s_memtime(), sr0 = __builtin_amdgcn_s_memrealtime();
+#endif
+  const unsigned frag0 = (unsigned)(uintptr_t)(panel_lds_cptr)(ring + q * 16 + c);
+  int slot = 0;
+  for (int64_t u = u0; u < u1; ++u) {
+    const int64_t n = u - u0;
+    const double bv = sbias[16 * t + c];
+    if (n >= RD - 1) {
+      asm volatile("s_waitcnt vmcnt(%0) lgkmcnt(0)" ::"n"(NWAIT) : "memory");
+    } else {
+      panel_static_for<RD - 1>([&](auto NC) {
+        constexpr int nc = decltype(NC)::value;
+        if (n == nc) asm volatile("s_waitcnt vmcnt(%0) lgkmcnt(0)" ::"n"((RD - 2) * NDMA + NST * nc) : "memory");
+      });
+    }
+#if !(defined(SI_PANEL_KNOB) && (SI_PANEL_KNOB & 4))
+    __builtin_amdgcn_s_barrier();
+#endif
+    const int nxt = slot == 0 ? RD - 1 : slot - 1;
+#if !(defined(SI_PANEL_KNOB) && (SI_PANEL_KNOB & 2))
+    issue(tpre, nxt);
+#endif
+    tpre = tpre + 1 == ntile ? 0 : tpre + 1;
+    d4 acc = (d4){0.0, 0.0, 0.0, 0.0};
+    {
+      const unsigned fa = frag0 + slot * (SLOT * 8);
+      double wa[4], wb[4];
+      panel_read_chunk<0>(fa, wa);
+      panel_chunks<KT, 0>(fa, xf, wa, wb, acc);
+    }
+    const int fi = t == ntile - 1 ? 16 * t + c - tail : 16 * t + c;
+    double v[4];
+#pragma unroll
+    for (int r = 0; r < 4; ++r) v[r] = acc[r] + bv;
+    if (act == SI_ACT_RELU) {
+#pragma unroll
+      for (int r = 0; r < 4; ++r) v[r] = v[r] > 0.0 ? v[r] : 0.0;
+    } else if (act != SI_ACT_IDENTITY) {
+#pragma unroll
+      for (int r = 0; r < 4; ++r) v[r] = panel_act(v[r], act);
+    }
+#pragma unroll
+    for (int r = 0; r < 4; ++r) {
+#if defined(SI_PANEL_KNOB) && (SI_PANEL_KNOB & 1)
+      if (v[r] == 1.2345e300) Hp[so[r] + fi] = v[r];
+#else
+      Hp[so[r] + fi] = v[r];
+#endif
+    }
+    slot = slot + 1 == RD ? 0 : slot + 1;
+    if (++t == ntile) {
+      t = 0;
+      ++pan;
+      if (u + 1 < u1) load_panel();
+    }
+  }
+#if defined(SI_PANEL_KNOB) && (SI_PANEL_KNOB & 8)
+  if (tid == 0 && blockIdx.x < 2048) {
+    si_panel_stamps[4 * blockIdx.x] = __builtin_amdgcn_s_memtime() - st0;
+    si_panel_stamps[4 * blockIdx.x + 1] = sr_entry;
+    si_panel_stamps[4 * blockIdx.x + 2] = sr0;
+    si_panel_stamps[4 * blockIdx.x + 3] = __builtin_amdgcn_s_memrealtime();
+  }
+#endif
+  asm volatile("s_waitcnt vmcnt(0)" ::: "memory");
+}
+
+int panel_grid();
+
+}
diff --git a/subspaceinference.jl_amd/csrc/kernels_gemm.hip b/subspaceinference.jl_amd/csrc/kernels_gemm.hip
--- a/subspaceinference.jl_amd/csrc/kernels_gemm.hip
+++ b/subspaceinference.jl_amd/csrc/kernels_gemm.hip
@@ -405,9 +405,9 @@
 int dense_fused_slots(int32_t out);
 
 void launch_dense_f64(hipStream_t st, const double* W, const double* bias, const double* Hin,
-                      double* Hout, int32_t out, int32_t in, int64_t B, int32_t act, const ChainBatch& cb) {
+                      double* Hout, int32_t out, int32_t in, int64_t B, int32_t act, const ChainBatch& cb, const double* Hin_frag) {
   if (act_is_extra(act)) {
-    launch_dense_f64(st, W, bias, Hin, Hout, out, in, B, SI_ACT_IDENTITY, cb);
+    launch_dense_f64(st, W, bias, Hin, Hout, out, in, B, SI_ACT_IDENTITY, cb, Hin_frag);
     for (int s = 0; s < cb.n; ++s) launch_act_inplace(st, Hout + (int64_t)s * cb.hout, (int64_t)out * B, act);
     return;
   }
@@ -415,8 +415,10 @@
     launch_dense_small_f64(st, W, bias, Hin, Hout, out, in, B, act, dense_fused_slot_feats(out), cb);
     return;
   }
-  if (cb.n <= 1 && dense_panel_applies(W, out, in, B, act) && launch_dense_f64_panel(st, W, bias, Hin, Hout, out, in, B, act))
-    return;
+  if (cb.n <= 1 && dense_panel_applies(W, out, in, B, act)) {
+    if (Hin_frag && launch_dense_f64_panel_xf(st, W, bias, Hin_frag, Hout, out, in, B, act)) return;
+    if (launch_dense_f64_panel(st, W, bias, Hin, Hout, out, in, B, act)) return;
+  }
   FuseArgs fa;
   fa.cb = cb;
   switch (pick_bm(out)) {
diff --git a/subspaceinference.jl_amd/csrc/kernels_gemm_panel.hip b/subspaceinference.jl_amd/csrc/kernels_gemm_panel.hip
--- a/subspaceinference.jl_amd/csrc/kernels_gemm_panel.hip
+++ b/subspaceinference.jl_amd/csrc/kernels_gemm_panel.hip
@@ -1,220 +1,15 @@
 #include <atomic>
 #include <cstdlib>
-#include <type_traits>
 
-#include "kernels_gemm.h"
+#include "gemm_panel_body.h"
 
 namespace si {
-
-typedef __attribute__((address_space(3))) void* lds_void_ptr_p;
-
-__device__ __attribute__((aligned(16))) double si_panel_zero[1024 + 16];
-
-#if defined(SI_PANEL_KNOB) && (SI_PANEL_KNOB & 8)
-__device__ long long si_panel_stamps[4 * 2048];
-#endif
-
-__device__ __forceinline__ double panel_act(double v, int act) {
-  switch (act) {
-    case SI_ACT_RELU: return v > 0.0 ? v : 0.0;
-    case SI_ACT_TANH: return tanh(v);
-    case SI_ACT_SIGMOID: return 1.0 / (1.0 + exp(-v));
-    default: return v;
-  }
-}
-
-template <int N, typename F>
-__device__ __forceinline__ void panel_static_for(F&& f) {
-  if constexpr (N > 0) {
-    panel_static_for<N - 1>(f);
-    f(std::integral_constant<int, N - 1>{});
-  }
-}
-
-typedef __attribute__((address_space(3))) const double* panel_lds_cptr;
-template <int OFF>
-__device__ __forceinline__ double panel_lds_read(unsigned addr) {
-  double v;
-  asm volatile("ds_read_b64 %0, %1 offset:%2" : "=v"(v) : "v"(addr), "n"(OFF));
-  return v;
-}
-template <int N>
-__device__ __forceinline__ void panel_lds_wait(double (&a)[4]) {
-  asm volatile("s_waitcnt lgkmcnt(%0)" ::"n"(N) : "memory");
-#pragma unroll
-  for (int i = 0; i < 4; ++i) asm volatile("" : "+v"(a[i]));
-}
-template <int CH>
-__device__ __forceinline__ void panel_read_chunk(unsigned fa, double (&a)[4]) {
-  a[0] = panel_lds_read<512 * (4 * CH + 0)>(fa);
-  a[1] = panel_lds_read<512 * (4 * CH + 1)>(fa);
-  a[2] = panel_lds_read<512 * (4 * CH + 2)>(fa);
-  a[3] = panel_lds_read<512 * (4 * CH + 3)>(fa);
-}
-template <int KT, int CH>
-__device__ __forceinline__ void panel_chunks(unsigned fa, const double (&xf)[4 * KT], double (&cur)[4], double (&nxt)[4], d4& acc) {
-  if constexpr (CH < KT) {
-    if constexpr (CH + 1 < KT) {
-      panel_read_chunk<CH + 1>(fa, nxt);
-      panel_lds_wait<4>(cur);
-    } else {
-      panel_lds_wait<0>(cur);
-    }
-#pragma unroll
-    for (int i = 0; i < 4; ++i) acc = __builtin_amdgcn_mfma_f64_16x16x4f64(xf[4 * CH + i], cur[i], acc, 0, 0, 0);
-    panel_chunks<KT, CH + 1>(fa, xf, nxt, cur, acc);
-  }
-}
 
 template <int KT, int RD, bool RAG>
 __global__ __launch_bounds__(512, 4) void dense_f64_panel_kernel(const double* __restrict__ W, const double* __restrict__ bias,
                                                                   const double* __restrict__ Hin, double* __restrict__ Hout, int out,
                                                                   int in, int64_t B, int act, int ntile, int64_t units) {
-  constexpr int IN = 16 * KT, KS = 4 * KT;
-  constexpr int SLOT = IN * 16;
-  constexpr int NINST = 2 * KT;
-  constexpr int NDMA = (NINST + 7) / 8;
-  constexpr int NST = 4;
-  constexpr int NWAIT = (RD - 1) * NST + (RD - 2) * NDMA;
-  static_assert(RD >= 2 && NWAIT <= 63, "vmcnt is a 6-bit counter");
-  extern __shared__ double ring[];
-
-#if defined(SI_PANEL_KNOB) && (SI_PANEL_KNOB & 8)
-  const long long sr_entry = __builtin_amdgcn_s_memrealtime();
-#endif
-  const int64_t u0 = units * blockIdx.x / gridDim.x, u1 = units * (blockIdx.x + 1) / gridDim.x;
-  if (u0 >= u1) return;
-  const int tid = threadIdx.x, lane = tid & 63, wave = tid >> 6, q = lane >> 4, c = lane & 15;
-  int64_t pan = u0 / ntile;
-  int t = (int)(u0 - pan * ntile);
-  const int tail = 16 * ntile - out;
-
-  double* sbias = ring + RD * SLOT;
-  for (int i = tid; i < 16 * ntile; i += 512) sbias[i] = bias[i >= 16 * (ntile - 1) ? i - tail : i];
-  __syncthreads();
-
-  const double* src[NDMA];
-  int dsto[NDMA];
-#pragma unroll
-  for (int s = 0; s < NDMA; ++s) {
-    int id = wave + 8 * s;
-    if (id > NINST - 1) id = NINST - 1;
-    const int k = 8 * id + (lane >> 3);
-    src[s] = RAG && k >= in ? si_panel_zero + 2 * (lane & 7) : W + (int64_t)out * k + 2 * (lane & 7);
-    dsto[s] = id * 128;
-  }
-  auto issue = [&](int tt, int slot) {
-    const int shift = tt == ntile - 1 ? 16 * tt - tail : 16 * tt;
-    panel_static_for<NDMA>([&](auto SC) {
-      constexpr int s = decltype(SC)::value;
-      __builtin_amdgcn_global_load_lds(reinterpret_cast<const void*>(src[s] + shift), (lds_void_ptr_p)(ring + slot * SLOT + dsto[s]), 16, 0, 0);
-    });
-  };
-
-  double xf[KS];
-  int so[4];
-  double* Hp = Hout;
-  auto load_panel = [&]() {
-    int64_t gb = pan * 128 + 16 * wave + c;
-    if (gb > B - 1) gb = B - 1;
-    if constexpr (RAG) {
-      const double* xp = Hin + (int64_t)in * gb + q;
-#pragma unroll
-      for (int s = 0; s < KS; ++s) {
-        double xv = 0.0;
-        if (4 * s + q < in) xv = xp[4 * s];
-        xf[s] = xv;
-      }
-    } else {
-      const double* xp = Hin + (int64_t)IN * gb + q;
-#pragma unroll
-      for (int s = 0; s < KS; ++s) xf[s] = xp[4 * s];
-    }
-    const int64_t left = B - 1 - pan * 128;
-#pragma unroll
-    for (int r = 0; r < 4; ++r) {
-      int b = 16 * wave + q + 4 * r;
-      if (b > left) b = (int)left;
-      so[r] = b * out;
-    }
-    Hp = Hout + pan * 128 * out;
-#pragma unroll
-    for (int s = 0; s < KS; ++s) asm volatile("" : "+v"(xf[s]));
-  };
-  load_panel();
-  int tpre = t;
-#pragma unroll
-  for (int d = 0; d < RD - 1; ++d) {
-    issue(tpre, d);
-    tpre = tpre + 1 == ntile ? 0 : tpre + 1;
-  }
-
-#if defined(SI_PANEL_KNOB) && (SI_PANEL_KNOB & 8)
-  const long long st0 = __builtin_amdgcn_s_memtime(), sr0 = __builtin_amdgcn_s_memrealtime();
-#endif
-  const unsigned frag0 = (unsigned)(uintptr_t)(panel_lds_cptr)(ring + q * 16 + c);
-  int slot = 0;
-  for (int64_t u = u0; u < u1; ++u) {
-    const int64_t n = u - u0;
-    const double bv = sbias[16 * t + c];
-    if (n >= RD - 1) {
-      asm volatile("s_waitcnt vmcnt(%0) lgkmcnt(0)" ::"n"(NWAIT) : "memory");
-    } else {
-      panel_static_for<RD - 1>([&](auto NC) {
-        constexpr int nc = decltype(NC)::value;
-        if (n == nc) asm volatile("s_waitcnt vmcnt(%0) lgkmcnt(0)" ::"n"((RD - 2) * NDMA + NST * nc) : "memory");
-      });
-    }
-#if !(defined(SI_PANEL_KNOB) && (SI_PANEL_KNOB & 4))
-    __builtin_amdgcn_s_barrier();
-#endif
-    const int nxt = slot == 0 ? RD - 1 : slot - 1;
-#if !(defined(SI_PANEL_KNOB) && (SI_PANEL_KNOB & 2))
-    issue(tpre, nxt);
-#endif
-    tpre = tpre + 1 == ntile ? 0 : tpre + 1;
-    d4 acc = (d4){0.0, 0.0, 0.0, 0.0};
-    {
-      const unsigned fa = frag0 + slot * (SLOT * 8);
-      double wa[4], wb[4];
-      panel_read_chunk<0>(fa, wa);
-      panel_chunks<KT, 0>(fa, xf, wa, wb, acc);
-    }
-    const int fi = t == ntile - 1 ? 16 * t + c - tail : 16 * t + c;
-    double v[4];
-#pragma unroll
-    for (int r = 0; r < 4; ++r) v[r] = acc[r] + bv;
-    if (act == SI_ACT_RELU) {
-#pragma unroll
-      for (int r = 0; r < 4; ++r) v[r] = v[r] > 0.0 ? v[r] : 0.0;
-    } else if (act != SI_ACT_IDENTITY) {
-#pragma unroll
-      for (int r = 0; r < 4; ++r) v[r] = panel_act(v[r], act);
-    }
-#pragma unroll
-    for (int r = 0; r < 4; ++r) {
-#if defined(SI_PANEL_KNOB) && (SI_PANEL_KNOB & 1)
-      if (v[r] == 1.2345e300) Hp[so[r] + fi] = v[r];
-#else
-      Hp[so[r] + fi] = v[r];
-#endif
-    }
-    slot = slot + 1 == RD ? 0 : slot + 1;
-    if (++t == ntile) {
-      t = 0;
-      ++pan;
-      if (u + 1 < u1) load_panel();
-    }
-  }
-#if defined(SI_PANEL_KNOB) && (SI_PANEL_KNOB & 8)
-  if (tid == 0 && blockIdx.x < 2048) {
-    si_panel_stamps[4 * blockIdx.x] = __builtin_amdgcn_s_memtime() - st0;
-    si_panel_stamps[4 * blockIdx.x + 1] = sr_entry;
-    si_panel_stamps[4 * blockIdx.x + 2] = sr0;
-    si_panel_stamps[4 * blockIdx.x + 3] = __builtin_amdgcn_s_memrealtime();
-  }
-#endif
-  asm volatile("s_waitcnt vmcnt(0)" ::: "memory");
+  panel_body<KT, RD, RAG, false>(W, bias, Hin, Hout, out, in, B, act, ntile, units);
 }
 
 template <int KT>
@@ -237,7 +32,7 @@
                        ntile, units);
 }
 
-static int panel_grid() {
+int panel_grid() {
   static std::atomic<int> cached[64];
   int dev = 0;
   if (hipGetDevice(&dev) != hipSuccess || dev < 0 || dev >= 64) return 512;
diff --git a/subspaceinference.jl_amd/csrc/kernels_gemm_panel_xf.hip b/subspaceinference.jl_amd/csrc/kernels_gemm_panel_xf.hip
--- /dev/null
+++ b/subspaceinference.jl_amd/csrc/kernels_gemm_panel_xf.hip
@@ -0,0 +1,67 @@
+#include "gemm_panel_body.h"
+
+namespace si {
+
+template <int KT, int RD>
+__global__ __launch_bounds__(512, 4) void dense_f64_panel_xf_kernel(const double* __restrict__ W, const double* __restrict__ bias,
+                                                                     const double* __restrict__ Xf, double* __restrict__ Hout, int out,
+                                                                     int in, int64_t B, int act, int ntile, int64_t units) {
+  panel_body<KT, RD, false, true>(W, bias, Xf, Hout, out, in, B, act, ntile, units);
+}
+
+__global__ __launch_bounds__(256) void panel_xfrag_kernel(const double* __restrict__ X, int in, int64_t B, int kt2, int64_t pieces,
+                                                           panel_d2* __restrict__ Xf) {
+  const int64_t idx = (int64_t)blockIdx.x * 256 + threadIdx.x;
+  if (idx >= pieces) return;
+  const int lane = (int)(idx & 63), q = lane >> 4, c = lane & 15;
+  const int64_t gj = idx >> 6, g = gj / kt2;
+  const int j = (int)(gj - g * kt2);
+  int64_t col = 16 * g + c;
+  if (col > B - 1) col = B - 1;
+  const int k0 = 8 * j + q, k1 = k0 + 4;
+  panel_d2 v;
+  v.x = k0 < in ? X[(int64_t)in * col + k0] : 0.0;
+  v.y = k1 < in ? X[(int64_t)in * col + k1] : 0.0;
+  Xf[idx] = v;
+}
+
+int64_t dense_panel_xfrag_elems(int32_t in, int64_t B) { return in >= 1 && in <= 128 && B >= 1 ? panel_xfrag_elems(in, B) : 0; }
+
+void launch_panel_xfrag(hipStream_t st, const double* X, int32_t in, int64_t B, double* Xf) {
+  const int kt2 = 2 * ((in + 15) / 16);
+  const int64_t pieces = panel_xfrag_groups(B) * kt2 * 64;
+  hipLaunchKernelGGL(panel_xfrag_kernel, dim3((unsigned)((pieces + 255) / 256)), dim3(256), 0, st, X, (int)in, B, kt2, pieces,
+                     reinterpret_cast<panel_d2*>(Xf));
+}
+
+template <int KT>
+static void launch_panel_xf_inst(hipStream_t st, const double* W, const double* bias, const double* Xf, double* Hout, int32_t out,
+                                 int32_t in, int64_t B, int32_t act, int grid) {
+  constexpr int RD = 4;
+  const int ntile = (out + 15) / 16;
+  const int64_t npan = (B + 127) / 128, units = npan * ntile;
+  if (grid > units) grid = (int)units;
+  const size_t lds = ((size_t)RD * KT * 256 + 16 * (size_t)ntile) * sizeof(double);
+  hipLaunchKernelGGL((dense_f64_panel_xf_kernel<KT, RD>), dim3((unsigned)grid), dim3(512), lds, st, W, bias, Xf, Hout, (int)out, (int)in, B, (int)act,
+                     ntile, units);
+}
+
+bool launch_dense_f64_panel_xf(hipStream_t st, const double* W, const double* bias, const double* Xf, double* Hout, int32_t out,
+                               int32_t in, int64_t B, int32_t act) {
+  if (in < 1 || in > 128 || out < 16 || out > 1024 || out % 2 != 0 || act_is_extra(act) || B < 1 || !Xf) return false;
+  if ((reinterpret_cast<uintptr_t>(W) & 15) != 0 || (reinterpret_cast<uintptr_t>(Xf) & 15) != 0) return false;
+  const int grid = panel_grid();
+  switch ((in + 15) / 16) {
+    case 1: launch_panel_xf_inst<1>(st, W, bias, Xf, Hout, out, in, B, act, grid); break;
+    case 2: launch_panel_xf_inst<2>(st, W, bias, Xf, Hout, out, in, B, act, grid); break;
+    case 3: launch_panel_xf_inst<3>(st, W, bias, Xf, Hout, out, in, B, act, grid); break;
+    case 4: launch_panel_xf_inst<4>(st, W, bias, Xf, Hout, out, in, B, act, grid); break;
+    case 5: launch_panel_xf_inst<5>(st, W, bias, Xf, Hout, out, in, B, act, grid); break;
+    case 6: launch_panel_xf_inst<6>(st, W, bias, Xf, Hout, out, in, B, act, grid); break;
+    case 7: launch_panel_xf_inst<7>(st, W, bias, Xf, Hout, out, in, B, act, grid); break;
+    default: launch_panel_xf_inst<8>(st, W, bias, Xf, Hout, out, in, B, act, grid); break;
+  }
+  return true;
+}
+
+}
diff --git a/subspaceinference.jl_amd/csrc/si_internal.h b/subspaceinference.jl_amd/csrc/si_internal.h
--- a/subspaceinference.jl_amd/csrc/si_internal.h
+++ b/subspaceinference.jl_amd/csrc/si_internal.h
@@ -215,6 +215,9 @@
   DevBuf<double> d_iP;
   DevBuf<double> d_X;
   DevBuf<double> d_Y;
+  DevBuf<double> d_Xfrag;
+  const double* xfrag_src = nullptr;
+  const double* xfrag_of(const double* X) const { return X && X == xfrag_src ? d_Xfrag.get() : nullptr; }
   double sigma_p = 0.0;
   DevBuf<double> d_wsq;
   DevBuf<double> d_wsqpart;
@@ -356,7 +359,8 @@
   int64_t part_ld = 0;
 };
 void launch_dense_f64(hipStream_t st, const double* W, const double* bias, const double* Hin,
-                      double* Hout, int32_t out, int32_t in, int64_t B, int32_t act, const ChainBatch& cb = ChainBatch());
+                      double* Hout, int32_t out, int32_t in, int64_t B, int32_t act, const ChainBatch& cb = ChainBatch(),
+                      const double* Hin_frag = nullptr);
 constexpr int SI_FUSE_MAX_OUT = 4;
 int dense_fused_slots(int32_t out);
 void launch_dense_f64_fused(hipStream_t st, const double* W, const double* bias, const double* Hin, int32_t out,
@@ -365,6 +369,10 @@
 bool dense_panel_applies(const double* W, int32_t out, int32_t in, int64_t B, int32_t act);
 bool launch_dense_f64_panel(hipStream_t st, const double* W, const double* bias, const double* Hin, double* Hout, int32_t out,
                             int32_t in, int64_t B, int32_t act, int grid = 0);
+int64_t dense_panel_xfrag_elems(int32_t in, int64_t B);
+void launch_panel_xfrag(hipStream_t st, const double* X, int32_t in, int64_t B, double* Xf);
+bool launch_dense_f64_panel_xf(hipStream_t st, const double* W, const double* bias, const double* Xf, double* Hout, int32_t out,
+                               int32_t in, int64_t B, int32_t act);
 bool dense_small_applies(int32_t out, int32_t in, int64_t B, int nchains, int32_t bm);
 void launch_dense_small_f64(hipStream_t st, const double* W, const double* bias, const double* Hin, double* Hout, int32_t out,
                             int32_t in, int64_t B, int32_t act, int32_t slot_feats, const ChainBatch& cb);
@@ -413,6 +421,7 @@
   bool defer_sse_final;
   int main_layer;
   bool traffic;
+  const double* Xfrag = nullptr;
 };
 template <typename T>
 const T* dense_forward(Ctx* ctx, hipStream_t st, const DenseForward<T>& a);
@@ -440,6 +449,7 @@
   int64_t N;
   double scale;
   bool traffic;
+  const double* Xfrag = nullptr;
 };
 int32_t dense_value_and_grad_f64(Ctx* ctx, hipStream_t st, const DenseValueGrad& s);
 bool sweep_f32_alloc(Ctx* ctx, SweepF32Ws& ws, const si_layer* layers, int L, bool fuse_tail, int64_t N, int32_t in_dim, int32_t out_dim,
```
